# timohouben/GNN-XAI-TimeSeries-QualityControl

Measured on AMD Instinct MI355X. Metric: ROC-AUC (5-fold CV) + train windows/sec, CML GCN at 1/2/4/8 MI355X, higher is better.
Workload: dtype bf16; 1 GPU; model=CML GCN (GeneralConv16+mean pool+LSTM TimeLayer f16 n_stacks2+dense64), global_batch=128, seq_len=181, parallelism=dp1, adjacency=radius(max_sample_distance=20), graph_steps=8, trainable_params=188193, hip_graph=True

## Files before the change

csrc/kernels/lstm_chain.hip:

```cpp
#include "chain_head.h"
#include "common.h"
#include "gcn_fused.h"
#include "lstm_grads_body.h"
#include "lstm_tm_common.h"

#include <cstdlib>
#include <type_traits>

namespace gq {

typedef unsigned long long u64x2_t __attribute__((ext_vector_type(2)));
typedef unsigned u32x4_t __attribute__((ext_vector_type(4)));
typedef __bf16 bf16x2_t __attribute__((ext_vector_type(2)));

static constexpr int CHAIN_MAX = 8;
static constexpr int CHAIN_SPIN = 1 << 20;
#ifndef CHAIN_D
#define CHAIN_D 4
#endif
#ifndef CHAIN_D3
#define CHAIN_D3 2
#endif
#ifndef CHAIN_LEAD1
#define CHAIN_LEAD1 1
#endif
#ifndef CHAIN_D0
#define CHAIN_D0 6
#endif
#ifndef CHAIN_LD16
#define CHAIN_LD16 0
#endif
#ifndef CHAIN_W_SLEEP
#define CHAIN_W_SLEEP 0
#endif
#ifndef CHAIN_W_NAPMAX
#define CHAIN_W_NAPMAX 1
#endif
#ifndef CHAIN_RP_NAPMAX
#define CHAIN_RP_NAPMAX 16
#endif
#ifndef CHAIN_PRIO
#define CHAIN_PRIO 2
#endif
#ifndef CHAIN_LEAD3
#define CHAIN_LEAD3 1
#endif

struct ChainStage {
  const float* x;
  const unsigned long long* xin;
  const float* W;
  const float* U;
  const float* b;
  float* h;
  __bf16* g;
  float* c;
  unsigned long long* sout;
  float* pout;
  unsigned* iout;
  float* pin_out;
  unsigned char* pin_idx;
  long long* prof;
  int H, T, Din, Dw, KX, P, PIN;
};

struct ChainT4 {
  const unsigned long long* xin;
  const float* W;
  const float* U;
  const float* b;
  float* h;
  float* g;
  float* c;
  float* pin_out;
  unsigned char* pin_idx;
  int T, Din, Dw, on;
  ChainHead hd;
  float* hb;
};

struct ChainArgs {
  ChainStage st[CHAIN_MAX];
  int ns, ntiles, nt8, Mp;
  int* ctl;
  long long* trace;
  const float* pkU;
  const float* pkW;
  bf16x8_t* pk;
  int pkDw;
  int npk;
  ChainT4 t4;
  GcnCoefFwdJob cf;
  GcnProdJob gp;
};
static_assert(sizeof(ChainArgs) <= 4096, "chain forward kernel arguments");

__device__ __forceinline__ unsigned long long ld_granule(const unsigned long long* p) {
  return __hip_atomic_load(p, __ATOMIC_RELAXED, __HIP_MEMORY_SCOPE_AGENT);
}

__device__ __forceinline__ void st_granule(unsigned long long* p, float v, unsigned tag) {
  __hip_atomic_store(p, ((unsigned long long)tag << 32) | __float_as_uint(v), __ATOMIC_RELAXED,
                     __HIP_MEMORY_SCOPE_AGENT);
}

template <bool INL>
__device__ __forceinline__ unsigned long long chain_wait_body(const unsigned long long* p, unsigned want, int* ctl);
__device__ __noinline__ unsigned long long chain_wait(const unsigned long long* p, unsigned want, int* ctl) {
  return chain_wait_body<false>(p, want, ctl);
}
__device__ __forceinline__ unsigned long long chain_wait_inl(const unsigned long long* p, unsigned want, int* ctl) {
  return chain_wait_body<true>(p, want, ctl);
}
template <bool INL>
__device__ __forceinline__ unsigned long long chain_wait_body(const unsigned long long* p, unsigned want, int* ctl) {
  unsigned long long v = 0;
  const bool l0 = (threadIdx.x & 63) == 0;
#ifdef GQ_CHAIN_PROF
  if (l0) __hip_atomic_fetch_add(ctl + 9, 1, __ATOMIC_RELAXED, __HIP_MEMORY_SCOPE_AGENT);
#endif
  int nap = 1;
  const int lim0 = __hip_atomic_load(ctl + 6, __ATOMIC_RELAXED, __HIP_MEMORY_SCOPE_AGENT);
  const int lim = lim0 > 0 ? lim0 : CHAIN_SPIN;
  for (int it = 0; it < lim; ++it) {
    unsigned t0 = want;
    if (l0) t0 = (unsigned)(ld_granule(p) >> 32);
    if ((unsigned)__builtin_amdgcn_readfirstlane((int)t0) == want) {
      v = ld_granule(p);
      if (__builtin_amdgcn_ballot_w64((unsigned)(v >> 32) != want) == 0) return v;
    }
    for (int k = 0; k < nap; ++k) __builtin_amdgcn_s_sleep(CHAIN_W_SLEEP);
    nap = min(nap * 2, CHAIN_W_NAPMAX);
  }
  __hip_atomic_store(ctl + 2, 1, __ATOMIC_RELAXED, __HIP_MEMORY_SCOPE_AGENT);
  return v;
}

__device__ __forceinline__ void chain_wait_count(const int* p, int n, int* ctl) {
  const int lim0 = __hip_atomic_load(ctl + 6, __ATOMIC_RELAXED, __HIP_MEMORY_SCOPE_AGENT);
  const int lim = lim0 > 0 ? lim0 : CHAIN_SPIN;
  int nap = 1;
  for (int it = 0; it < lim; ++it) {
    if (__hip_atomic_load(p, __ATOMIC_RELAXED, __HIP_MEMORY_SCOPE_AGENT) >= n) return;
    for (int k = 0; k < nap; ++k) __builtin_amdgcn_s_sleep(CHAIN_W_SLEEP);
    nap = min(nap * 2, CHAIN_W_NAPMAX);
  }
  __hip_atomic_store(ctl + 2, 1, __ATOMIC_RELAXED, __HIP_MEMORY_SCOPE_AGENT);
}

static constexpr int CHAIN_PROF_STEPS = 64;
#ifdef GQ_CHAIN_PROF
__device__ __forceinline__ void chain_mark(long long* pr, int step, int k) {
  if (pr != nullptr && threadIdx.x == 0 && step < CHAIN_PROF_STEPS)
    pr[step * 8 + k] = (long long)__builtin_amdgcn_s_memtime();
}
__device__ __forceinline__ void chain_mark_wave(long long* pr, int step, int k) {
  if (pr != nullptr && (threadIdx.x & 63) == 0 && step < CHAIN_PROF_STEPS)
    pr[step * 8 + k] = (long long)__builtin_amdgcn_s_memtime();
}
#else
__device__ __forceinline__ void chain_mark(long long*, int, int) {}
__device__ __forceinline__ void chain_mark_wave(long long*, int, int) {}
#endif

__device__ __forceinline__ unsigned chain_tag_base(unsigned E) { return ((E % 0xFFFFFu) + 1u) << 12; }

template <int H, int KX>
struct ChainLds {
  static constexpr int HS = 2 * 16 * (TMC<H>::KPH + 8) * 2;
  static constexpr int XS = 2 * 16 * (32 * KX + 8) * 2;
  static constexpr int HF = 2 * 16 * TMC<H>::HP * 4;
  static constexpr int GS = 2 * 16 * H * 8;
  static constexpr int CS = 2 * 16 * H * 4;
  static constexpr int BYTES = HS + XS + HF + GS + CS;
};
constexpr int chain_max2(int a, int b) { return a > b ? a : b; }
static constexpr int CHAIN_LDS_STAGE = chain_max2(chain_max2(ChainLds<64, 2>::BYTES, ChainLds<32, 2>::BYTES),
                                                  ChainLds<16, 2>::BYTES);

__device__ __forceinline__ float chain_gate_scale(int ag) { return ag == 2 ? -2.8853900817779268f : -1.4426950408889634f; }

__host__ __device__ constexpr int chain_io_waves(int nt, int d, int ngl = 1, int pin = 1) {
  return nt + 64 * d + 64 <= 1024 && ngl * pin <= 12 ? d : 0;
}
__host__ __device__ constexpr int chain_io_group(int pin, int kx = 1, int h = 16) {
  return pin > 1 || (h == 64 && kx == 2) ? 2 : 1;
}
__host__ __device__ constexpr int chain_stage_d(int h, int kx, int d) {
  return h == 64 && kx == 2 && d > 3 ? 3 : d;
}
__host__ __device__ constexpr int chain_live_threads(int nt, int d, int kx, bool src, int pin, int h = 16) {
  return nt + 64 * chain_io_waves(nt, d * chain_io_group(pin, kx, h),
                                  (16 * 32 * kx / (src ? 2 : 4) + 64 * chain_io_group(pin, kx, h) - 1) /
                                      (64 * chain_io_group(pin, kx, h)),
                                  pin) +
         (chain_io_waves(nt, d * chain_io_group(pin, kx, h),
                         (16 * 32 * kx / (src ? 2 : 4) + 64 * chain_io_group(pin, kx, h) - 1) /
                             (64 * chain_io_group(pin, kx, h)),
                         pin) > 0 ? 64 : 0);
}

template <int H>
struct ChainCfg {
  static constexpr int CPL = H == 64 ? 2 : 1;
  static constexpr int NW = H / 4 / CPL, NT = 64 * NW, G4 = 4 * H;
  static constexpr int KSH = TMC<H>::KSH, KPH = TMC<H>::KPH, HP = TMC<H>::HP;
  static constexpr int NWV = H / 4, NCELL = 64 * NWV;
};

template <int H, bool TRAIN, int KX, int D, bool SRC, int PIN>
__device__ __forceinline__ void chain_stage(const ChainStage& S, int tile, int ntiles, int Mp, unsigned tagb,
                                            int* ctl, char* smem) {
  using C = ChainCfg<H>;
  constexpr int NW = C::NW, NT = C::NT, G4 = C::G4, CPL = C::CPL, NWV = C::NWV, NCELL = C::NCELL;
  constexpr int KPX = 32 * KX;
  constexpr int GR = SRC ? 2 : 4;
  constexpr int G = chain_io_group(PIN, KX, H);
  constexpr int NIOW = chain_io_waves(NT, D * G, (16 * KPX / GR + 64 * G - 1) / (64 * G), PIN);
  constexpr bool IOW = NIOW > 0;
  constexpr int NIO = IOW ? 64 * G : NT;
  constexpr int NSLOT = IOW ? 1 : D;
  constexpr int NGL = IOW ? (16 * KPX / GR + NIO - 1) / NIO : 1;
  using L = ChainLds<H, KX>;
  static_assert(L::BYTES <= CHAIN_LDS_STAGE && L::HS % 16 == 0 && L::XS % 16 == 0, "chain LDS layout");
  auto hs = reinterpret_cast<__bf16 (*)[16][C::KPH + 8]>(smem);
  auto xs = reinterpret_cast<__bf16 (*)[16][KPX + 8]>(smem + L::HS);
  auto hf = reinterpret_cast<float (*)[16][C::HP]>(smem + L::HS + L::XS);
  auto gst = reinterpret_cast<uint2 (*)[NCELL]>(smem + L::HS + L::XS + L::HF);
  auto cst = reinterpret_cast<float (*)[NCELL]>(smem + L::HS + L::XS + L::HF + L::GS);

  const int T = S.T, Din = S.Din, Dw = S.Dw, P = S.P;
  const int tid = threadIdx.x, lane = tid & 63;
  const int w = __builtin_amdgcn_readfirstlane(tid >> 6);
  const int col = lane & 15, quad = lane >> 4;
  const int row0 = tile * 16;
  const size_t hstep = (size_t)Mp * H;
  const int To = P > 0 ? T / P : T;

  constexpr int NTL = NT + 64 * NIOW + (IOW ? 64 : 0);
  for (int i = tid; i < 2 * 16 * (C::KPH + 8); i += NTL) (&hs[0][0][0])[i] = (__bf16)0.0f;
  for (int i = tid; i < 2 * 16 * (KPX + 8); i += NTL) (&xs[0][0][0])[i] = (__bf16)0.0f;

  const bool compute = w < NW;
  const int iow = IOW ? (w - NW) / G : 0;
  const int iot = IOW ? ((w - NW) % G) * 64 + lane : tid;
  const int n_gx = 16 * Din / GR;
  const size_t xstep = (size_t)Mp * Din;
  int goff[NGL], loff[NGL];
#pragma unroll
  for (int j = 0; j < NGL; ++j) {
    const int gx = min(iot + NIO * j, n_gx - 1) * GR;
    goff[j] = gx;
    loff[j] = ((gx / Din) * (KPX + 8) + gx % Din) * 2;
  }
  const size_t xbase = (size_t)row0 * Din;
  char* xsb = reinterpret_cast<char*>(&xs[0][0][0]);
  constexpr int XBUF = 16 * (KPX + 8) * 2;
  f32x4_t xr[NSLOT][NGL];
  u64x2_t xq[NSLOT][NGL][PIN];
  const __amdgpu_buffer_rsrc_t xrs = __builtin_amdgcn_make_buffer_rsrc(
      const_cast<unsigned long long*>(SRC ? S.xin : nullptr), (short)0, 0x7fffffff, 0x00020000);
  auto load_x = [&](int r, int tx) {
#pragma unroll
    for (int q = 0; q < (SRC ? PIN : 1); ++q) {
      const size_t tb = xbase + (size_t)(SRC ? PIN * tx + q : tx) * xstep;
#pragma unroll
      for (int j = 0; j < NGL; ++j) {
        if constexpr (SRC) {
#if CHAIN_LD16
          const u32x4_t v = __builtin_amdgcn_raw_buffer_load_b128(xrs, (int)((tb + goff[j]) * 8), 0, 16);
          xq[r][j][q] = u64x2_t{((unsigned long long)v.y << 32) | v.x, ((unsigned long long)v.w << 32) | v.z};
#else
          xq[r][j][q] = u64x2_t{ld_granule(S.xin + tb + goff[j]), ld_granule(S.xin + tb + goff[j] + 1)};
#endif
        } else {
          xr[r][j] = *reinterpret_cast<const f32x4_t*>(S.x + tb + goff[j]);
        }
      }
    }
  };
  auto stage_x = [&](int buf, int r, int tx) {
    if constexpr (SRC) {
      bool bad = false;
#pragma unroll
      for (int j = 0; j < NGL; ++j)
#pragma unroll
        for (int q = 0; q < PIN; ++q) {
          const unsigned want = tagb | (unsigned)(PIN * tx + q);
          bad |= (unsigned)(xq[r][j][q].x >> 32) != want || (unsigned)(xq[r][j][q].y >> 32) != want;
        }
      if (__builtin_amdgcn_ballot_w64(bad) != 0) {
#ifdef GQ_CHAIN_PROF
        if (lane == 0) __hip_atomic_fetch_add(ctl + 9, 1, __ATOMIC_RELAXED, __HIP_MEMORY_SCOPE_AGENT);
#endif
        const int lim0 = __hip_atomic_load(ctl + 6, __ATOMIC_RELAXED, __HIP_MEMORY_SCOPE_AGENT);
        const int lim = lim0 > 0 ? lim0 : CHAIN_SPIN;
        int nap = 1;
        for (int it = 0;; ++it) {
#pragma unroll
          for (int q = 0; q < PIN; ++q) {
            const size_t tb = xbase + (size_t)(PIN * tx + q) * xstep;
#pragma unroll
            for (int j = 0; j < NGL; ++j)
              xq[r][j][q] = u64x2_t{ld_granule(S.xin + tb + goff[j]), ld_granule(S.xin + tb + goff[j] + 1)};
          }
          bad = false;
#pragma unroll
          for (int j = 0; j < NGL; ++j)
#pragma unroll
            for (int q = 0; q < PIN; ++q) {
              const unsigned want = tagb | (unsigned)(PIN * tx + q);
              bad |= (unsigned)(xq[r][j][q].x >> 32) != want || (unsigned)(xq[r][j][q].y >> 32) != want;
            }
          if (__builtin_amdgcn_ballot_w64(bad) == 0) break;
          if (it >= lim) {
            __hip_atomic_store(ctl + 2, 1, __ATOMIC_RELAXED, __HIP_MEMORY_SCOPE_AGENT);
            break;
          }
          for (int k = 0; k < nap; ++k) __builtin_amdgcn_s_sleep(2);
          nap = min(nap * 2, CHAIN_RP_NAPMAX);
        }
      }
      const size_t po = xbase + (size_t)tx * xstep;
#pragma unroll
      for (int j = 0; j < NGL; ++j) {
        float m0 = __uint_as_float((unsigned)xq[r][j][0].x), m1 = __uint_as_float((unsigned)xq[r][j][0].y);
        if constexpr (PIN > 1) {
          unsigned a0 = 0, a1 = 0;
#pragma unroll
          for (int q = 1; q < PIN; ++q) {
            const float v0 = __uint_as_float((unsigned)xq[r][j][q].x), v1 = __uint_as_float((unsigned)xq[r][j][q].y);
            if (v0 > m0) { m0 = v0; a0 = q; }
            if (v1 > m1) { m1 = v1; a1 = q; }
          }
          *reinterpret_cast<float2*>(S.pin_out + po + goff[j]) = make_float2(m0, m1);
          *reinterpret_cast<unsigned short*>(S.pin_idx + po + goff[j]) = (unsigned short)(a0 | (a1 << 8));
        }
        *reinterpret_cast<bf16x2_t*>(xsb + buf * XBUF + loff[j]) = bf16x2_t{(__bf16)m0, (__bf16)m1};
      }
    } else {
#pragma unroll
      for (int j = 0; j < NGL; ++j) {
        const bf16x4_t v = __builtin_convertvector(xr[r][j], bf16x4_t);
        *reinterpret_cast<bf16x4_t*>(xsb + buf * XBUF + loff[j]) = v;
      }
    }
  };

  const int wc = compute ? w : 0;
  const int ag = col & 3;
  int unit[CPL];
  bf16x8_t ufr[CPL][C::KSH], wfr[CPL][KX];
  f32x4_t bias4[CPL];
#pragma unroll
  for (int cc = 0; cc < CPL; ++cc) {
    const int gi = wc + NW * cc;
    const int au = 4 * gi + (col >> 2);
    unit[cc] = 4 * gi + quad;
    bias4[cc] = f32x4_t{0.f, 0.f, 0.f, 0.f};
    if (compute) {
#pragma unroll
      for (int s = 0; s < C::KSH; ++s) {
        bf16x8_t v;
#pragma unroll
        for (int j = 0; j < 8; ++j) {
          const int k = 32 * s + 8 * quad + j;
          v[j] = (__bf16)(S.U[min(k, H - 1) * G4 + ag * H + au] * (k < H ? 1.0f : 0.0f));
        }
        ufr[cc][s] = v;
      }
#pragma unroll
      for (int s = 0; s < KX; ++s) {
        bf16x8_t v;
#pragma unroll
        for (int j = 0; j < 8; ++j) {
          const int k = 32 * s + 8 * quad + j;
          v[j] = (__bf16)(S.W[min(k, Dw - 1) * G4 + ag * H + au] * (k < Dw ? 1.0f : 0.0f));
        }
        wfr[cc][s] = v;
      }
      const int u = unit[cc];
      bias4[cc] = f32x4_t{S.b[u], S.b[H + u], S.b[2 * H + u], S.b[3 * H + u]};
    }
  }
  float* hp[CPL];
  unsigned long long* sp[CPL];
  __bf16* gp[CPL];
  float* cp[CPL];
  const size_t gstride = (size_t)ntiles * NWV * 64;
#pragma unroll
  for (int cc = 0; cc < CPL; ++cc) {
    const size_t hoff = (size_t)(row0 + col) * H + unit[cc];
    hp[cc] = S.h + hoff;
    sp[cc] = S.sout != nullptr ? S.sout + hoff : nullptr;
    gp[cc] = S.g + (((size_t)tile * NWV + wc + NW * cc) * 64 + lane) * 4;
    cp[cc] = S.c + ((size_t)tile * NWV + wc + NW * cc) * 64 + lane;
  }
  const bool publish = S.sout != nullptr;
  const bool own_pool = P > 0;

  constexpr int n_gh = 16 * H / 4;
  constexpr int NPT = IOW ? 64 : NT;
  constexpr int NPL = (n_gh + NPT - 1) / NPT;
  PoolAcc pool[NPL];
  const bool publisher = IOW && w == NW + NIOW;
  const bool pooler = IOW ? publisher : wave_uniform(tid < n_gh);
  auto pool_step = [&](int tp) {
#pragma unroll
    for (int q = 0; q < NPL; ++q) {
      const int gh = (((IOW ? lane : tid) + NPT * q) % n_gh) * 4;
      const float4 v = *reinterpret_cast<const float4*>(&hf[tp & 1][gh / H][gh % H]);
      pool[q].step(v, tp, P, To, S.pout, S.iout, (size_t)row0 * H + gh, hstep);
    }
  };

  const bool streamer = IOW ? (!compute && !publisher) : true;
  if (streamer) {
    if constexpr (SRC) {
      constexpr int LEAD = PIN > 1 ? CHAIN_LEAD3 : CHAIN_LEAD1;
      const int tw = min(D + LEAD, T - 1);
      (void)chain_wait(S.xin + xbase + goff[0] + 1 + (size_t)(PIN * tw + PIN - 1) * xstep,
                       tagb | (unsigned)(PIN * tw + PIN - 1), ctl);
    }
    if constexpr (IOW) {
      load_x(0, min(iow, T - 1));
    } else {
#pragma unroll
      for (int r = 0; r < D; ++r) load_x(r, min(r, T - 1));
    }
  }
  __syncthreads();
  if (IOW ? (streamer && iow == 0) : streamer) {
    stage_x(0, 0, 0);
    if (!IOW) load_x(0, min(D, T - 1));
  }
  float c[CPL];
#pragma unroll
  for (int cc = 0; cc < CPL; ++cc) c[cc] = 0.f;
  __syncthreads();

  long long* pr = (S.prof != nullptr && tile == 0) ? S.prof : nullptr;
  auto compute_step = [&](int t, auto IO, int rn) {
    constexpr bool DOI = decltype(IO)::value;
    const int p = t & 1;
    chain_mark(pr, t, 0);
    f32x4_t acc[CPL];
#pragma unroll
    for (int cc = 0; cc < CPL; ++cc) {
      f32x4_t accx = bias4[cc], acch = {0.f, 0.f, 0.f, 0.f};
#pragma unroll
      for (int s = 0; s < KX; ++s) {
        const bf16x8_t bx = *reinterpret_cast<const bf16x8_t*>(&xs[p][col][32 * s + 8 * quad]);
        accx = __builtin_amdgcn_mfma_f32_16x16x32_bf16(wfr[cc][s], bx, accx, 0, 0, 0);
      }
#pragma unroll
      for (int s = 0; s < C::KSH; ++s) {
        const bf16x8_t bh = *reinterpret_cast<const bf16x8_t*>(&hs[p][col][32 * s + 8 * quad]);
        acch = __builtin_amdgcn_mfma_f32_16x16x32_bf16(ufr[cc][s], bh, acch, 0, 0, 0);
      }
      acc[cc] = accx + acch;
    }
    chain_mark(pr, t, 1);
    if constexpr (DOI) {
      stage_x(p ^ 1, rn, min(t + 1, T - 1));
      load_x(rn, min(t + 1 + D, T - 1));
    }
#pragma unroll
    for (int cc = 0; cc < CPL; ++cc) {
      const f32x4_t a = acc[cc];
      const int u = unit[cc], cell = (wc + NW * cc) * 64 + lane;
      const float iv = __builtin_amdgcn_rcpf(1.0f + __builtin_amdgcn_exp2f(chain_gate_scale(0) * a[0]));
      const float fv = __builtin_amdgcn_rcpf(1.0f + __builtin_amdgcn_exp2f(chain_gate_scale(1) * a[1]));
      const float gv = 2.0f * __builtin_amdgcn_rcpf(1.0f + __builtin_amdgcn_exp2f(chain_gate_scale(2) * a[2])) - 1.0f;
      const float ov = __builtin_amdgcn_rcpf(1.0f + __builtin_amdgcn_exp2f(chain_gate_scale(3) * a[3]));
      c[cc] = fv * c[cc] + iv * gv;
      const float rc = __builtin_amdgcn_rcpf(1.0f + __builtin_amdgcn_exp2f(-2.8853900817779268f * c[cc]));
      const float hv = (2.0f * ov) * rc - ov;
      hs[p ^ 1][col][u] = (__bf16)hv;
      if (publish) st_granule(sp[cc] + (size_t)t * hstep, hv, tagb | (unsigned)t);
      if constexpr (IOW) {
        hf[p][col][u] = hv;
        if constexpr (TRAIN) {
          gst[p][cell] = gates_pack(iv, fv, gv, ov);
          cst[p][cell] = c[cc];
        }
      } else {
        if (own_pool) hf[p][col][u] = hv;
        hp[cc][(size_t)t * hstep] = hv;
        if constexpr (TRAIN) {
          *reinterpret_cast<uint2*>(gp[cc] + (size_t)t * gstride * 4) = gates_pack(iv, fv, gv, ov);
          cp[cc][(size_t)t * gstride] = c[cc];
        }
      }
    }
    chain_mark(pr, t, 2);
  };
  auto publish_step = [&](int tp) {
    const int pb = tp & 1;
    const size_t tile_off = ((size_t)tp * Mp + row0) * H;
#pragma unroll
    for (int q = lane; q < 16 * H / 4; q += 64) {
      const int e = 4 * q;
      *reinterpret_cast<float4*>(S.h + tile_off + e) = *reinterpret_cast<const float4*>(&hf[pb][e / H][e % H]);
    }
    if constexpr (TRAIN) {
      const size_t cell0 = ((size_t)tp * ntiles + tile) * NCELL;
#pragma unroll
      for (int q = lane; q < NCELL / 2; q += 64)
        *reinterpret_cast<uint4*>(S.g + (cell0 + 2 * q) * 4) = *reinterpret_cast<const uint4*>(&gst[pb][2 * q]);
#pragma unroll
      for (int q = lane; q < NCELL / 4; q += 64)
        *reinterpret_cast<float4*>(S.c + cell0 + 4 * q) = *reinterpret_cast<const float4*>(&cst[pb][4 * q]);
    }
    if (own_pool) pool_step(tp);
  };
  using yes = std::true_type;
  using no = std::false_type;
  if constexpr (IOW) {
    if (compute) {
      if (CHAIN_PRIO > 0) __builtin_amdgcn_s_setprio(CHAIN_PRIO);
      for (int t = 0; t < T; ++t) {
        compute_step(t, no{}, 0);
        lds_barrier();
        chain_mark(pr, t, 3);
      }
      __builtin_amdgcn_s_setprio(0);
    } else if (publisher) {
      for (int t = 0; t < T; ++t) {
        if (t >= 1) publish_step(t - 1);
        chain_mark_wave(pr, t, 7);
        lds_barrier();
      }
      publish_step(T - 1);
    } else {
      int kt = (iow + D - 1) % D;
      int next_ld = iow == 0 ? D : -1;
      for (int t = 0; t < T; ++t) {
        if (next_ld >= 0) {
          load_x(0, min(next_ld, T - 1));
          next_ld = -1;
        }
        if (kt == 0 && t + 1 < T) {
          if (iot == 0) chain_mark_wave(pr, t, 4);
          stage_x((t + 1) & 1, 0, t + 1);
          if (iot == 0) chain_mark_wave(pr, t, 5);
          next_ld = t + 1 + D;
          if (iot == 0) chain_mark_wave(pr, t, 6);
        }
        kt = kt == 0 ? D - 1 : kt - 1;
        lds_barrier();
      }
    }
  } else {
    for (int t0 = 0; t0 < T; t0 += D) {
#pragma unroll
      for (int r = 0; r < D; ++r) {
        const int t = t0 + r;
        if (t >= T) break;
        compute_step(t, yes{}, (r + 1 == D) ? 0 : r + 1);
        if (own_pool && pooler && t >= 1) pool_step(t - 1);
        lds_barrier();
        chain_mark(pr, t, 3);
      }
    }
  }
  if constexpr (!IOW) {
    if (own_pool && pooler) pool_step(T - 1);
  }
}

struct ChainT4Lds {
  static constexpr int HS = 2 * 16 * (128 + 8) * 2;
  static constexpr int XS = 2 * 16 * (64 + 8) * 2;
  static constexpr int HL = 16 * (128 + 4) * 4;
  static constexpr int DHT = 16 * (128 + 4) * 4;
  static constexpr int HF = ChainHeadFwdLds<128>::BYTES;
  static constexpr int HB = DHT + ChainHeadDhLds<128>::BYTES;
  static constexpr int BYTES = HS + XS + HL + HF + HB;
};

template <bool TRAIN>
__device__ __forceinline__ void chain_t4_stage(const ChainT4 Q, int tile, int ntiles, int Mp, unsigned tagb, int* ctl,
                                               char* smem) {
  constexpr int H = 128, G4 = 4 * H, NW = 16, CPL = 2, KX = 2, KSH = H / 32, HPB = H + 8, XP = 64 + 8;
  static_assert(ChainT4Lds::HS % 16 == 0 && ChainT4Lds::XS % 16 == 0 && ChainT4Lds::HL % 16 == 0, "t4 LDS layout");
  auto hs = reinterpret_cast<__bf16 (*)[16][HPB]>(smem);
  auto xs = reinterpret_cast<__bf16 (*)[16][XP]>(smem + ChainT4Lds::HS);
  float* hl = reinterpret_cast<float*>(smem + ChainT4Lds::HS + ChainT4Lds::XS);
  const int T = Q.T, Din = Q.Din, Dw = Q.Dw;
  const int tid = threadIdx.x, lane = tid & 63;
  const int w = __builtin_amdgcn_readfirstlane(tid >> 6);
  const int col = lane & 15, quad = lane >> 4;
  const int row0 = tile * 16;

  for (int i = tid; i < 2 * 16 * HPB; i += 1024) (&hs[0][0][0])[i] = (__bf16)0.0f;
  for (int i = tid; i < 2 * 16 * XP; i += 1024) (&xs[0][0][0])[i] = (__bf16)0.0f;
  const int n_el = 16 * Din;
  const bool own = tid < n_el;
  const int el = min(tid, n_el - 1), er = el / Din, ek = el % Din;
  const size_t xstep = (size_t)Mp * Din, xoff = (size_t)(row0 + er) * Din + ek;
  unsigned long long xq[3];
  auto load_x = [&](int tx) {
#pragma unroll
    for (int r = 0; r < 3; ++r) xq[r] = ld_granule(Q.xin + xoff + (size_t)(3 * tx + r) * xstep);
  };
  load_x(0);

  bf16x8_t ufr[CPL][KSH], wfr[CPL][KX];
  f32x4_t bias4[CPL];
  int unit[CPL];
#pragma unroll
  for (int cc = 0; cc < CPL; ++cc) {
    const int gi = w + NW * cc;
    const int au = 4 * gi + (col >> 2), ag = col & 3;
    unit[cc] = 4 * gi + quad;
#pragma unroll
    for (int s = 0; s < KSH; ++s) {
      bf16x8_t v;
#pragma unroll
      for (int j = 0; j < 8; ++j) v[j] = (__bf16)Q.U[(32 * s + 8 * quad + j) * G4 + ag * H + au];
      ufr[cc][s] = v;
    }
#pragma unroll
    for (int s = 0; s < KX; ++s) {
      bf16x8_t v;
#pragma unroll
      for (int j = 0; j < 8; ++j) {
        const int k = 32 * s + 8 * quad + j;
        v[j] = (__bf16)(Q.W[min(k, Dw - 1) * G4 + ag * H + au] * (k < Dw ? 1.0f : 0.0f));
      }
      wfr[cc][s] = v;
    }
    const int u = unit[cc];
    bias4[cc] = f32x4_t{Q.b[u], Q.b[H + u], Q.b[2 * H + u], Q.b[3 * H + u]};
  }

  auto stage_x = [&](int buf, int tx) {
    bool bad = false;
#pragma unroll
    for (int r = 0; r < 3; ++r) bad |= (unsigned)(xq[r] >> 32) != (tagb | (unsigned)(3 * tx + r));
    if (__builtin_amdgcn_ballot_w64(bad) != 0) {
      const int lim0 = __hip_atomic_load(ctl + 6, __ATOMIC_RELAXED, __HIP_MEMORY_SCOPE_AGENT);
      const int lim = lim0 > 0 ? lim0 : CHAIN_SPIN;
      for (int it = 0;; ++it) {
        __builtin_amdgcn_s_sleep(1);
#pragma unroll
        for (int r = 0; r < 3; ++r) xq[r] = ld_granule(Q.xin + xoff + (size_t)(3 * tx + r) * xstep);
        bad = false;
#pragma unroll
        for (int r = 0; r < 3; ++r) bad |= (unsigned)(xq[r] >> 32) != (tagb | (unsigned)(3 * tx + r));
        if (__builtin_amdgcn_ballot_w64(bad) == 0) break;
        if (it >= lim) {
          __hip_atomic_store(ctl + 2, 1, __ATOMIC_RELAXED, __HIP_MEMORY_SCOPE_AGENT);
          break;
        }
      }
    }
    float m = __uint_as_float((unsigned)xq[0]);
    unsigned arg = 0;
#pragma unroll
    for (int r = 1; r < 3; ++r) {
      const float v = __uint_as_float((unsigned)xq[r]);
      if (v > m) { m = v; arg = r; }
    }
    if (own) {
      Q.pin_out[xoff + (size_t)tx * xstep] = m;
      Q.pin_idx[xoff + (size_t)tx * xstep] = (unsigned char)arg;
      xs[buf][er][ek] = (__bf16)m;
    }
  };

  __syncthreads();
  stage_x(0, 0);
  if (T > 1) load_x(1);
  float c[CPL];
#pragma unroll
  for (int cc = 0; cc < CPL; ++cc) c[cc] = 0.f;
  __syncthreads();

  for (int t = 0; t < T; ++t) {
    const int p = t & 1;
    f32x4_t acc[CPL];
#pragma unroll
    for (int cc = 0; cc < CPL; ++cc) {
      f32x4_t accx = bias4[cc], acch = {0.f, 0.f, 0.f, 0.f};
#pragma unroll
      for (int s = 0; s < KX; ++s) {
        const bf16x8_t bx = *reinterpret_cast<const bf16x8_t*>(&xs[p][col][32 * s + 8 * quad]);
        accx = __builtin_amdgcn_mfma_f32_16x16x32_bf16(wfr[cc][s], bx, accx, 0, 0, 0);
      }
#pragma unroll
      for (int s = 0; s < KSH; ++s) {
        const bf16x8_t bh = *reinterpret_cast<const bf16x8_t*>(&hs[p][col][32 * s + 8 * quad]);
        acch = __builtin_amdgcn_mfma_f32_16x16x32_bf16(ufr[cc][s], bh, acch, 0, 0, 0);
      }
      acc[cc] = accx + acch;
    }
    if (wave_uniform(t + 1 < T)) {
      stage_x(p ^ 1, t + 1);
      if (wave_uniform(t + 2 < T)) load_x(t + 2);
    }
#pragma unroll
    for (int cc = 0; cc < CPL; ++cc) {
      const float iv = sigmoidf_fast(acc[cc][0]);
      const float fv = sigmoidf_fast(acc[cc][1]);
      const float gv = tanhf_fast(acc[cc][2]);
      const float ov = sigmoidf_fast(acc[cc][3]);
      const float cold = c[cc];
      c[cc] = fv * cold + iv * gv;
      const float hv = ov * tanhf_fast(c[cc]);
      const int u = unit[cc];
      hs[p ^ 1][col][u] = (__bf16)hv;
      Q.h[((size_t)t * Mp + row0 + col) * H + u] = hv;
      if (t == T - 1) hl[col * (H + 4) + u] = hv;
      if constexpr (TRAIN) {
        const int gi = w + NW * cc;
        const size_t o = ((((size_t)t * ntiles + tile) * 8 + (gi & 7)) * 4 + (gi >> 3)) * 64 + lane;
        *reinterpret_cast<float4*>(Q.g + o * 4) = make_float4(iv, fv, gv, ov);
        *reinterpret_cast<float2*>(Q.c + o * 2) = make_float2(c[cc], cold);
      }
    }
    lds_barrier();
  }
  __syncthreads();
}

__device__ __forceinline__ void chain_finish(int* ctl, int nblk) {
  if (threadIdx.x == 0) {
    const int old = __hip_atomic_fetch_add(ctl + 1, 1, __ATOMIC_RELAXED, __HIP_MEMORY_SCOPE_AGENT);
    if (old == nblk - 1) {
      __hip_atomic_store(ctl + 1, 0, __ATOMIC_RELAXED, __HIP_MEMORY_SCOPE_AGENT);
      __hip_atomic_store(ctl + 10, 0, __ATOMIC_RELAXED, __HIP_MEMORY_SCOPE_AGENT);
      __hip_atomic_fetch_add(ctl, 1, __ATOMIC_RELAXED, __HIP_MEMORY_SCOPE_AGENT);
    }
  }
}

static constexpr int CHAIN_LDS = ChainT4Lds::BYTES > CHAIN_LDS_STAGE ? ChainT4Lds::BYTES : CHAIN_LDS_STAGE;

template <bool TRAIN>
__global__ __launch_bounds__(1024) void lstm_chain_fwd_kernel(ChainArgs A) {
  const int nblk = gridDim.x;
  __shared__ __attribute__((aligned(16))) char smem[CHAIN_LDS];
  if ((int)blockIdx.x >= A.ns * A.nt8) {
    int r = (int)blockIdx.x - A.ns * A.nt8;
    if (A.t4.on) {
      if (r < A.nt8) {
        if (r < A.ntiles) {
          if (threadIdx.x == 0) A.trace[2 * blockIdx.x] = (long long)__builtin_amdgcn_s_memrealtime();
          const unsigned tagb = chain_tag_base((unsigned)__hip_atomic_load(A.ctl, __ATOMIC_RELAXED, __HIP_MEMORY_SCOPE_AGENT));
          constexpr int HOFF = ChainT4Lds::HS + ChainT4Lds::XS + ChainT4Lds::HL;
          float* hW1 = ch_head_fwd_weights<128>(smem + HOFF);
          ch_stage_weights<128>(A.t4.hd, hW1, hW1 + 128 * CH_WP);
          if (A.gp.on) {
            if (threadIdx.x == 0) chain_wait_count(A.ctl + 10, A.gp.Mp, A.ctl);
            __syncthreads();
          }
          const bool pre = TRAIN && A.t4.hb != nullptr;
          constexpr int OFF = HOFF + ChainT4Lds::HF;
          char* dhscr = smem + OFF + ChainT4Lds::DHT;
          if (pre) ch_mask_partials(A.t4.hd.mask, A.t4.hd.M, ch_head_dh_red<128>(dhscr));
          chain_t4_stage<TRAIN>(A.t4, r, A.ntiles, A.Mp, tagb, A.ctl, smem);
          long long* mk = blockIdx.x < 64 ? A.trace + 512 + blockIdx.x : nullptr;
          if (mk != nullptr && threadIdx.x == 0) mk[0] = (long long)__builtin_amdgcn_s_memrealtime();
          if (threadIdx.x >= 64 * CH_NW) return;
          ChainHeadKeep keep;
          chain_head_fwd<128>(A.t4.hd, r, A.ntiles, reinterpret_cast<const float*>(smem + ChainT4Lds::HS + ChainT4Lds::XS),
                              smem + HOFF, true, !pre, pre ? ch_head_dh_sz1<128>(dhscr) : nullptr, &keep);
          if (mk != nullptr && threadIdx.x == 0) mk[64] = (long long)__builtin_amdgcn_s_memrealtime();
          if constexpr (TRAIN) {
            if (A.t4.hb != nullptr) {
              float* dhs = reinterpret_cast<float*>(smem + OFF);
              chain_head_dh<128>(A.t4.hd, r, keep, smem + HOFF, dhscr, dhs);
              __syncthreads();
              for (int e = ch_tid(); e < 16 * 128; e += 64 * CH_NW)
                A.t4.hb[((size_t)r * 16 + e / 128) * 128 + e % 128] = dhs[(e / 128) * 132 + e % 128];
              chain_head_fwd_handoff<128>(A.t4.hd, r, A.ntiles, smem + HOFF);
            }
          }
          __syncthreads();
          if (threadIdx.x == 0) A.trace[2 * blockIdx.x + 1] = (long long)__builtin_amdgcn_s_memrealtime();
        }
        chain_finish(A.ctl, nblk);
        return;
      }
      r -= A.nt8;
    }
    if (r < A.npk) {
      const int f = r * 1024 + (int)threadIdx.x;
      if (A.pk != nullptr && f < T4PK_ALL) t4_pack_one(f, A.pkU, A.pkW, A.pkDw, A.pk);
    } else if (A.cf.on && r - A.npk < A.cf.Mp) {
      gcn_coef_fwd_body<2, 16>(A.cf, r - A.npk, smem);
    } else if (A.gp.on && r - A.npk - (A.cf.on ? A.cf.Mp : 0) < A.gp.Mp) {
      if (threadIdx.x == 0 && blockIdx.x < 256) A.trace[2 * blockIdx.x] = (long long)__builtin_amdgcn_s_memrealtime();
      const unsigned E = (unsigned)__hip_atomic_load(A.ctl, __ATOMIC_RELAXED, __HIP_MEMORY_SCOPE_AGENT);
      const int row = r - A.npk - (A.cf.on ? A.cf.Mp : 0);
      gcn_prod_body<2, 16>(A.gp, row, chain_tag_base(E), A.ctl + 10, smem, row < 32 ? A.trace + 640 + 4 * row : nullptr);
      if (threadIdx.x == 0 && blockIdx.x < 256) A.trace[2 * blockIdx.x + 1] = (long long)__builtin_amdgcn_s_memrealtime();
    }
    chain_finish(A.ctl, nblk);
    return;
  }
  const int s = blockIdx.x / A.nt8, tile = blockIdx.x % A.nt8;
  if (s >= A.ns || tile >= A.ntiles) {
    chain_finish(A.ctl, nblk);
    return;
  }
  if (threadIdx.x == 0) A.trace[2 * blockIdx.x] = (long long)__builtin_amdgcn_s_memrealtime();
  const unsigned E = (unsigned)__hip_atomic_load(A.ctl, __ATOMIC_RELAXED, __HIP_MEMORY_SCOPE_AGENT);
  const unsigned tagb = chain_tag_base(E);
  const ChainStage S = A.st[s];
  const int H = S.H, KX = S.KX;
  const bool src = s > 0 || A.gp.on;
#define GQ_CHAIN_BODY(HH, KXX, DD, SRCV, PINV)                                          \
  {                                                                                     \
    constexpr int DS = chain_stage_d(HH, KXX, DD);                                      \
    if (threadIdx.x >= chain_live_threads(ChainCfg<HH>::NT, DS, KXX, SRCV, PINV, HH)) return; \
    chain_stage<HH, TRAIN, KXX, DS, SRCV, PINV>(S, tile, A.ntiles, A.Mp, tagb, A.ctl, smem); \
  }
#define GQ_CHAIN_SRC(HH, PINV, DD)                                                      \
  if (KX == 1) GQ_CHAIN_BODY(HH, 1, DD, true, PINV) else GQ_CHAIN_BODY(HH, 2, DD, true, PINV)
#define GQ_CHAIN_KX(HH)                                                                 \
  if (src) { if (S.PIN == 3) { GQ_CHAIN_SRC(HH, 3, CHAIN_D3) } else { GQ_CHAIN_SRC(HH, 1, CHAIN_D) } } \
  else { if (KX == 1) GQ_CHAIN_BODY(HH, 1, CHAIN_D0, false, 1) else GQ_CHAIN_BODY(HH, 2, CHAIN_D0, false, 1) }
  if (H == 16) GQ_CHAIN_KX(16)
  else if (H == 32) GQ_CHAIN_KX(32)
  else GQ_CHAIN_KX(64)
#undef GQ_CHAIN_KX
#undef GQ_CHAIN_SRC
#undef GQ_CHAIN_BODY
  __syncthreads();
  if (threadIdx.x == 0) A.trace[2 * blockIdx.x + 1] = (long long)__builtin_amdgcn_s_memrealtime();
  chain_finish(A.ctl, nblk);
}

struct ChainBStage {
  const float* dh;
  const unsigned long long* din;
  const unsigned char* pidx;
  const __bf16* g;
  const float* c;
  const float* W;
  const float* U;
  __bf16* dz;
  unsigned long long* sout;
  float* dx;
  long long* trace_mid;
  long long* prof;
  const unsigned char* uidx;
  int uP, uT, punp;
  int H, T, Din, Dw, KX, P, Ts;
};

struct ChainT4B {
  const float* h;
  const float* g;
  const float* c;
  const bf16x8_t* pk;
  const float* hb;
  __bf16* dz;
  unsigned long long* sout;
  int T, Din, Dw, on;
  ChainHead hd;
};

struct ChainBArgs {
  ChainBStage st[CHAIN_MAX];
  int ns, ntiles, nt8, Mp;
  int* ctl;
  long long* trace;
  ChainT4B t4;
};
static_assert(sizeof(ChainBArgs) <= 4096, "chain backward kernel arguments");

#ifndef CHAINB_ZPAD
#define CHAINB_ZPAD 16
#endif
#ifndef CHAINB_XPAD
#define CHAINB_XPAD 1
#endif
template <int KX>
struct ChainBLds16 {
  static constexpr int ZS = 2 * 16 * (4 * 16 + CHAINB_ZPAD) * 2;
  static constexpr int DH = 2 * 16 * TMC<16>::HP * 4;
  static constexpr int DX = 2 * 16 * (32 * KX + CHAINB_XPAD) * 4;
  static constexpr int BYTES = ZS + DH + DX;
};
template <int H, int KX>
struct ChainBLdsSK {
  static constexpr int NW = TMC<H>::NW, UT = H / 16, KG = NW / UT, NXB = 2 * KX, KXG = NW / NXB;
  static constexpr int ZS = 2 * 16 * (4 * H + CHAINB_ZPAD) * 2;
  static constexpr int DH = 2 * 16 * TMC<H>::HP * 4;
  static constexpr int DP = KG * 16 * TMC<H>::HP * 4;
  static constexpr int XPP = 32 * KX + 4;
  static constexpr int XP = 2 * KXG * 16 * XPP * 4;
  static constexpr int BYTES = ZS + DH + DP + XP;
};
constexpr int chainb_max(int a, int b) { return a > b ? a : b; }
static constexpr int CHAINB_LDS_STAGE =
    chainb_max(chainb_max(ChainBLds16<1>::BYTES, ChainBLds16<2>::BYTES),
               chainb_max(chainb_max(ChainBLdsSK<32, 1>::BYTES, ChainBLdsSK<32, 2>::BYTES),
                          chainb_max(ChainBLdsSK<64, 1>::BYTES, ChainBLdsSK<64, 2>::BYTES)));

struct ChainT4BLds {
  static constexpr int DHT = 16 * 132 * 4;
  static constexpr int ZS = 16 * (512 + 8) * 2;
  static constexpr int DN = 2 * 16 * 132 * 4;
  static constexpr int DXP = 4 * 16 * 68 * 4;
  static constexpr int STEP = ZS + DN + DXP;
  static constexpr int HEAD = ChainHeadBwdLds<128>::BYTES;
  static constexpr int BYTES = DHT + (STEP > HEAD ? STEP : HEAD);
};
static constexpr int CHAINB_LDS = ChainT4BLds::BYTES > CHAINB_LDS_STAGE ? ChainT4BLds::BYTES : CHAINB_LDS_STAGE;

#ifndef CHAINB_LEAD
#define CHAINB_LEAD 1
#endif
#ifndef CHAINB_PUBBATCH
#define CHAINB_PUBBATCH 4
#endif
#ifndef CHAINB_NPUB
#define CHAINB_NPUB 4
#endif
#ifndef CHAINB_PUBPRIO
#define CHAINB_PUBPRIO 2
#endif
#ifndef CHAINB_DXPRIO
#define CHAINB_DXPRIO 2
#endif
#ifndef CHAINB_D16
#define CHAINB_D16 4
#endif
#ifndef CHAINB_D32
#define CHAINB_D32 4
#endif
#ifndef CHAINB_D64
#define CHAINB_D64 2
#endif
__host__ __device__ constexpr bool chainb_dxw(int h) {
  return h < 32 && TMC<16>::NT + 64 * CHAINB_NPUB + 64 <= 1024;
}
__host__ __device__ constexpr int chainb_npub(int h, int nt) {
  return nt + 64 > 1024 ? 0
       : chainb_max(1, CHAINB_NPUB < (1024 - nt - (chainb_dxw(h) ? 64 : 0) - 64) / 64
                           ? CHAINB_NPUB : (1024 - nt - (chainb_dxw(h) ? 64 : 0) - 64) / 64);
}
__host__ __device__ constexpr bool chainb_dzw(int h, int nt) {
  return chainb_npub(h, nt) > 0 && nt + 64 * chainb_npub(h, nt) + 64 + (chainb_dxw(h) ? 64 : 0) <= 1024;
}
__host__ __device__ constexpr int chainb_live_threads(int h, int nt) {
  return nt + 64 * chainb_npub(h, nt) + (chainb_dxw(h) ? 64 : 0) + (chainb_dzw(h, nt) ? 64 : 0);
}
static_assert(chainb_dxw(16) && chainb_dzw(16, TMC<16>::NT) && chainb_npub(16, TMC<16>::NT) == CHAINB_NPUB &&
                  !chainb_dxw(32) && chainb_dzw(32, TMC<32>::NT) && chainb_npub(32, TMC<32>::NT) == CHAINB_NPUB &&
                  chainb_live_threads(64, TMC<64>::NT) == 1024,
              "wave roles of the backward stages (chain_bwd_stage16, chain_bwd_stage_sk)");

template <int KX, int D, bool SRC, bool UP, bool XO>
__device__ __forceinline__ void chain_bwd_stage16(const ChainBStage S, int tile, int ntiles, int Mp, unsigned tagb,
                                                  int* ctl, char* smem) {
  constexpr int H = 16;
  using C = TMC<H>;
  constexpr int NW = C::NW, NT = C::NT, G4 = C::G4, KB = C::KB;
  constexpr int NXB = KX * 2;
  constexpr int NPUB = CHAINB_NPUB;
  static_assert(C::CPL == 1 && 16 * H == NT && KB == 2, "one dh element per lane, two K blocks of dz");
  static_assert(D >= 2, "H = 16 stage: ring of at least two steps");
  using L = ChainBLds16<KX>;
  static_assert(L::BYTES <= CHAINB_LDS_STAGE && L::ZS % 16 == 0 && L::DH % 16 == 0, "chain bwd LDS layout");
  auto zs = reinterpret_cast<__bf16 (*)[16][G4 + CHAINB_ZPAD]>(smem);
  auto dhs = reinterpret_cast<float (*)[16][C::HP]>(smem + L::ZS);
  auto dxs = reinterpret_cast<float (*)[16][32 * KX + CHAINB_XPAD]>(smem + L::ZS + L::DH);

  const int T = S.T, Din = S.Din, Dw = S.Dw, P = S.P, Ts = S.Ts;
  const int tid = threadIdx.x, lane = tid & 63;
  const int row0 = tile * 16;
  if (tid >= NT + 64 * NPUB + 64) {
    if (CHAINB_PUBPRIO > 0) __builtin_amdgcn_s_setprio(CHAINB_PUBPRIO);
    const int nsteps = (T + D - 1) / D * D;
    __syncthreads();
    __syncthreads();
    for (int s = 0; s < nsteps; ++s) {
      lds_barrier();
      if (s < T) {
        const int pb = s & 1;
        __bf16* zt = S.dz + ((size_t)(T - 1 - s) * Mp + row0) * G4;
#pragma unroll
        for (int q = lane; q < 16 * G4 / 8; q += 64) {
          const int e = 8 * q;
          *reinterpret_cast<uint4*>(zt + e) = *reinterpret_cast<const uint4*>(&zs[pb][e / G4][e % G4]);
        }
      }
    }
    __syncthreads();
    return;
  }
  if (tid >= NT + 64 * NPUB) {
    if (CHAINB_DXPRIO > 0) __builtin_amdgcn_s_setprio(CHAINB_DXPRIO);
    const int col = lane & 15, quad = lane >> 4;
    bf16x8_t wx[NXB][KB];
#pragma unroll
    for (int xb = 0; xb < NXB; ++xb) {
      const int din = 16 * xb + col;
#pragma unroll
      for (int k = 0; k < KB; ++k) {
        bf16x8_t v;
#pragma unroll
        for (int j = 0; j < 8; ++j)
          v[j] = (__bf16)(S.W[(size_t)min(din, Dw - 1) * G4 + 32 * k + 8 * quad + j] * (din < Dw ? 1.f : 0.f));
        wx[xb][k] = v;
      }
    }
    const int nsteps = (T + D - 1) / D * D;
    __syncthreads();
    __syncthreads();
    for (int s = 0; s < nsteps; ++s) {
      lds_barrier();
      if (s < T) {
        const int p = s & 1;
        bf16x8_t bz[KB];
#pragma unroll
        for (int k = 0; k < KB; ++k) bz[k] = *reinterpret_cast<const bf16x8_t*>(&zs[p][col][32 * k + 8 * quad]);
#pragma unroll
        for (int xb = 0; xb < NXB; ++xb) {
          f32x4_t a = {0.f, 0.f, 0.f, 0.f};
#pragma unroll
          for (int k = 0; k < KB; ++k) a = __builtin_amdgcn_mfma_f32_16x16x32_bf16(wx[xb][k], bz[k], a, 0, 0, 0);
#pragma unroll
          for (int r = 0; r < 4; ++r) dxs[p][col][16 * xb + 4 * quad + r] = a[r];
        }
        chain_mark_wave((S.prof != nullptr && tile == 0) ? S.prof : nullptr, s, 6);
      }
    }
    __syncthreads();
    return;
  }
  if (tid >= NT) {
    if (CHAINB_PUBPRIO > 0) __builtin_amdgcn_s_setprio(CHAINB_PUBPRIO);
    const int nsteps = (T + D - 1) / D * D;
    const int nx = 16 * Din;
    const size_t xstep = (size_t)Mp * Din;
    const int pj = (tid - NT) >> 6;
    constexpr int ESTR = 64 * NPUB;
    const int dq = ESTR / Din, dr = ESTR % Din;
    constexpr int PUBN = CHAINB_PUBBATCH > 0 ? CHAINB_PUBBATCH : 1;
    auto publish = [&](int buf, int ts) {
      const unsigned tag = tagb | (unsigned)ts;
      for (int e0 = 64 * pj; e0 < nx; e0 += ESTR * PUBN) {
        const int niter = min((nx - e0 + ESTR - 1) / ESTR, PUBN);
        float vv[PUBN];
        int row = (lane + e0) / Din, k = (lane + e0) % Din;
#pragma unroll
        for (int i = 0; i < PUBN; ++i) {
          if (i < niter) {
            vv[i] = dxs[buf][row][k];
          }
          row += dq;
          k += dr;
          if (k >= Din) { k -= Din; ++row; }
        }
#pragma unroll
        for (int i = 0; i < PUBN; ++i) {
          if (i < niter) {
            const int e = e0 + lane + ESTR * i;
            const size_t o = (size_t)row0 * Din + e + (size_t)ts * xstep;
            if constexpr (XO) st_granule(S.sout + o, vv[i], tag);
            else S.dx[o] = vv[i];
          }
        }
      }
    };
    __syncthreads();
    __syncthreads();
    long long* prw = (S.prof != nullptr && tile == 0 && pj == 0) ? S.prof : nullptr;
    for (int s = 0; s < nsteps; ++s) {
      lds_barrier();
      const int t = T - 1 - s;
      if (s >= 1 && s <= T) publish((s - 1) & 1, t + 1);
      if (s < T) chain_mark_wave(prw, s, 7);
    }
    __syncthreads();
    publish((T - 1) & 1, 0);
    return;
  }
  const int w = __builtin_amdgcn_readfirstlane(tid >> 6);
  const int col = lane & 15, quad = lane >> 4;

  for (int i = tid; i < 2 * 16 * C::HP; i += NT) (&dhs[0][0][0])[i] = 0.f;

  const int unit = 4 * w + quad;
  bf16x8_t ufr[KB];
  {
    const int au = 4 * w + (col >> 2);
#pragma unroll
    for (int s = 0; s < KB; ++s) {
      bf16x8_t v;
#pragma unroll
      for (int j = 0; j < 8; ++j) {
        const float val = S.U[(size_t)au * G4 + 32 * s + 8 * quad + j];
        v[j] = (__bf16)(val * ((col & 3) == 0 ? 1.f : 0.f));
      }
      ufr[s] = v;
    }
  }

  uint2 rg[D];
  float rc[D];
  unsigned long long rq[D];
  unsigned ri[D];
  const unsigned pmag = (UP && P > 1) ? 0xFFFFFFFFu / (unsigned)P + 1u : 0u;
  auto divp = [&](int tt) { return P > 1 ? (int)__umulhi((unsigned)tt, pmag) : tt; };
  auto src_t = [&](int tt) {
    if constexpr (UP) return tt < Ts * P ? divp(tt) : -1;
    else return tt;
  };
  const size_t eoff = (size_t)row0 * H + tid;
  const size_t hstep = (size_t)Mp * H;

  if constexpr (SRC) {
    int tw = T - 1 - (D + CHAINB_LEAD);
    tw = max(tw, 0);
    const int st = src_t(tw);
    if (st >= 0) (void)chain_wait(S.din + eoff + (size_t)st * hstep, tagb | (unsigned)st, ctl);
  }
  constexpr unsigned NOSRC = 0xFFFFFFFFu;
  const unsigned lo8 = (unsigned)((tile * NW + w) * 64 + lane) * 8u;
  const unsigned gstr = (unsigned)(ntiles * NW * 64 * 8);
  const char* gbase = reinterpret_cast<const char*>(S.g);
  const char* cbase = reinterpret_cast<const char*>(S.c);
  int stt = T - 1;
  auto state_load = [&](int J) {
    const unsigned o = (unsigned)__builtin_amdgcn_readfirstlane(stt) * gstr + lo8;
    rg[J] = *reinterpret_cast<const uint2*>(gbase + o);
    rc[J] = *reinterpret_cast<const float*>(cbase + (o >> 1));
    stt = max(stt - 1, 0);
  };
  constexpr unsigned ESZ = SRC ? 8 : 4;
  const unsigned eo = (unsigned)eoff;
  const unsigned hrow = (unsigned)hstep;
  const char* dbase = SRC ? reinterpret_cast<const char*>(S.din) : reinterpret_cast<const char*>(S.dh);
  const char* pbase = reinterpret_cast<const char*>(S.pidx);
  int dtt = T - 1;
  int dst = UP ? min(divp(dtt), Ts - 1) : dtt;
  int dph = UP ? dtt - dst * P : 0;
  const unsigned dlim = (unsigned)(UP ? Ts * P : T);
  unsigned rinf[D];
  auto ring_load = [&](int J) {
    const unsigned o = (unsigned)max(dst, 0) * hrow + eo;
    if constexpr (SRC) rq[J] = ld_granule(reinterpret_cast<const unsigned long long*>(dbase + o * ESZ));
    else rq[J] = (unsigned long long)__float_as_uint(*reinterpret_cast<const float*>(dbase + o * ESZ));
    if constexpr (UP) ri[J] = (unsigned)*reinterpret_cast<const unsigned char*>(pbase + o);
    else ri[J] = 0u;
    const unsigned inf = ((unsigned)dph << 12) | (unsigned)dst;
    rinf[J] = (unsigned)dtt < dlim ? inf : NOSRC;
    --dtt;
    if constexpr (UP) {
      const bool wrap = dph == 0;
      dst = wrap ? dst - 1 : dst;
      dph = wrap ? P - 1 : dph - 1;
    } else {
      --dst;
    }
  };
  auto stage = [&](int J) -> float {
    const unsigned inf = rinf[J];
    const bool has = inf != NOSRC;
    if constexpr (SRC) {
      const unsigned want = tagb | (inf & 0xfffu);
      const bool bad = has && (unsigned)(rq[J] >> 32) != want;
      if (__builtin_amdgcn_ballot_w64(bad) != 0) {
        rq[J] = chain_wait(S.din + eoff + (size_t)(inf & 0xfffu) * hstep, want, ctl);
      }
    }
    const float v = __uint_as_float((unsigned)rq[J]);
    bool keep = has;
    if constexpr (UP) keep = keep && ri[J] == (inf >> 12);
    return keep ? v : 0.f;
  };
  float tc, fo, ff, z0, z1, z2, z3;
  auto cell_pre_c = [&](int J) { tc = tanhf_fast(rc[J]); };
  auto cell_pre = [&](int J, int JN, int tt) {
    const float cp = rc[JN] * (tt > 0 ? 1.f : 0.f);
    const float4 g4 = gates_unpack(rg[J]);
    fo = g4.w * (1.f - tc * tc);
    ff = g4.y;
    z0 = g4.z * g4.x * (1.f - g4.x);
    z1 = cp * g4.y * (1.f - g4.y);
    z2 = g4.x * (1.f - g4.z * g4.z);
    z3 = tc * g4.w * (1.f - g4.w);
  };
  float dc = 0.f;
  auto cell_tail = [&](int pb, float dh) {
    const float dct = dc + dh * fo;
    dc = dct * ff;
    zs[pb][col][0 * H + unit] = (__bf16)(dct * z0);
    zs[pb][col][1 * H + unit] = (__bf16)(dct * z1);
    zs[pb][col][2 * H + unit] = (__bf16)(dct * z2);
    zs[pb][col][3 * H + unit] = (__bf16)(dh * z3);
  };

#pragma unroll
  for (int j = 0; j < D; ++j) {
    state_load(j);
    ring_load(j);
  }
  __syncthreads();
  dhs[0][tid / H][tid % H] = stage(0);
  ring_load(0);
  dhs[1][tid / H][tid % H] = stage(1);
  ring_load(1);
  __syncthreads();
  float dhn = dhs[0][col][unit];
  if (tid == 0 && S.trace_mid) S.trace_mid[blockIdx.x] = (long long)__builtin_amdgcn_s_memrealtime();
  cell_pre_c(0);
  cell_pre(0, 1, T - 1);
  cell_tail(0, dhn);
  state_load(0);

  long long* pr = (S.prof != nullptr && tile == 0) ? S.prof : nullptr;
  for (int s0 = 0; s0 < T; s0 += D) {
#pragma unroll
    for (int j = 0; j < D; ++j) {
      const int s = s0 + j;
      const int p = s & 1;
      const int j1 = (j + 1) % D, j2 = (j + 2) % D;
      lds_barrier();
      chain_mark(pr, s, 0);
      const bf16x8_t bz0 = *reinterpret_cast<const bf16x8_t*>(&zs[p][col][8 * quad]);
      __builtin_amdgcn_sched_barrier(0);
      f32x4_t a0 = __builtin_amdgcn_mfma_f32_16x16x32_bf16(ufr[0], bz0, f32x4_t{0.f, 0.f, 0.f, 0.f}, 0, 0, 0);
      __builtin_amdgcn_sched_barrier(0);
      const bf16x8_t bz1 = *reinterpret_cast<const bf16x8_t*>(&zs[p][col][32 + 8 * quad]);
      dhn = dhs[p ^ 1][col][unit];
      dhs[p][tid / H][tid % H] = stage(j2);
      ring_load(j2);
      chain_mark(pr, s, 1);
      __builtin_amdgcn_sched_barrier(0);
      const f32x4_t a1 = __builtin_amdgcn_mfma_f32_16x16x32_bf16(ufr[1], bz1, f32x4_t{0.f, 0.f, 0.f, 0.f}, 0, 0, 0);
      __builtin_amdgcn_sched_barrier(0);
      cell_pre_c(j1);
      cell_pre(j1, j2, T - 2 - s);
      __builtin_amdgcn_sched_barrier(0);
      float dhr = a0[0] + a1[0];
#ifdef GQ_CHAIN_PROF
      if (pr != nullptr) asm volatile("" : "+v"(dhr));
#endif
      chain_mark(pr, s, 2);
      cell_tail(p ^ 1, dhn + dhr);
      chain_mark(pr, s, 3);
      state_load(j1);
      chain_mark(pr, s, 4);
    }
  }
  __syncthreads();
}

template <int H, int KX, int D, bool SRC, bool UP, bool XO>
__device__ __forceinline__ void chain_bwd_stage_sk(const ChainBStage S, int tile, int ntiles, int Mp, unsigned tagb,
                                                   int* ctl, char* smem) {
  using C = TMC<H>;
  constexpr int CPL = C::CPL, NW = C::NW, NT = C::NT, G4 = C::G4, KB = C::KB;
  constexpr int NXB = KX * 2;
  static_assert(H >= 32 && CPL == 1 && 16 * H == NT, "one dh element per lane");
  using LK = ChainBLdsSK<H, KX>;
  constexpr int UT = LK::UT, KG = LK::KG, KXG = LK::KXG, KPG = KB / KG, KPX = KB / KXG;
  constexpr int NPUB = CHAINB_NPUB;
  static_assert(NW % UT == 0 && KB % KG == 0 && NW % NXB == 0 && KB % KXG == 0, "split-K tiling");
  static_assert(LK::BYTES <= CHAINB_LDS_STAGE && LK::ZS % 16 == 0 && LK::DH % 16 == 0, "chain bwd LDS layout");
  auto zs = reinterpret_cast<__bf16 (*)[16][G4 + CHAINB_ZPAD]>(smem);
  auto dhs = reinterpret_cast<float (*)[16][C::HP]>(smem + LK::ZS);
  auto dpart = reinterpret_cast<float (*)[16][C::HP]>(smem + LK::ZS + LK::DH);
  auto xpart = reinterpret_cast<float (*)[KXG][16][LK::XPP]>(smem + LK::ZS + LK::DH + LK::DP);

  const int T = S.T, Din = S.Din, Dw = S.Dw, P = S.P, Ts = S.Ts;
  const int tid = threadIdx.x, lane = tid & 63;
  const int row0 = tile * 16;
  constexpr bool PUBW = H == 32;
  if constexpr (PUBW) {
    if (tid >= NT + 64 * NPUB) {
      if (CHAINB_PUBPRIO > 0) __builtin_amdgcn_s_setprio(CHAINB_PUBPRIO);
      const int nsteps = (T + D - 1) / D * D;
      __syncthreads();
      __syncthreads();
      for (int s = 0; s < nsteps; ++s) {
        lds_barrier();
        if (s < T) {
          const int pb = s & 1;
          __bf16* zt = S.dz + ((size_t)(T - 1 - s) * Mp + row0) * G4;
#pragma unroll
          for (int q = lane; q < 16 * G4 / 8; q += 64) {
            const int e = 8 * q;
            *reinterpret_cast<uint4*>(zt + e) = *reinterpret_cast<const uint4*>(&zs[pb][e / G4][e % G4]);
          }
        }
        lds_barrier();
      }
      __syncthreads();
      return;
    }
    if (tid >= NT) {
      if (CHAINB_PUBPRIO > 0) __builtin_amdgcn_s_setprio(CHAINB_PUBPRIO);
      const int nsteps = (T + D - 1) / D * D;
      const int nx = 16 * Din;
      const size_t xstep = (size_t)Mp * Din;
      const int pj = (tid - NT) >> 6;
      constexpr int ESTR = 64 * NPUB;
      const int dq = ESTR / Din, dr = ESTR % Din;
      constexpr int PUBN = CHAINB_PUBBATCH > 0 ? CHAINB_PUBBATCH : 1;
      auto publish = [&](int buf, int ts) {
        const unsigned tag = tagb | (unsigned)ts;
        for (int e0 = 64 * pj; e0 < nx; e0 += ESTR * PUBN) {
          const int niter = min((nx - e0 + ESTR - 1) / ESTR, PUBN);
          float vv[PUBN];
          int row = (lane + e0) / Din, k = (lane + e0) % Din;
#pragma unroll
          for (int i = 0; i < PUBN; ++i) {
            if (i < niter) {
              float v = 0.f;
#pragma unroll
              for (int g = 0; g < KXG; ++g) v += xpart[buf][g][row][k];
              vv[i] = v;
            }
            row += dq;
            k += dr;
            if (k >= Din) { k -= Din; ++row; }
          }
#pragma unroll
          for (int i = 0; i < PUBN; ++i) {
            if (i < niter) {
              const int e = e0 + lane + ESTR * i;
              const size_t o = (size_t)row0 * Din + e + (size_t)ts * xstep;
              if constexpr (XO) st_granule(S.sout + o, vv[i], tag);
              else S.dx[o] = vv[i];
            }
          }
        }
      };
      __syncthreads();
      __syncthreads();
      for (int s = 0; s < nsteps; ++s) {
        lds_barrier();
        lds_barrier();
        if (s < T) publish(s & 1, T - 1 - s);
      }
      __syncthreads();
      return;
    }
  }
  const int w = __builtin_amdgcn_readfirstlane(tid >> 6);
  const int col = lane & 15, quad = lane >> 4;

  for (int i = tid; i < 2 * 16 * C::HP; i += NT) (&dhs[0][0][0])[i] = 0.f;

  const int unit = 4 * w + quad;
  const int ut = w % UT, kg = w / UT, xt = w % NXB, kx = w / NXB;
  bf16x8_t ufr[KPG];
  bf16x8_t ufk[KPX];
#pragma unroll
  for (int q = 0; q < KPG; ++q) {
    bf16x8_t v;
#pragma unroll
    for (int j = 0; j < 8; ++j) v[j] = (__bf16)S.U[(size_t)(16 * ut + col) * G4 + 32 * (kg * KPG + q) + 8 * quad + j];
    ufr[q] = v;
  }
  {
    const int din = 16 * xt + col;
#pragma unroll
    for (int q = 0; q < KPX; ++q) {
      bf16x8_t v;
#pragma unroll
      for (int j = 0; j < 8; ++j)
        v[j] = (__bf16)(S.W[(size_t)min(din, Dw - 1) * G4 + 32 * (kx * KPX + q) + 8 * quad + j] * (din < Dw ? 1.f : 0.f));
      ufk[q] = v;
    }
  }

  uint2 rg[D];
  float rc[D];
  unsigned long long rq[D];
  unsigned ri[D];
  auto sidx = [&](int tt) { return ((((size_t)tt * ntiles + tile) * NW + w)) * 64 + lane; };
  const unsigned pmag = (UP && P > 1) ? 0xFFFFFFFFu / (unsigned)P + 1u : 0u;
  auto divp = [&](int tt) { return P > 1 ? (int)__umulhi((unsigned)tt, pmag) : tt; };
  auto src_t = [&](int tt) {
    if constexpr (UP) return tt < Ts * P ? divp(tt) : -1;
    else return tt;
  };
  const size_t eoff = (size_t)row0 * H + tid;
  const size_t hstep = (size_t)Mp * H;
  auto load_dh = [&](int J, int SS) {
    const int tt = max(T - 1 - SS, 0);
    const int st = max(src_t(tt), 0);
    if constexpr (SRC) rq[J] = ld_granule(S.din + eoff + (size_t)st * hstep);
    else rq[J] = (unsigned long long)__float_as_uint(S.dh[eoff + (size_t)st * hstep]);
    if constexpr (UP) ri[J] = (unsigned)S.pidx[eoff + (size_t)st * hstep];
    else ri[J] = 0u;
  };
  auto load = [&](int J, int SS) {
    const size_t o = sidx(max(T - 1 - SS, 0));
    rg[J] = *reinterpret_cast<const uint2*>(S.g + o * 4);
    rc[J] = S.c[o];
    load_dh(J, SS);
  };
  auto stage_dh = [&](int J, int tt) -> float {
    const int st = tt >= 0 ? src_t(tt) : -1;
    if constexpr (SRC) {
      const bool bad = st >= 0 && (unsigned)(rq[J] >> 32) != (tagb | (unsigned)st);
      if (__builtin_amdgcn_ballot_w64(bad) != 0)
        rq[J] = chain_wait(S.din + eoff + (size_t)max(st, 0) * hstep, tagb | (unsigned)max(st, 0), ctl);
    }
    const float v = __uint_as_float((unsigned)rq[J]);
    bool keep = st >= 0;
    if constexpr (UP) keep = keep && ri[J] == (unsigned)(tt - st * P);
    return keep ? v : 0.f;
  };
  const int gz_seq = tid / (G4 / 4), gz_c = (tid % (G4 / 4)) * 4;
  __bf16* zbase = S.dz + (size_t)(row0 + gz_seq) * G4 + gz_c;
  const size_t zstep = (size_t)Mp * G4;
  constexpr int NQ = (16 * 64 + NT - 1) / NT;
  const int nx = 16 * Din;
  const size_t xstep = (size_t)Mp * Din;
  int xrow[NQ], xk[NQ], xo[NQ];
#pragma unroll
  for (int q = 0; q < NQ; ++q) {
    const int e = min(tid + q * NT, nx - 1);
    xrow[q] = e / Din;
    xk[q] = e % Din;
    xo[q] = row0 * Din + e;
  }
  auto store_dx = [&](int buf, int ts, unsigned tag) {
#pragma unroll
    for (int q = 0; q < NQ; ++q) {
      float v = 0.f;
#pragma unroll
      for (int g = 0; g < KXG; ++g) v += xpart[buf][g][xrow[q]][xk[q]];
      const size_t o = (size_t)xo[q] + (size_t)ts * xstep;
      if constexpr (XO) st_granule(S.sout + o, v, tag);
      else S.dx[o] = v;
    }
  };

  if constexpr (SRC) {
    int tw = T - 1 - (D + CHAINB_LEAD);
    tw = max(tw, 0);
    const int st = src_t(tw);
    if (st >= 0) (void)chain_wait(S.din + eoff + (size_t)st * hstep, tagb | (unsigned)st, ctl);
  }
#pragma unroll
  for (int j = 0; j < D; ++j) load(j, j);
  __syncthreads();
  dhs[0][tid / H][tid % H] = stage_dh(0, T - 1);
  load_dh(0, D);
  float dc = 0.f, dhr = 0.f, dhn;
  __syncthreads();
  dhn = dhs[0][col][unit];
  if (tid == 0 && S.trace_mid) S.trace_mid[blockIdx.x] = (long long)__builtin_amdgcn_s_memrealtime();

  long long* pr = (S.prof != nullptr && tile == 0) ? S.prof : nullptr;
  for (int s0 = 0; s0 < T; s0 += D) {
#pragma unroll
    for (int j = 0; j < D; ++j) {
      const int s = s0 + j;
      const int t = T - 1 - s;
      const int p = s & 1;
      const int jn = (j + 1 == D) ? 0 : j + 1;
      chain_mark(pr, s, 0);
      {
        const float cp = rc[jn] * (t > 0 ? 1.f : 0.f);
        const float dh = dhn + dhr;
        const float4 g4 = gates_unpack(rg[j]);
        const float tc = tanhf_fast(rc[j]);
        const float dct = dc + dh * g4.w * (1.f - tc * tc);
        dc = dct * g4.y;
        zs[p][col][0 * H + unit] = (__bf16)(dct * g4.z * g4.x * (1.f - g4.x));
        zs[p][col][1 * H + unit] = (__bf16)(dct * cp * g4.y * (1.f - g4.y));
        zs[p][col][2 * H + unit] = (__bf16)(dct * g4.x * (1.f - g4.z * g4.z));
        zs[p][col][3 * H + unit] = (__bf16)(dh * tc * g4.w * (1.f - g4.w));
      }
      {
        const int tt = max(T - 1 - (s + D), 0);
        const size_t o = sidx(tt);
        rg[j] = *reinterpret_cast<const uint2*>(S.g + o * 4);
        rc[j] = S.c[o];
      }
      chain_mark(pr, s, 1);
      dhs[p ^ 1][tid / H][tid % H] = stage_dh(jn, t - 1);
      chain_mark(pr, s, 2);
      {
        const int tt = max(T - 1 - (s + 1 + D), 0);
        const int st = max(src_t(tt), 0);
        if constexpr (SRC) rq[jn] = ld_granule(S.din + eoff + (size_t)st * hstep);
        else rq[jn] = (unsigned long long)__float_as_uint(S.dh[eoff + (size_t)st * hstep]);
        if constexpr (UP) ri[jn] = (unsigned)S.pidx[eoff + (size_t)st * hstep];
        else ri[jn] = 0u;
      }
      lds_barrier();
      chain_mark(pr, s, 3);
      dhn = dhs[p ^ 1][col][unit];
      {
        f32x4_t a = {0.f, 0.f, 0.f, 0.f};
#pragma unroll
        for (int q = 0; q < KPG; ++q) {
          const bf16x8_t bz = *reinterpret_cast<const bf16x8_t*>(&zs[p][col][32 * (kg * KPG + q) + 8 * quad]);
          a = __builtin_amdgcn_mfma_f32_16x16x32_bf16(ufr[q], bz, a, 0, 0, 0);
        }
        f32x4_t b = {0.f, 0.f, 0.f, 0.f};
#pragma unroll
        for (int q = 0; q < KPX; ++q) {
          const bf16x8_t bz = *reinterpret_cast<const bf16x8_t*>(&zs[p][col][32 * (kx * KPX + q) + 8 * quad]);
          b = __builtin_amdgcn_mfma_f32_16x16x32_bf16(ufk[q], bz, b, 0, 0, 0);
        }
#pragma unroll
        for (int r = 0; r < 4; ++r) {
          dpart[kg][col][16 * ut + 4 * quad + r] = a[r];
          xpart[p][kx][col][16 * xt + 4 * quad + r] = b[r];
        }
      }
      chain_mark(pr, s, 4);
      if constexpr (!PUBW) {
        const uint2 zv = *reinterpret_cast<const uint2*>(&zs[p][gz_seq][gz_c]);
        const int tz = t >= 0 ? t : T;
        *reinterpret_cast<uint2*>(zbase + (size_t)tz * zstep) = zv;
      }
      if constexpr (!PUBW) {
        const int ts = (s >= 1 && s <= T) ? t + 1 : T;
        store_dx(p ^ 1, ts, tagb | (unsigned)ts);
      }
      {
        lds_barrier();
        float sdh = 0.f;
#pragma unroll
        for (int g = 0; g < KG; ++g) sdh += dpart[g][col][unit];
        dhr = sdh;
      }
      chain_mark(pr, s, 5);
    }
  }
  __syncthreads();
  if constexpr (!PUBW) store_dx((T - 1) & 1, 0, tagb);
}

typedef __attribute__((address_space(4))) ChainBArgs ChainBKernArgs;
typedef __attribute__((address_space(3))) char ChainLdsChar;
__device__ __noinline__ void chain_t4_bwd_records(const ChainBKernArgs* ka, ChainLdsChar* smem, int tile, int ntiles,
                                                  int Mp) {
  using L = ChainT4BLds;
  char* s = (char*)smem;
  const ChainT4B& Q = ((const ChainBArgs*)ka)->t4;
  chain_head_bwd<128>(Q.hd, Q.h + (size_t)(Q.T - 1) * Mp * 128, tile, ntiles, reinterpret_cast<float*>(s), s + L::DHT);
}

__device__ __forceinline__ void chain_t4_bwd_stage(const ChainT4B Q, const ChainBKernArgs* kargs, int tile, int ntiles,
                                                   int Mp, unsigned tagb, char* smem, long long* mk = nullptr) {
  constexpr int H = 128, G4 = 4 * H, NW = 16, CPL = 2, HP = H + 4, ZP = G4 + 8, XP = 68;
  using L = ChainT4BLds;
  static_assert(L::DHT % 16 == 0 && L::ZS % 16 == 0 && L::DN % 16 == 0, "t4 backward LDS layout");
  float* dhT = reinterpret_cast<float*>(smem);
  char* rs = smem + L::DHT;
  auto zs = reinterpret_cast<__bf16 (*)[ZP]>(rs);
  auto dhn = reinterpret_cast<float (*)[16][HP]>(rs + L::ZS);
  auto dxp = reinterpret_cast<float (*)[16][XP]>(rs + L::ZS + L::DN);
  const int T = Q.T, Din = Q.Din, Dw = Q.Dw;
  const int tid = threadIdx.x, lane = tid & 63;
  const int w = __builtin_amdgcn_readfirstlane(tid >> 6);
  const int col = lane & 15, quad = lane >> 4;
  const int row0 = tile * 16;

  int unit[CPL];
  size_t so[CPL];
#pragma unroll
  for (int cc = 0; cc < CPL; ++cc) {
    const int gi = w + NW * cc;
    unit[cc] = 4 * gi + quad;
    so[cc] = (((size_t)tile * 8 + (gi & 7)) * 4 + (gi >> 3)) * 64 + lane;
  }
  const size_t sstep = (size_t)ntiles * 8 * 4 * 64;
  float4 rg[2][CPL];
  float2 rcs[2][CPL];
  auto load_slot = [&](int j, int t) {
    const size_t tc = (size_t)max(t, 0);
#pragma unroll
    for (int cc = 0; cc < CPL; ++cc) {
      const size_t o = tc * sstep + so[cc];
      rg[j][cc] = *reinterpret_cast<const float4*>(Q.g + o * 4);
      rcs[j][cc] = *reinterpret_cast<const float2*>(Q.c + o * 2);
    }
  };
  load_slot(0, T - 1);
  load_slot(1, T - 2);
  if (Q.hb != nullptr) {
    const float gl = Q.hd.dloss[0];
    for (int e = tid; e < 16 * H; e += 1024) dhT[(e / H) * HP + e % H] = gl * Q.hb[((size_t)tile * 16 + e / H) * H + e % H];
  } else {
    chain_head_bwd<H>(Q.hd, Q.h + (size_t)(T - 1) * Mp * H, tile, ntiles, dhT, rs);
  }
  const int ut = w & 7, kh = w >> 3, dt = w & 3, kq = w >> 2;
  bf16x8_t ufr[8], wfr[4];
  {
    const bf16x8_t* pu = Q.pk + T4PK_N + (size_t)ut * 16 * 64 + lane;
    const bf16x8_t* pw = Q.pk + T4PK_N + T4PK_BU + (size_t)(dt + 4 * (kq >> 1)) * 8 * 64 + lane;
#pragma unroll
    for (int s = 0; s < 8; ++s) ufr[s] = pu[(8 * kh + s) * 64];
#pragma unroll
    for (int s = 0; s < 4; ++s) wfr[s] = pw[(4 * (kq & 1) + s) * 64];
  }
  __syncthreads();
  if (mk != nullptr && tid == 0) mk[0] = (long long)__builtin_amdgcn_s_memrealtime();
  const int nx = 16 * Din;
  const bool ownx = tid < nx;
  const int ex = min(tid, nx - 1), er = ex / Din, ek = ex % Din;
  const size_t xstep = (size_t)Mp * Din, xoff = (size_t)(row0 + er) * Din + ek;
  const int zq = tid >> 6, zc = (tid & 63) * 8;
  float dc[CPL], dhr[CPL];
#pragma unroll
  for (int cc = 0; cc < CPL; ++cc) dc[cc] = dhr[cc] = 0.f;
  for (int s0 = 0; s0 < T; s0 += 2) {
#pragma unroll
  for (int j = 0; j < 2; ++j) {
    const int s = s0 + j;
    if (s >= T) break;
    const int t = T - 1 - s;
#pragma unroll
    for (int cc = 0; cc < CPL; ++cc) {
      const int u = unit[cc];
      const float dh = dhr[cc] + (s == 0 ? dhT[col * HP + u] : 0.f);
      const float4 g = rg[j][cc];
      const float cprev = rcs[j][cc].y;
      const float tc = tanhf_fast(rcs[j][cc].x);
      const float dct = dc[cc] + dh * g.w * (1.f - tc * tc);
      dc[cc] = dct * g.y;
      zs[col][0 * H + u] = (__bf16)(dct * g.z * g.x * (1.f - g.x));
      zs[col][1 * H + u] = (__bf16)(dct * cprev * g.y * (1.f - g.y));
      zs[col][2 * H + u] = (__bf16)(dct * g.x * (1.f - g.z * g.z));
      zs[col][3 * H + u] = (__bf16)(dh * tc * g.w * (1.f - g.w));
    }
    load_slot(j, t - 2);
    lds_barrier();
    *reinterpret_cast<uint4*>(Q.dz + ((size_t)t * Mp + row0 + zq) * G4 + zc) = *reinterpret_cast<const uint4*>(&zs[zq][zc]);
    {
      f32x4_t a0 = {0.f, 0.f, 0.f, 0.f}, a1 = a0, b0 = a0, b1 = a0;
#pragma unroll
      for (int q = 0; q < 8; ++q) {
        const bf16x8_t bz = *reinterpret_cast<const bf16x8_t*>(&zs[col][32 * (8 * kh + q) + 8 * quad]);
        if (q & 1) a1 = __builtin_amdgcn_mfma_f32_16x16x32_bf16(ufr[q], bz, a1, 0, 0, 0);
        else a0 = __builtin_amdgcn_mfma_f32_16x16x32_bf16(ufr[q], bz, a0, 0, 0, 0);
      }
#pragma unroll
      for (int q = 0; q < 4; ++q) {
        const bf16x8_t bz = *reinterpret_cast<const bf16x8_t*>(&zs[col][32 * (4 * kq + q) + 8 * quad]);
        if (q & 1) b1 = __builtin_amdgcn_mfma_f32_16x16x32_bf16(wfr[q], bz, b1, 0, 0, 0);
        else b0 = __builtin_amdgcn_mfma_f32_16x16x32_bf16(wfr[q], bz, b0, 0, 0, 0);
      }
      const f32x4_t a = a0 + a1, b = b0 + b1;
#pragma unroll
      for (int r = 0; r < 4; ++r) {
        dhn[kh][col][16 * ut + 4 * quad + r] = a[r];
        dxp[kq][col][16 * dt + 4 * quad + r] = b[r];
      }
    }
    lds_barrier();
#pragma unroll
    for (int cc = 0; cc < CPL; ++cc) dhr[cc] = dhn[0][col][unit[cc]] + dhn[1][col][unit[cc]];
    const float v = (dxp[0][er][ek] + dxp[1][er][ek]) + (dxp[2][er][ek] + dxp[3][er][ek]);
    if (ownx) st_granule(Q.sout + xoff + (size_t)t * xstep, v, tagb | (unsigned)t);
  }
  }
  if (mk != nullptr && tid == 0) mk[64] = (long long)__builtin_amdgcn_s_memrealtime();
  if (Q.hb != nullptr) {
    __syncthreads();
    chain_t4_bwd_records(kargs, (ChainLdsChar*)smem, tile, ntiles, Mp);
  }
  chain_head_bwd_reduce<H>(Q.hd, tile, ntiles);
}

__global__ __launch_bounds__(1024) void lstm_chain_bwd_kernel(ChainBArgs A) {
  const int nblk = gridDim.x;
  __shared__ __attribute__((aligned(16))) char smem[CHAINB_LDS];
  const int s = blockIdx.x / A.nt8, tile = blockIdx.x % A.nt8;
  if (s == A.ns && A.t4.on && tile < A.ntiles) {
    if (threadIdx.x == 0) A.trace[2 * blockIdx.x] = (long long)__builtin_amdgcn_s_memrealtime();
    const unsigned tagb = chain_tag_base((unsigned)__hip_atomic_load(A.ctl, __ATOMIC_RELAXED, __HIP_MEMORY_SCOPE_AGENT));
    chain_t4_bwd_stage(A.t4, (const ChainBKernArgs*)__builtin_amdgcn_kernarg_segment_ptr(), tile, A.ntiles, A.Mp, tagb,
                       smem, blockIdx.x < 64 ? A.trace + 512 + blockIdx.x : nullptr);
    __syncthreads();
    if (threadIdx.x == 0) A.trace[2 * blockIdx.x + 1] = (long long)__builtin_amdgcn_s_memrealtime();
    chain_finish(A.ctl, nblk);
    return;
  }
  if (s >= A.ns || tile >= A.ntiles) {
    chain_finish(A.ctl, nblk);
    return;
  }
  if (threadIdx.x == 0) A.trace[2 * blockIdx.x] = (long long)__builtin_amdgcn_s_memrealtime();
  const unsigned E = (unsigned)__hip_atomic_load(A.ctl, __ATOMIC_RELAXED, __HIP_MEMORY_SCOPE_AGENT);
  const unsigned tagb = chain_tag_base(E);
  const ChainBStage S = A.st[s];
  const int H = S.H, KX = S.KX;
  const bool src = s > 0 || A.t4.on;
#define GQ_CHAINB_STAGE_16(KXX, DD, SRCV, UPV, XOV) chain_bwd_stage16<KXX, DD, SRCV, UPV, XOV>
#define GQ_CHAINB_STAGE_32(KXX, DD, SRCV, UPV, XOV) chain_bwd_stage_sk<32, KXX, DD, SRCV, UPV, XOV>
#define GQ_CHAINB_STAGE_64(KXX, DD, SRCV, UPV, XOV) chain_bwd_stage_sk<64, KXX, DD, SRCV, UPV, XOV>
#define GQ_CHAINB_BODY3(HH, KXX, DD, SRCV, UPV, XOV)                                    \
  {                                                                                     \
    if (threadIdx.x >= chainb_live_threads(HH, TMC<HH>::NT)) return;                    \
    GQ_CHAINB_STAGE_##HH(KXX, DD, SRCV, UPV, XOV)(S, tile, A.ntiles, A.Mp, tagb, A.ctl, smem); \
  }
#define GQ_CHAINB_BODY2(HH, KXX, DD, SRCV, UPV)                                         \
  if (!SRCV || S.sout) GQ_CHAINB_BODY3(HH, KXX, DD, SRCV, UPV, true)                    \
  else GQ_CHAINB_BODY3(HH, KXX, DD, SRCV, UPV, false)
#define GQ_CHAINB_BODY(HH, KXX, DD)                                                     \
  {                                                                                     \
    if (src) { if (S.P > 0 && !S.punp) { GQ_CHAINB_BODY2(HH, KXX, DD, true, true) }    \
               else { GQ_CHAINB_BODY2(HH, KXX, DD, true, false) } }                     \
    else { if (S.P > 0) { GQ_CHAINB_BODY3(HH, KXX, DD, false, true, true) }             \
           else { GQ_CHAINB_BODY3(HH, KXX, DD, false, false, true) } }                  \
  }
  if (H == 16) { if (KX == 1) GQ_CHAINB_BODY(16, 1, CHAINB_D16) else GQ_CHAINB_BODY(16, 2, CHAINB_D16) }
  else if (H == 32) { if (KX == 1) GQ_CHAINB_BODY(32, 1, CHAINB_D32) else GQ_CHAINB_BODY(32, 2, CHAINB_D32) }
  else { if (KX == 1) GQ_CHAINB_BODY(64, 1, CHAINB_D64) else GQ_CHAINB_BODY(64, 2, CHAINB_D64) }
#undef GQ_CHAINB_BODY
#undef GQ_CHAINB_BODY2
#undef GQ_CHAINB_BODY3
#undef GQ_CHAINB_STAGE_16
#undef GQ_CHAINB_STAGE_32
#undef GQ_CHAINB_STAGE_64
  __syncthreads();
  if (threadIdx.x == 0) A.trace[2 * blockIdx.x + 1] = (long long)__builtin_amdgcn_s_memrealtime();
  chain_finish(A.ctl, nblk);
}

static long long* chain_trace_buf(int dev) {
  static long long* tr[64] = {nullptr};
  if (!tr[dev]) TORCH_CHECK(hipMalloc(&tr[dev], 3 * 256 * sizeof(long long)) == hipSuccess,
                            "lstm_chain: trace");
  return tr[dev];
}

static long long* chain_prof_buf(int dev);
static void chain_prof_clear(int dev) {
  long long* pb = chain_prof_buf(dev);
  if (pb != nullptr)
    TORCH_CHECK(hipMemsetAsync(pb, 0, CHAIN_MAX * CHAIN_PROF_STEPS * 8 * sizeof(long long), stream()) == hipSuccess,
                "chain prof clear");
}
static long long* chain_prof_buf(int dev) {
#ifdef GQ_CHAIN_PROF
  static const bool on = [] {
    const char* e = std::getenv("GNNQC_CHAIN_PROF");
    return e != nullptr && e[0] == '1';
  }();
#else
  const bool on = false;
#endif
  if (!on) return nullptr;
  static long long* pb[64] = {nullptr};
  if (!pb[dev]) {
    TORCH_CHECK(hipMalloc(&pb[dev], CHAIN_MAX * CHAIN_PROF_STEPS * 8 * sizeof(long long)) == hipSuccess, "chain prof");
    TORCH_CHECK(hipMemset(pb[dev], 0, CHAIN_MAX * CHAIN_PROF_STEPS * 8 * sizeof(long long)) == hipSuccess, "chain prof");
  }
  return pb[dev];
}

at::Tensor lstm_chain_prof(const at::Tensor& like) {
  c10::DeviceGuard guard(like.device());
  long long* p = chain_prof_buf(like.get_device());
  TORCH_CHECK(p != nullptr, "lstm_chain_prof: build with GNNQC_CHAIN_PROF_BUILD=1 and set GNNQC_CHAIN_PROF=1 "
                            "before the first chain launch");
  at::Tensor o = at::empty({CHAIN_MAX, CHAIN_PROF_STEPS, 8}, like.options().dtype(at::kLong));
  TORCH_CHECK(hipMemcpyAsync(o.data_ptr<int64_t>(), p, o.numel() * sizeof(long long), hipMemcpyDeviceToDevice,
                             stream()) == hipSuccess, "lstm_chain_prof");
  return o;
}

int* chain_ctl(int dev) {
  static int* ctl[64] = {nullptr};
  TORCH_CHECK(dev >= 0 && dev < 64, "lstm_chain: device index");
  if (!ctl[dev]) {
    hipStreamCaptureStatus cs;
    TORCH_CHECK(hipStreamIsCapturing(stream(), &cs) == hipSuccess && cs == hipStreamCaptureStatusNone,
                "lstm_chain: first use must not be inside a graph capture");
    int* p = nullptr;
    TORCH_CHECK(hipMalloc(&p, 16 * sizeof(int)) == hipSuccess, "lstm_chain: control word allocation");
    const int init[16] = {1, 0};
    TORCH_CHECK(hipMemcpy(p, init, sizeof(init), hipMemcpyHostToDevice) == hipSuccess, "lstm_chain: init");
    ctl[dev] = p;
  }
  return ctl[dev];
}

static int chain_capacity(int dev) {
  static int cap[64] = {0};
  TORCH_CHECK(dev >= 0 && dev < 64, "lstm_chain: device index");
  if (cap[dev] == 0) {
    hipDeviceProp_t prop;
    TORCH_CHECK(hipGetDeviceProperties(&prop, dev) == hipSuccess, "lstm_chain: device properties");
    int occ = 1 << 30;
    const void* kernels[] = {reinterpret_cast<const void*>(&lstm_chain_fwd_kernel<true>),
                             reinterpret_cast<const void*>(&lstm_chain_fwd_kernel<false>),
                             reinterpret_cast<const void*>(&lstm_chain_bwd_kernel)};
    for (const void* k : kernels) {
      int n = 0;
      TORCH_CHECK(hipOccupancyMaxActiveBlocksPerMultiprocessor(&n, k, 1024, 0) == hipSuccess,
                  "lstm_chain: occupancy query");
      occ = std::min(occ, n);
    }
    cap[dev] = std::max(0, occ) * prop.multiProcessorCount;
  }
  return cap[dev];
}

int64_t lstm_chain_capacity(const at::Tensor& like) {
  TORCH_CHECK(like.is_cuda(), "lstm_chain_capacity: a GPU tensor names the device");
  return chain_capacity(like.get_device());
}

at::Tensor lstm_chain_ctl(const at::Tensor& like) {
  TORCH_CHECK(like.is_cuda(), "lstm_chain_ctl: a GPU tensor names the device");
  c10::DeviceGuard guard(like.device());
  int* p = chain_ctl(like.get_device());
  return at::from_blob(p, {16}, like.options().dtype(at::kInt));
}

struct T4Host {
  const at::Tensor* b;
  at::TensorList head;
  const at::Tensor* y;
  const at::Tensor* mask;
  int64_t M;
  double alpha1, alpha2, w0, w1;
  at::Tensor sums, hist;
};

void t4_head_fwd_args(ChainHead& hd, at::TensorList head, const at::Tensor& y, const at::Tensor& mask, int64_t M,
                      int Mp, double alpha1, double alpha2, double w0, double w1, const at::Tensor& sums,
                      const at::Tensor& hist, at::Tensor& logits, at::Tensor& loss, at::Tensor& part);

static std::vector<at::Tensor> chain_fwd_impl(const at::Tensor& x, at::TensorList W, at::TensorList U,
                                              at::TensorList b, at::IntArrayRef pool, bool train, const at::Tensor* pkW,
                                              const at::Tensor* pkU, const T4Host* t4 = nullptr);

std::vector<at::Tensor> lstm_chain_fwd(const at::Tensor& x, at::TensorList W, at::TensorList U, at::TensorList b,
                                       at::IntArrayRef pool, bool train) {
  return chain_fwd_impl(x, W, U, b, pool, train, nullptr, nullptr);
}

std::vector<at::Tensor> lstm_chain_fwd_pack(const at::Tensor& x, at::TensorList W, at::TensorList U,
                                            at::TensorList b, at::IntArrayRef pool, bool train, const at::Tensor& Wt4,
                                            const at::Tensor& Ut4) {
  return chain_fwd_impl(x, W, U, b, pool, train, &Wt4, &Ut4);
}

std::vector<at::Tensor> lstm_chain_head_fwd(const at::Tensor& x, at::TensorList W, at::TensorList U, at::TensorList b,
                                            at::IntArrayRef pool, bool train, const at::Tensor& Wt4,
                                            const at::Tensor& Ut4, const at::Tensor& bt4, at::TensorList head,
                                            const at::Tensor& y, const at::Tensor& mask, int64_t M, double alpha1,
                                            double alpha2, double w0, double w1, at::Tensor sums, at::Tensor hist) {
  T4Host h4{&bt4, head, &y, &mask, M, alpha1, alpha2, w0, w1, sums, hist};
  return chain_fwd_impl(x, W, U, b, pool, train, &Wt4, &Ut4, &h4);
}

static std::vector<at::Tensor> chain_fwd_impl(const at::Tensor& x, at::TensorList W, at::TensorList U,
                                              at::TensorList b, at::IntArrayRef pool, bool train, const at::Tensor* pkW,
                                              const at::Tensor* pkU, const T4Host* t4) {
  check_f32_cuda(x, "x");
  const int ns = (int)W.size();
  TORCH_CHECK(ns >= 1 && ns <= CHAIN_MAX && (int)U.size() == ns && (int)b.size() == ns && (int)pool.size() == ns,
              "lstm_chain: stage lists");
  TORCH_CHECK(x.dim() == 3 && x.is_contiguous(), "lstm_chain: x must be a contiguous [T, Mp, Din]");
  const int Mp = (int)x.size(1);
  TORCH_CHECK(Mp % 16 == 0, "lstm_chain: Mp must be a multiple of 16");
  const int ntiles = Mp / 16, nt8 = (ntiles + 7) / 8 * 8;
  TORCH_CHECK(ns * nt8 <= chain_capacity(x.get_device()), "lstm_chain: ", ns * nt8,
              " workgroups cannot all be resident on this device");
  TORCH_CHECK(x.size(2) % 4 == 0 && reinterpret_cast<uintptr_t>(x.data_ptr()) % 16 == 0,
              "lstm_chain: x channels must be float4 granules");
  c10::DeviceGuard guard(x.device());
  auto opt = x.options();
  ChainArgs A{};
  A.ns = ns;
  A.ntiles = ntiles;
  A.nt8 = nt8;
  A.Mp = Mp;
  A.ctl = chain_ctl(x.get_device());
  A.trace = chain_trace_buf(x.get_device());
  chain_prof_clear(x.get_device());
  std::vector<at::Tensor> out;
  at::Tensor prev_stream;
  int T = (int)x.size(0), Din = (int)x.size(2);
  for (int s = 0; s < ns; ++s) {
    for (const at::Tensor* t : {&W[s], &U[s], &b[s]}) check_f32_cuda(*t, "lstm_chain weight");
    const int H = (int)U[s].size(0), Dw = (int)W[s].size(0);
    TORCH_CHECK(H == 16 || H == 32 || H == 64, "lstm_chain: hidden size ", H);
    TORCH_CHECK(W[s].size(1) == 4 * H && U[s].size(1) == 4 * H && b[s].numel() == 4 * H, "lstm_chain: weights");
    TORCH_CHECK(Dw <= Din && Din <= 64 && (s == 0 || Din <= H), "lstm_chain: stage ", s, " input width ", Din);
    TORCH_CHECK(T >= 1 && T < 4096, "lstm_chain: sequence length");
    const int P = (int)pool[s];
    const bool last = s + 1 == ns && t4 == nullptr;
    TORCH_CHECK(last || P == 0 || P == 3, "lstm_chain: pools between stages must be 3 (got ", P, ")");
    TORCH_CHECK(t4 == nullptr || s + 1 < ns || P == 3, "lstm_chain_head_fwd: the last chain stage must pool by 3");
    ChainStage& S = A.st[s];
    S.x = s == 0 ? x.data_ptr<float>() : nullptr;
    S.xin = s == 0 ? nullptr : reinterpret_cast<const unsigned long long*>(prev_stream.data_ptr<int64_t>());
    S.W = W[s].data_ptr<float>();
    S.U = U[s].data_ptr<float>();
    S.b = b[s].data_ptr<float>();
    at::Tensor h = at::empty({T + 1, Mp, H}, opt);
    at::Tensor g = train ? at::empty({T + 1, Mp, H, 4}, opt.dtype(at::kBFloat16)) : at::empty({0}, opt);
    at::Tensor c = train ? at::empty({T + 1, Mp, H}, opt) : at::empty({0}, opt);
    at::Tensor pooled, pidx;
    const TmPool pl = tm_pool_outputs(P, T, Mp, H, opt, pooled, pidx);
    const int To = P > 0 ? T / P : T;
    TORCH_CHECK(To >= 1, "lstm_chain: pooled length");
    at::Tensor so = !last ? at::empty({T, Mp, H}, opt.dtype(at::kLong)) : at::Tensor();
    S.h = h.data_ptr<float>();
    S.g = train ? bf16_ptr(g) : nullptr;
    S.c = train ? c.data_ptr<float>() : nullptr;
    S.sout = so.defined() ? reinterpret_cast<unsigned long long*>(so.data_ptr<int64_t>()) : nullptr;
    S.pout = last ? pl.out : nullptr;
    S.iout = last ? pl.idx : nullptr;
    S.P = last ? P : 0;
    if (!last && P > 0 && s + 1 < ns) {
      A.st[s + 1].pin_out = pooled.data_ptr<float>();
      A.st[s + 1].pin_idx = pidx.data_ptr<uint8_t>();
    } else if (!last && P > 0) {
      A.t4.pin_out = pooled.data_ptr<float>();
      A.t4.pin_idx = pidx.data_ptr<uint8_t>();
    }
    S.H = H;
    S.T = T;
    S.Din = Din;
    S.Dw = Dw;
    S.KX = (Din + 31) / 32;
    S.PIN = s > 0 ? std::max(1, (int)pool[s - 1]) : 1;
    TORCH_CHECK(H < 64 || 16 * Din / (s == 0 ? 4 : 2) <= 64 * TMC<64>::NW, "lstm_chain: stage ", s, " input tile");
    TORCH_CHECK(s == 0 || (long)T * Mp * Din * 8 < (1L << 31), "lstm_chain: stage ", s, " input stream too large");
    TORCH_CHECK(s == 0 || Din % 2 == 0, "lstm_chain: stage ", s, " input width must be even");
    TORCH_CHECK(s > 0 || Din % 4 == 0, "lstm_chain: the input width must be a multiple of 4");
    {
      long long* pb = chain_prof_buf(x.get_device());
      S.prof = pb != nullptr ? pb + (size_t)s * CHAIN_PROF_STEPS * 8 : nullptr;
    }
    out.insert(out.end(), {h.narrow(0, 0, T), g, c, pooled, pidx});
    if (so.defined()) out.push_back(so);
    prev_stream = so;
    T = To;
    Din = H;
  }
  int nblk = ns * nt8;
  std::vector<at::Tensor> t4out;
  at::Tensor hb_t;
  if (t4 != nullptr) {
    TORCH_CHECK(pkW != nullptr && pkU != nullptr, "lstm_chain_head_fwd: time4 weights");
    check_f32_cuda(*t4->b, "bt4");
    const int Dw4 = (int)pkW->size(0);
    TORCH_CHECK(T >= 1 && T <= 16, "lstm_chain_head_fwd: time4 sequence length 1..16 (got ", T, ")");
    TORCH_CHECK(Din <= 64 && Dw4 >= 1 && Dw4 <= Din && t4->b->numel() == 512, "lstm_chain_head_fwd: time4 input width");
    ChainT4& Q = A.t4;
    Q.on = 1;
    Q.xin = reinterpret_cast<const unsigned long long*>(prev_stream.data_ptr<int64_t>());
    Q.W = pkW->data_ptr<float>();
    Q.U = pkU->data_ptr<float>();
    Q.b = t4->b->data_ptr<float>();
    at::Tensor h4 = at::empty({T, Mp, 128}, opt);
    at::Tensor g4 = train ? at::empty({(long)T * Mp * 128 * 4}, opt) : at::empty({0}, opt);
    at::Tensor c4 = train ? at::empty({(long)T * Mp * 128 * 2}, opt) : at::empty({0}, opt);
    Q.h = h4.data_ptr<float>();
    Q.g = train ? g4.data_ptr<float>() : nullptr;
    Q.c = train ? c4.data_ptr<float>() : nullptr;
    Q.T = T;
    Q.Din = Din;
    Q.Dw = Dw4;
    at::Tensor logits, loss, part;
    t4_head_fwd_args(Q.hd, t4->head, *t4->y, *t4->mask, t4->M, Mp, t4->alpha1, t4->alpha2, t4->w0, t4->w1, t4->sums,
                     t4->hist, logits, loss, part);
    t4out = {h4, g4, c4, logits, loss, part};
    const char* hbe = std::getenv("GNNQC_HEAD_BWD_IN_FWD");
    if (train && !(hbe != nullptr && hbe[0] == '0')) {
      hb_t = at::empty({(long)ntiles * 16 * 128}, opt);
      Q.hb = hb_t.data_ptr<float>();
    } else {
      hb_t = at::empty({0}, opt);
    }
    nblk += nt8;
  }
  at::Tensor pk;
  if (pkW != nullptr) {
    check_f32_cuda(*pkW, "Wt4");
    check_f32_cuda(*pkU, "Ut4");
    TORCH_CHECK(pkU->size(0) == 128 && pkU->size(1) == 512 && pkW->size(1) == 512 && pkW->size(0) <= 64,
                "lstm_chain_fwd_pack: time4 weights must be [<=64, 512] and [128, 512]");
    pk = at::empty({(long)T4PK_ALL * 4}, opt);
    A.pkU = pkU->data_ptr<float>();
    A.pkW = pkW->data_ptr<float>();
    A.pkDw = (int)pkW->size(0);
    A.pk = reinterpret_cast<bf16x8_t*>(pk.data_ptr<float>());
    A.npk = (T4PK_ALL + 1023) / 1024;
    nblk += A.npk;
    TORCH_CHECK(nblk <= chain_capacity(x.get_device()), "lstm_chain: ", nblk,
                " workgroups cannot all be resident on this device");
  }
  std::vector<at::Tensor> gp_keep;
  {
    const int dev = x.get_device();
    const GcnProdJob& P = gcn_pending(dev).prod;
    if (P.on) {
      const int H0 = A.st[0].H, Din0 = A.st[0].Din;
      const bool mine = train && t4 != nullptr && P.out == x.data_ptr<float>() && P.Mp == Mp &&
                        P.Cp == Din0 && P.D.T == (int)x.size(0) && Din0 % 2 == 0 &&
                        (H0 < 64 || 16 * Din0 / 2 <= 64 * TMC<64>::NW) &&
                        (long)P.D.T * Mp * Din0 * 8 < (1L << 31) && nblk + P.Mp <= chain_capacity(dev);
      if (mine) {
        static_assert(GcnProdLds::BYTES <= CHAIN_LDS, "GCN producer LDS");
        gcn_prod_take(dev, A.gp, gp_keep);
        A.st[0].xin = A.gp.gout;
        nblk += A.gp.Mp;
      } else {
        gcn_prod_flush_dev(dev);
      }
    }
  }
  std::vector<at::Tensor> cf_keep;
  if (gcn_pending(x.get_device()).job.on && train &&
      nblk + gcn_pending(x.get_device()).job.Mp <= chain_capacity(x.get_device())) {
    static_assert(GcnCoefFwdLds::BYTES <= CHAIN_LDS, "coefficient job LDS");
    gcn_coef_take(x.get_device(), A.cf, cf_keep);
    nblk += A.cf.Mp;
  }
  if (train)
    hipLaunchKernelGGL(lstm_chain_fwd_kernel<true>, dim3(nblk), dim3(1024), 0, stream(), A);
  else
    hipLaunchKernelGGL(lstm_chain_fwd_kernel<false>, dim3(nblk), dim3(1024), 0, stream(), A);
  GQ_LAUNCH_CHECK();
  std::vector<at::Tensor> res;
  for (auto& t : out)
    if (t.scalar_type() != at::kLong) res.push_back(t);
  if (pk.defined()) res.push_back(pk);
  if (hb_t.defined()) res.push_back(hb_t);
  for (int i = 0; i < 5 && i < (int)t4out.size(); ++i) res.push_back(t4out[i]);
  return res;
}

static std::vector<at::Tensor> chain_bwd_setup(ChainBArgs& A, std::vector<at::Tensor>& keep, const at::Tensor& dh,
                                               at::TensorList g, at::TensorList c, at::TensorList W, at::TensorList U,
                                               at::TensorList pidx, at::IntArrayRef pool, at::IntArrayRef x_width,
                                               at::IntArrayRef T_in, int extra_blocks);

std::vector<at::Tensor> lstm_chain_bwd(const at::Tensor& dh, at::TensorList g, at::TensorList c, at::TensorList W,
                                       at::TensorList U, at::TensorList pidx, at::IntArrayRef pool,
                                       at::IntArrayRef x_width, at::IntArrayRef T_in) {
  ChainBArgs A{};
  std::vector<at::Tensor> keep;
  auto res = chain_bwd_setup(A, keep, dh, g, c, W, U, pidx, pool, x_width, T_in, 0);
  hipLaunchKernelGGL(lstm_chain_bwd_kernel, dim3(A.ns * A.nt8), dim3(1024), 0, stream(), A);
  GQ_LAUNCH_CHECK();
  return res;
}

void t4_head_bwd_args(ChainHead& hd, at::TensorList head, const at::Tensor& y, const at::Tensor& mask, int64_t M,
                      int Mp, double alpha1, double alpha2, double w0, double w1, const at::Tensor& dloss,
                      at::TensorList hgrads, at::Tensor& gpart);

std::vector<at::Tensor> lstm_chain_head_bwd(const at::Tensor& dloss, const at::Tensor& x4, const at::Tensor& h4,
                                            const at::Tensor& g4, const at::Tensor& c4, const at::Tensor& Wt4,
                                            const at::Tensor& Ut4, const at::Tensor& pk, const at::Tensor& hb,
                                            at::TensorList head, const at::Tensor& y,
                                            const at::Tensor& mask, int64_t M, double alpha1, double alpha2, double w0,
                                            double w1, at::TensorList hgrads, at::TensorList g, at::TensorList c,
                                            at::TensorList W, at::TensorList U, at::TensorList pidx,
                                            at::IntArrayRef pool, at::IntArrayRef x_width, at::IntArrayRef T_in) {
  check_f32_cuda(x4, "x4");
  for (const at::Tensor* t : {&dloss, &h4, &g4, &c4, &Wt4, &Ut4}) check_f32_cuda(*t, "lstm_chain_head_bwd operand");
  TORCH_CHECK(x4.dim() == 3 && x4.is_contiguous(), "lstm_chain_head_bwd: x4 must be a contiguous [T4, Mp, Din]");
  const int T4 = (int)x4.size(0), Mp = (int)x4.size(1), Din = (int)x4.size(2), Dw = (int)Wt4.size(0);
  TORCH_CHECK(T4 >= 1 && T4 <= 16 && Din <= 64 && Dw >= 1 && Dw <= Din && Wt4.size(1) == 512 && Ut4.size(0) == 128 &&
                  Ut4.size(1) == 512, "lstm_chain_head_bwd: time4 shapes");
  TORCH_CHECK(dloss.numel() == 1, "lstm_chain_head_bwd: dloss must be a scalar");
  TORCH_CHECK(h4.numel() == (long)T4 * Mp * 128 && g4.numel() == (long)T4 * Mp * 128 * 4 && c4.numel() == (long)T4 * Mp * 128 * 2,
              "lstm_chain_head_bwd: time4 saved state shapes");
  TORCH_CHECK(pool.size() >= 1 && pool[0] == 3, "lstm_chain_head_bwd: the top chain stage must pool by 3");
  ChainBArgs A{};
  std::vector<at::Tensor> keep;
  c10::DeviceGuard guard(x4.device());
  auto opt = x4.options();
  at::Tensor so = at::empty({T4, Mp, Din}, opt.dtype(at::kLong));
  auto res = chain_bwd_setup(A, keep, x4, g, c, W, U, pidx, pool, x_width, T_in, (Mp / 16 + 7) / 8 * 8);
  A.st[0].dh = nullptr;
  A.st[0].din = reinterpret_cast<const unsigned long long*>(so.data_ptr<int64_t>());
  ChainT4B& Q = A.t4;
  Q.on = 1;
  Q.h = h4.data_ptr<float>();
  Q.g = g4.data_ptr<float>();
  Q.c = c4.data_ptr<float>();
  TORCH_CHECK(pk.is_cuda() && pk.is_contiguous() && pk.nbytes() == (size_t)T4PK_ALL * 16,
              "lstm_chain_head_bwd: pk must be the forward's full fragment image");
  Q.pk = reinterpret_cast<const bf16x8_t*>(pk.data_ptr());
  if (hb.numel() > 0) {
    check_f32_cuda(hb, "lstm_chain_head_bwd hb");
    TORCH_CHECK(hb.numel() == (long)(Mp / 16) * 16 * 128, "lstm_chain_head_bwd: hb must be the forward's dh tiles");
    Q.hb = hb.data_ptr<float>();
  } else {
    Q.hb = nullptr;
  }
  at::Tensor dz4 = at::empty({T4 + 1, Mp, 512}, opt.dtype(at::kBFloat16));
  Q.dz = bf16_ptr(dz4);
  Q.sout = reinterpret_cast<unsigned long long*>(so.data_ptr<int64_t>());
  Q.T = T4;
  Q.Din = Din;
  Q.Dw = Dw;
  at::Tensor gpart;
  t4_head_bwd_args(Q.hd, head, y, mask, M, Mp, alpha1, alpha2, w0, w1, dloss, hgrads, gpart);
  hipLaunchKernelGGL(lstm_chain_bwd_kernel, dim3((A.ns + 1) * A.nt8), dim3(1024), 0, stream(), A);
  GQ_LAUNCH_CHECK();
  res.insert(res.begin(), dz4);
  return res;
}

static std::vector<at::Tensor> chain_bwd_setup(ChainBArgs& A, std::vector<at::Tensor>& keep, const at::Tensor& dh,
                                               at::TensorList g, at::TensorList c, at::TensorList W, at::TensorList U,
                                               at::TensorList pidx, at::IntArrayRef pool, at::IntArrayRef x_width,
                                               at::IntArrayRef T_in, int extra_blocks) {
  check_f32_cuda(dh, "dh");
  const int ns = (int)W.size();
  TORCH_CHECK(ns >= 1 && ns <= CHAIN_MAX && (int)U.size() == ns && (int)g.size() == ns && (int)c.size() == ns &&
                  (int)pidx.size() == ns && (int)pool.size() == ns && (int)x_width.size() == ns &&
                  (int)T_in.size() == ns, "lstm_chain_bwd: stage lists");
  TORCH_CHECK(dh.dim() == 3 && dh.is_contiguous(), "lstm_chain_bwd: dh must be a contiguous [Ts, Mp, H]");
  const int Mp = (int)dh.size(1);
  TORCH_CHECK(Mp % 16 == 0, "lstm_chain_bwd: Mp");
  const int ntiles = Mp / 16, nt8 = (ntiles + 7) / 8 * 8;
  TORCH_CHECK(ns * nt8 + extra_blocks <= chain_capacity(dh.get_device()), "lstm_chain_bwd: ", ns * nt8 + extra_blocks,
              " workgroups cannot all be resident on this device");
  c10::DeviceGuard guard(dh.device());
  auto opt = dh.options();
  A.ns = ns;
  A.ntiles = ntiles;
  A.nt8 = nt8;
  A.Mp = Mp;
  A.ctl = chain_ctl(dh.get_device());
  A.trace = chain_trace_buf(dh.get_device());
  chain_prof_clear(dh.get_device());
  std::vector<at::Tensor> dzs;
  at::Tensor dx, prev;
  for (int s = 0; s < ns; ++s) {
    const int H = (int)U[s].size(0), Dw = (int)W[s].size(0), T = (int)T_in[s], Din = (int)x_width[s];
    const int P = (int)pool[s];
    TORCH_CHECK(H == 16 || H == 32 || H == 64, "lstm_chain_bwd: hidden size ", H);
    TORCH_CHECK(Dw <= Din && Din <= 64 && Din % 4 == 0 && T >= 1 && T < 4096, "lstm_chain_bwd: stage ", s, " shape");
    for (const at::Tensor* t : {&c[s], &W[s], &U[s]}) check_f32_cuda(*t, "lstm_chain_bwd operand");
    check_gates_cuda(g[s]);
    TORCH_CHECK(g[s].numel() == (long)(T + 1) * Mp * H * 4 && c[s].numel() == (long)(T + 1) * Mp * H,
                "lstm_chain_bwd: saved state shapes");
    TORCH_CHECK(H != 16 || (long)(T + 1) * Mp * H * 8 < (1L << 32), "lstm_chain_bwd: stage ", s, " state too large");
    const int Ts = P > 0 ? T / P : T;
    if (s == 0) {
      TORCH_CHECK(dh.size(0) == Ts && dh.size(2) == H, "lstm_chain_bwd: dh shape");
    } else {
      TORCH_CHECK((int)x_width[s - 1] == H, "lstm_chain_bwd: stage ", s, " output width");
      TORCH_CHECK((int)T_in[s - 1] == Ts, "lstm_chain_bwd: lengths");
    }
    if (P > 0) {
      TORCH_CHECK(pidx[s].numel() == (long)Ts * Mp * H && pidx[s].scalar_type() == at::kByte,
                  "lstm_chain_bwd: argmax bytes");
    }
    ChainBStage& S = A.st[s];
    S.dh = s == 0 ? dh.data_ptr<float>() : nullptr;
    S.din = s == 0 ? nullptr : reinterpret_cast<const unsigned long long*>(prev.data_ptr<int64_t>());
    S.pidx = P > 0 ? pidx[s].data_ptr<uint8_t>() : nullptr;
    S.g = bf16_ptr(g[s]);
    S.c = c[s].data_ptr<float>();
    S.W = W[s].data_ptr<float>();
    S.U = U[s].data_ptr<float>();
    at::Tensor dz = at::empty({T + 1, Mp, 4 * H}, opt.dtype(at::kBFloat16));
    S.dz = bf16_ptr(dz);
    dzs.push_back(dz);
    const bool last = s + 1 == ns && ns > 1;
    if (!last) {
      at::Tensor so = at::empty({T + 1, Mp, Din}, opt.dtype(at::kLong));
      S.sout = reinterpret_cast<unsigned long long*>(so.data_ptr<int64_t>());
      S.dx = nullptr;
      keep.push_back(so);
      prev = so;
    } else {
      dx = at::empty({T + 1, Mp, Din}, opt);
      S.sout = nullptr;
      S.dx = dx.data_ptr<float>();
    }
    S.H = H;
    S.T = T;
    S.Din = Din;
    S.Dw = Dw;
    S.KX = (Din + 31) / 32;
    S.P = P;
    S.Ts = Ts;
    S.trace_mid = A.trace + 512;
    {
      long long* pb = chain_prof_buf(dh.get_device());
      S.prof = pb != nullptr ? pb + (size_t)s * CHAIN_PROF_STEPS * 8 : nullptr;
    }
  }
  dzs.push_back(dx.defined() ? dx.narrow(0, 0, (int)T_in[ns - 1]) : at::empty({0}, opt));
  return dzs;
}

at::Tensor lstm_chain_status(const at::Tensor& like) {
  c10::DeviceGuard guard(like.device());
  int* p = chain_ctl(like.get_device());
  at::Tensor o = at::empty({12}, like.options().dtype(at::kInt));
  TORCH_CHECK(hipMemcpyAsync(o.data_ptr<int>(), p, 12 * sizeof(int), hipMemcpyDeviceToDevice, stream()) == hipSuccess,
              "lstm_chain_status");
  return o;
}

at::Tensor lstm_chain_trace(const at::Tensor& like) {
  c10::DeviceGuard guard(like.device());
  long long* p = chain_trace_buf(like.get_device());
  at::Tensor o = at::empty({3 * 256}, like.options().dtype(at::kLong));
  TORCH_CHECK(hipMemcpyAsync(o.data_ptr<int64_t>(), p, o.numel() * sizeof(long long), hipMemcpyDeviceToDevice,
                             stream()) == hipSuccess, "lstm_chain_trace");
  return o;
}

}

TORCH_LIBRARY_IMPL(gnnqc, CUDA, m) {
  m.impl("lstm_chain_fwd", &gq::lstm_chain_fwd);
  m.impl("lstm_chain_fwd_pack", &gq::lstm_chain_fwd_pack);
  m.impl("lstm_chain_head_fwd", &gq::lstm_chain_head_fwd);
  m.impl("lstm_chain_status", &gq::lstm_chain_status);
  m.impl("lstm_chain_capacity", &gq::lstm_chain_capacity);
  m.impl("lstm_chain_ctl", &gq::lstm_chain_ctl);
  m.impl("lstm_chain_trace", &gq::lstm_chain_trace);
  m.impl("lstm_chain_prof", &gq::lstm_chain_prof);
  m.impl("lstm_chain_bwd", &gq::lstm_chain_bwd);
  m.impl("lstm_chain_head_bwd", &gq::lstm_chain_head_bwd);
}
```

csrc/kernels/lstm_grads_jobs.hip:

```cpp
#include "common.h"

#include <cstdlib>
#include "gcn_fused.h"
#include "lstm_grads_body.h"
#include "lstm_tm_bwd_body.h"
#include "lstm_tm_common.h"

namespace gq {

template <int HR, int HG, int DT>
__global__ __launch_bounds__(TMC<HR>::NT) void lstm_tm_bwd_dual_kernel(
    const float* __restrict__ dh, const __bf16* __restrict__ g, const float* __restrict__ c,
    const float* __restrict__ W, const float* __restrict__ U, __bf16* __restrict__ dz, int Mp, int T, int Dw,
    int ntiles, GradJob gj, RedJob rj) {
  constexpr int D = HR >= 64 ? 2 : 4;
  const int b = blockIdx.x;
  if (b < ntiles) {
    lstm_tm_bwd_body<HR, 1, 1, D, true, false, false>(dh, g, c, W, U, nullptr, dz, Mp, T, Dw, Dw, b, ntiles);
    return;
  }
  if (threadIdx.x >= 256) return;
  const int gb = b - ntiles;
  if (gb < gj.nblocks) {
    if constexpr (HG > 0)
      {
      __shared__ __attribute__((aligned(16))) char gsm[GradsLds<HG, DT>::BYTES];
      lstm_grads_body<HG, DT, 4>(gj.dz, gj.x, gj.h, gj.W, nullptr, gj.ws, gj.rows, gj.period, gj.hshift, gj.Din,
                                 gj.ldx, 0, gj.Din, gj.xg, gj.x_elems, gb % gj.ncb, gb / gj.ncb, gj.ncb, gj.splits, gsm);
    }
    return;
  }
  const int rb = gb - gj.nblocks;
  if (rb < rj.nblocks) {
    if (rj.kb > 1)
      lstm_grads_reduce_multi<PIPE_RED_KB>(rj.ws, rj.splits, rj.RC, rj.ncb, rj.DT, rj.HT, rj.Din, rj.H, rj.dW, rj.db,
                                           rj.dU, rb, rj.nf);
    else
      lstm_grads_reduce_body(rj.ws, rj.splits, rj.RC, nullptr, rj.ncb, rj.DT, rj.HT, rj.Din, rj.H, rj.dW, rj.db,
                             rj.dU, rb, 0, 1, rj.nf);
  }
}

static constexpr int MULTI_MAX = 12;
struct MultiGrad {
  GradJob j[MULTI_MAX];
  int start[MULTI_MAX + 1];
  int key[MULTI_MAX];
  int n;
  int gcn_nb;
  GcnBwdJob gcn;
  int gcn_coef;
  GcnCoefJob gcnc;
};
struct MultiRed {
  RedJob j[MULTI_MAX];
  int start[MULTI_MAX + 1];
  int n;
  int* nf;
};

__global__ __launch_bounds__(256) void lstm_grads_multi_kernel(MultiGrad M) {
  __shared__ __attribute__((aligned(16))) char smem[GradsLds<128, 5>::BYTES];
  static_assert(GcnBwdLds<2, 16>::BYTES <= GradsLds<128, 5>::BYTES, "GCN job LDS");
  if ((int)blockIdx.x < M.gcn_nb) {
    const int gb = blockIdx.x;
    if (M.gcn_coef) gcn_coef_bwd_body<2, 16>(M.gcnc, gb);
    else if (M.gcn.key == 2 * 64 + 16)
      gcn_fused_bwd_body<2, 16>(M.gcn, gb % M.gcn.B, gb / M.gcn.B, smem);
    return;
  }
  const int b = blockIdx.x - M.gcn_nb;
  int k = 0;
  while (k + 1 < M.n && b >= M.start[k + 1]) ++k;
  const GradJob gj = M.j[k];
  const int gb = b - M.start[k];
#define GQ_MG(HG, DT)                                                                                    \
  case HG * 8 + DT:                                                                                      \
    lstm_grads_body<HG, DT, 4>(gj.dz, gj.x, gj.h, gj.W, nullptr, gj.ws, gj.rows, gj.period, gj.hshift, gj.Din, \
                               gj.ldx, 0, gj.Din, gj.xg, gj.x_elems, gb % gj.ncb, gb / gj.ncb, gj.ncb, gj.splits, \
                               smem);                                                                    \
    break;
#define GQ_MG_H(HG) GQ_MG(HG, 1) GQ_MG(HG, 2) GQ_MG(HG, 3) GQ_MG(HG, 4) GQ_MG(HG, 5)
  switch (M.key[k]) {
    GQ_MG_H(16) GQ_MG_H(32) GQ_MG_H(64) GQ_MG_H(128)
    default: break;
  }
#undef GQ_MG_H
#undef GQ_MG
}

__global__ __launch_bounds__(256) void lstm_grads_reduce_multi_kernel(MultiRed M) {
  const int b = blockIdx.x;
  int k = 0;
  while (k + 1 < M.n && b >= M.start[k + 1]) ++k;
  const RedJob rj = M.j[k];
  if (rj.kb > 1)
    lstm_grads_reduce_multi<PIPE_RED_KB>(rj.ws, rj.splits, rj.RC, rj.ncb, rj.DT, rj.HT, rj.Din, rj.H, rj.dW, rj.db,
                                         rj.dU, b - M.start[k], M.nf);
  else
    lstm_grads_reduce_body(rj.ws, rj.splits, rj.RC, nullptr, rj.ncb, rj.DT, rj.HT, rj.Din, rj.H, rj.dW, rj.db,
                           rj.dU, b - M.start[k], 0, 1, M.nf);
}

at::Tensor lstm_grads_job_ws(const at::Tensor& dz, const at::Tensor& x, const at::Tensor& W, int64_t H) {
  check_f32_cuda(W, "W");
  const GradsGeom geo((int)H, (int)W.size(0));
  const long rows = x.numel() / x.size(-1);
  const long ntiles = (rows + 31) / 32;
  static const int tps = [] {
    const char* e = std::getenv("GNNQC_GRADS_TPS");
    return e != nullptr ? std::max(1, std::atoi(e)) : 4;
  }();
  const int splits = (int)std::max<long>(1, std::min<long>({(ntiles + tps - 1) / tps, (long)std::max(64, 2048 / geo.ncb),
                                                            (long)PIPE_MAX_SPLITS}));
  c10::DeviceGuard guard(x.device());
  return at::empty({(long)splits * geo.RC}, x.options());
}

static bool grads_job_ok(const at::Tensor& x, int Dw) {
  const int ldx = (int)x.stride(-2);
  return ldx % 4 == 0 && ldx >= Dw && ldx <= 144 && reinterpret_cast<uintptr_t>(x.data_ptr()) % 16 == 0 &&
         GradsGeom::din_tiles(Dw) <= 5 && x.stride(-1) == 1;
}

at::Tensor lstm_tm_bwd_pipe(const at::Tensor& dh, const at::Tensor& g, const at::Tensor& c, const at::Tensor& W,
                            const at::Tensor& U, int64_t T, const at::Tensor& gz, const at::Tensor& gx,
                            const at::Tensor& gh, const at::Tensor& gW, int64_t g_period, int64_t g_hshift,
                            const at::Tensor& gws, const at::Tensor& rws, const at::Tensor& rW, at::Tensor rdW,
                            at::Tensor rdU, at::Tensor rdb) {
  const bool rec = dh.numel() > 0, job = gz.numel() > 0, red = rws.numel() > 0;
  const at::Tensor& ref = rec ? dh : (job ? gz : rws);
  c10::DeviceGuard guard(ref.device());
  int HR = 16, Mp = 0, ntiles = 0, Dw = 1;
  at::Tensor dz = at::empty({0}, ref.options());
  if (rec) {
    for (const at::Tensor* t : {&dh, &c, &W, &U}) check_f32_cuda(*t, "lstm_tm_bwd_pipe operand");
    check_gates_cuda(g);
    HR = (int)U.size(0);
    Mp = (int)dh.size(1);
    TORCH_CHECK(dh.dim() == 3 && dh.size(0) == T && dh.size(2) == HR && Mp % 16 == 0, "lstm_tm_bwd_pipe: dh shape");
    TORCH_CHECK(g.numel() == (long)(T + 1) * Mp * HR * 4 && c.numel() == (long)(T + 1) * Mp * HR,
                "lstm_tm_bwd_pipe: saved state shapes");
    TORCH_CHECK(HR == 16 || HR == 32 || HR == 64, "lstm_tm_bwd_pipe: hidden size");
    ntiles = Mp / 16;
    Dw = (int)W.size(0);
    dz = at::empty({T + 1, Mp, 4 * HR}, dh.options().dtype(at::kBFloat16));
  }
  GradJob gj{};
  at::Tensor gz_b;
  int HG = 0, DTG = 1;
  if (job) {
    check_dz_cuda(gz);
    for (const at::Tensor* t : {&gh, &gW, &gws}) check_f32_cuda(*t, "lstm_tm_bwd_pipe job operand");
    gz_b = job_dz(gz);
    TORCH_CHECK(gx.is_cuda() && gx.scalar_type() == at::kFloat, "lstm_tm_bwd_pipe: job x");
    HG = (int)gW.size(1) / 4;
    TORCH_CHECK(grads_job_ok(gx, (int)gW.size(0)), "lstm_tm_bwd_pipe: job x layout");
    DTG = GradsGeom::din_tiles((int)gW.size(0));
    gj = make_grad_job(gz_b, gx, gh, gW, g_period, g_hshift, gws, "lstm_tm_bwd_pipe: job workspace size");
  }
  RedJob rj{};
  if (red) {
    for (const at::Tensor* t : {&rws, &rW}) check_f32_cuda(*t, "lstm_tm_bwd_pipe reduce operand");
    for (at::Tensor* t : {&rdW, &rdU, &rdb}) check_f32_cuda(*t, "lstm_tm_bwd_pipe reduce gradient");
    const int H = (int)rW.size(1) / 4, Din = (int)rW.size(0);
    const int splits = GradsGeom(H, Din).job_splits(rws, "lstm_tm_bwd_pipe: reduce workspace size");
    TORCH_CHECK(rdW.numel() == rW.numel() && rdU.numel() == (long)H * 4 * H && rdb.numel() == 4 * H,
                "lstm_tm_bwd_pipe: reduce gradient buffers");
    rj = make_red_job(rws.data_ptr<float>(), H, Din, splits, rdW.data_ptr<float>(), rdU.data_ptr<float>(),
                      rdb.data_ptr<float>(), chain_ctl(rws.get_device()) + 7);
  }
  const int nblk = ntiles + gj.nblocks + rj.nblocks;
  if (nblk == 0) return dz;
  TORCH_CHECK(!job || HG == HR || HG == 2 * HR || !rec, "lstm_tm_bwd_pipe: job hidden size must be H or 2H of the rec");
  const __bf16* gp = rec ? bf16_ptr(g) : nullptr;
  const float* dhp = rec ? dh.data_ptr<float>() : nullptr;
  const float* cp = rec ? c.data_ptr<float>() : nullptr;
  const float* Wp = rec ? W.data_ptr<float>() : nullptr;
  const float* Up = rec ? U.data_ptr<float>() : nullptr;
  __bf16* dzp = rec ? bf16_ptr(dz) : nullptr;
  auto st = stream();
  const int HL = rec ? HR : (HG <= 32 ? 16 : HG / 2);
  dispatch_int<16, 32, 64>(HL, "lstm_tm_bwd_pipe: job hidden size", [&](auto hrc) {
    dispatch_int<0, 1, 2>(job ? HG / HL : 0, "lstm_tm_bwd_pipe: job hidden size", [&](auto kc) {
      dispatch_int<1, 2, 3, 4, 5>(DTG, "lstm_tm_bwd_pipe: job x layout", [&](auto dtc) {
        constexpr int HRV = decltype(hrc)::value, HGV = decltype(kc)::value * HRV, DTV = decltype(dtc)::value;
        if constexpr (HGV == 0 && DTV != 1) {
          TORCH_CHECK(false, "lstm_tm_bwd_pipe: no job, no din tiles");
        } else
          hipLaunchKernelGGL((lstm_tm_bwd_dual_kernel<HRV, HGV, DTV>), dim3(nblk), dim3(TMC<HRV>::NT), 0, st, dhp, gp,
                             cp, Wp, Up, dzp, Mp, (int)T, Dw, ntiles, gj, rj);
      });
    });
  });
  GQ_LAUNCH_CHECK();
  return dz;
}

void lstm_grads_multi(at::TensorList gz, at::TensorList gx, at::TensorList gh, at::TensorList gW,
                      at::IntArrayRef period, at::IntArrayRef hshift, at::TensorList gws, at::TensorList rws,
                      at::TensorList rW, at::TensorList rdW, at::TensorList rdU, at::TensorList rdb,
                      at::TensorList gcn_t, at::IntArrayRef gcn_i) {
  const int ng = (int)gz.size(), nr = (int)rws.size();
  TORCH_CHECK(ng <= MULTI_MAX && nr <= MULTI_MAX && (int)gx.size() == ng && (int)gh.size() == ng &&
                  (int)gW.size() == ng && (int)period.size() == ng && (int)hshift.size() == ng &&
                  (int)gws.size() == ng && (int)rW.size() == nr && (int)rdW.size() == nr && (int)rdU.size() == nr &&
                  (int)rdb.size() == nr, "lstm_grads_multi: job lists");
  TORCH_CHECK((gcn_t.size() == 0 && gcn_i.size() == 0) || (gcn_t.size() == 21 && gcn_i.size() == 4) ||
                  (gcn_t.size() == 10 && gcn_i.size() == 1), "lstm_grads_multi: gcn job lists");
  TORCH_CHECK(gcn_t.size() == 0 || ng > 0, "lstm_grads_multi: a GCN job rides on a gradient launch");
  if (ng + nr == 0) return;
  c10::DeviceGuard guard(ng ? gz[0].device() : rws[0].device());
  auto st = stream();
  if (ng) {
    MultiGrad M{};
    M.n = ng;
    if (gcn_t.size() == 10) {
      M.gcnc = gcn_coef_job(gcn_t[0], gcn_i[0], gcn_t[1], gcn_t[2], gcn_t[3], gcn_t[4], gcn_t[5], gcn_t[6], gcn_t[7],
                            gcn_t[8], gcn_t[9]);
      M.gcn_coef = 1;
      M.gcn_nb = M.gcnc.nblocks;
    } else if (gcn_t.size() > 0) {
      const c10::optional<at::Tensor> cur = gcn_t[11].numel() > 0 ? c10::optional<at::Tensor>(gcn_t[11]) : c10::nullopt;
      M.gcn = gcn_bwd_job(gcn_t[0], gcn_i[0], gcn_t[1], gcn_t[2], gcn_t[3], gcn_t[4], gcn_t[5], gcn_t[6], gcn_t[7],
                          gcn_t[8], gcn_t[9], gcn_t[10], cur, gcn_i[1], gcn_i[2], gcn_i[3] != 0, gcn_t[12], gcn_t[13],
                          gcn_t[14], gcn_t[15], gcn_t[16], gcn_t[17], gcn_t[18], gcn_t[19], gcn_t[20], M.gcn_nb);
      TORCH_CHECK(M.gcn.key == 2 * 64 + 16, "lstm_grads_multi: the GCN job takes 2 input / 16 output channels");
    }
    int nb = 0;
    std::vector<at::Tensor> zb(ng);
    for (int k = 0; k < ng; ++k) {
      check_dz_cuda(gz[k]);
      zb[k] = job_dz(gz[k]);
      for (const at::Tensor* t : {&gh[k], &gW[k], &gws[k]}) check_f32_cuda(*t, "lstm_grads_multi operand");
      TORCH_CHECK(gx[k].is_cuda() && gx[k].scalar_type() == at::kFloat, "lstm_grads_multi: x");
      const int HG = (int)gW[k].size(1) / 4, Dw = (int)gW[k].size(0);
      TORCH_CHECK(HG == 16 || HG == 32 || HG == 64 || HG == 128, "lstm_grads_multi: hidden size");
      TORCH_CHECK(grads_job_ok(gx[k], Dw), "lstm_grads_multi: x layout");
      M.j[k] = make_grad_job(zb[k], gx[k], gh[k], gW[k], period[k], hshift[k], gws[k], "lstm_grads_multi: workspace size");
      M.key[k] = HG * 8 + GradsGeom::din_tiles(Dw);
      M.start[k] = nb;
      nb += M.j[k].nblocks;
    }
    M.start[ng] = nb;
    hipLaunchKernelGGL(lstm_grads_multi_kernel, dim3(M.gcn_nb + nb), dim3(256), 0, st, M);
    GQ_LAUNCH_CHECK();
  }
  if (nr) {
    MultiRed R{};
    R.n = nr;
    R.nf = chain_ctl(rws[0].get_device()) + 7;
    int nb = 0;
    for (int k = 0; k < nr; ++k) {
      const int H = (int)rW[k].size(1) / 4, Din = (int)rW[k].size(0);
      const int splits = GradsGeom(H, Din).job_splits(rws[k], "lstm_grads_multi: reduce workspace size");
      TORCH_CHECK(rdW[k].numel() == rW[k].numel() && rdU[k].numel() == (long)H * 4 * H && rdb[k].numel() == 4 * H,
                  "lstm_grads_multi: gradient buffers");
      R.j[k] = make_red_job(rws[k].data_ptr<float>(), H, Din, splits, rdW[k].data_ptr<float>(), rdU[k].data_ptr<float>(),
                            rdb[k].data_ptr<float>(), nullptr);
      R.start[k] = nb;
      nb += R.j[k].nblocks;
    }
    R.start[nr] = nb;
    hipLaunchKernelGGL(lstm_grads_reduce_multi_kernel, dim3(nb), dim3(256), 0, st, R);
    GQ_LAUNCH_CHECK();
  }
}

bool lstm_defer_reduce(bool flag) {
  const bool old = defer_reduce_mode();
  defer_reduce_mode() = flag;
  return old;
}

int64_t lstm_reduce_flush() {
  auto& q = deferred_reds();
  const int n = (int)q.size();
  for (int k0 = 0; k0 < n; k0 += MULTI_MAX) {
    const int kn = std::min(MULTI_MAX, n - k0);
    MultiRed R{};
    R.n = kn;
    R.nf = chain_ctl(c10::hip::current_device()) + 7;
    int nb = 0;
    for (int k = 0; k < kn; ++k) {
      const DeferredRed& d = q[k0 + k];
      TORCH_CHECK(d.ws.numel() >= (long)d.splits * GradsGeom(d.H, d.Din).RC, "lstm_reduce_flush: workspace size");
      R.j[k] = make_red_job(d.ws.data_ptr<float>(), d.H, d.Din, d.splits, d.dW, d.dU, d.db, nullptr);
      R.start[k] = nb;
      nb += R.j[k].nblocks;
    }
    R.start[kn] = nb;
    c10::DeviceGuard guard(q[k0].ws.device());
    hipLaunchKernelGGL(lstm_grads_reduce_multi_kernel, dim3(nb), dim3(256), 0, stream(), R);
    GQ_LAUNCH_CHECK();
  }
  q.clear();
  return n;
}

at::Tensor lstm_tm_grads(const at::Tensor& dz, const at::Tensor& x, const at::Tensor& h, const at::Tensor& W,
                         at::Tensor dW, at::Tensor dU, at::Tensor db, bool need_dx) {
  check_dz_cuda(dz);
  for (const at::Tensor* t : {&x, &h, &W}) check_f32_cuda(*t, "lstm_tm_grads operand");
  for (const at::Tensor* t : {&dW, &dU, &db}) check_f32_cuda(*t, "lstm_tm_grads gradient");
  const int T = (int)x.size(0), Mp = (int)x.size(1), Din = (int)x.size(2), H = (int)h.size(2);
  const int Dw = (int)W.size(0);
  TORCH_CHECK(dz.size(0) >= T && dz.size(1) == Mp && dz.size(2) == 4 * H && h.size(0) == T && h.size(1) == Mp,
              "lstm_tm_grads: shapes");
  TORCH_CHECK(Dw <= Din && dW.numel() == (long)Dw * 4 * H && dU.numel() == (long)H * 4 * H && db.numel() == 4 * H,
              "lstm_tm_grads: gradient buffer shapes");
  c10::DeviceGuard guard(x.device());
  const long rows = (long)T * Mp;
  const int ncb = lstm_grads_col_blocks(H);
  at::Tensor dx = need_dx ? at::empty({ncb, T, Mp, Din}, x.options()) : at::empty({0}, x.options());
  lstm_grads_rows(dz.data_ptr(), dz_bf16(dz), x.data_ptr<float>(), h.data_ptr<float>(), W.data_ptr<float>(),
                  need_dx ? dx.data_ptr<float>() : nullptr, dW.data_ptr<float>(), dU.data_ptr<float>(),
                  db.data_ptr<float>(), rows, rows, Mp, H, Dw, Din, rows * Din, Din, rows * Din, stream());
  if (!need_dx) return dx;
  return ncb == 1 ? dx[0] : dx.sum(0);
}

}

TORCH_LIBRARY_IMPL(gnnqc, CUDA, m) {
  m.impl("lstm_tm_grads", &gq::lstm_tm_grads);
  m.impl("lstm_tm_bwd_pipe", &gq::lstm_tm_bwd_pipe);
  m.impl("lstm_grads_job_ws", &gq::lstm_grads_job_ws);
  m.impl("lstm_grads_multi", &gq::lstm_grads_multi);
}
```

csrc/kernels/registry.hip:

```cpp
#include <ATen/ATen.h>
#include <torch/library.h>

#include "common.h"

namespace gq {
bool lstm_defer_reduce(bool flag);
int64_t lstm_reduce_flush();
static bool set_deterministic(bool flag) {
  const bool old = deterministic_mode();
  deterministic_mode() = flag;
  return old;
}
}

TORCH_LIBRARY(gnnqc, m) {
  m.def("set_deterministic(bool flag) -> bool", &gq::set_deterministic);
  m.def("lstm_defer_reduce(bool flag) -> bool", &gq::lstm_defer_reduce);
  m.def("lstm_reduce_flush() -> int", &gq::lstm_reduce_flush);
  m.def("lstm_fwd(Tensor x, Tensor W, Tensor U, Tensor b, bool train, bool bf16) -> Tensor[]");
  m.def("lstm_bwd(Tensor dh, Tensor gates, Tensor cseq, Tensor U, bool bf16) -> Tensor");
  m.def("lstm_grads(Tensor dz, Tensor x, Tensor hseq, Tensor W, Tensor(a!) dW, Tensor(b!) dU, Tensor(c!) db, "
        "bool need_dx) -> Tensor");
  m.def("lstm_tm_fwd(Tensor x, Tensor W, Tensor U, Tensor b, bool train, bool store_gates=True) -> Tensor[]");
  m.def("lstm_tm2_fwd(Tensor x, Tensor WA, Tensor UA, Tensor bA, Tensor WB, Tensor UB, Tensor bB, "
        "bool train, bool store_gates=True, int pool=0) -> Tensor[]");
  m.def("lstm_tm_grads(Tensor dz, Tensor x, Tensor h, Tensor W, Tensor(a!) dW, Tensor(b!) dU, Tensor(c!) db, "
        "bool need_dx) -> Tensor");
  m.def("lstm_dx(Tensor dz, Tensor W, Tensor like) -> Tensor");
  m.def("lstm_chain_fwd(Tensor x, Tensor[] W, Tensor[] U, Tensor[] b, int[] pool, bool train) -> Tensor[]");
  m.def("lstm_chain_fwd_pack(Tensor x, Tensor[] W, Tensor[] U, Tensor[] b, int[] pool, bool train, Tensor Wt4, "
        "Tensor Ut4) -> Tensor[]");
  m.def("lstm_chain_head_fwd(Tensor x, Tensor[] W, Tensor[] U, Tensor[] b, int[] pool, bool train, Tensor Wt4, "
        "Tensor Ut4, Tensor bt4, Tensor[] head, Tensor y, Tensor mask, int M, float alpha1, float alpha2, float w0, "
        "float w1, Tensor(a!) sums, Tensor(b!) hist) -> Tensor[]");
  m.def("lstm_chain_status(Tensor like) -> Tensor");
  m.def("lstm_chain_capacity(Tensor like) -> int");
  m.def("lstm_chain_ctl(Tensor like) -> Tensor");
  m.def("lstm_grads_multi(Tensor[] gz, Tensor[] gx, Tensor[] gh, Tensor[] gW, int[] period, int[] hshift, "
        "Tensor[] gws, Tensor[] rws, Tensor[] rW, Tensor(a!)[] rdW, Tensor(b!)[] rdU, Tensor(c!)[] rdb, "
        "Tensor[] gcn_t, int[] gcn_i) -> ()");
  m.def("lstm_chain_trace(Tensor like) -> Tensor");
  m.def("lstm_chain_prof(Tensor like) -> Tensor");
  m.def("lstm_chain_bwd(Tensor dh, Tensor[] g, Tensor[] c, Tensor[] W, Tensor[] U, Tensor[] pidx, int[] pool, "
        "int[] x_width, int[] T_in) -> Tensor[]");
  m.def("lstm_chain_head_bwd(Tensor dloss, Tensor x4, Tensor h4, Tensor g4, Tensor c4, Tensor Wt4, Tensor Ut4, "
        "Tensor pk, Tensor hb, Tensor[] head, Tensor y, Tensor mask, int M, float alpha1, float alpha2, float w0, float w1, "
        "Tensor(a!)[] hgrads, Tensor[] g, Tensor[] c, Tensor[] W, Tensor[] U, Tensor[] pidx, int[] pool, "
        "int[] x_width, int[] T_in) -> Tensor[]");
  m.def("time4_head_fwd(Tensor x, Tensor W, Tensor U, Tensor b, Tensor pk, bool train, Tensor[] head, Tensor y, Tensor mask, "
        "int M, float alpha1, float alpha2, float w0, float w1, Tensor(a!) sums, Tensor(b!) hist) -> Tensor[]");
  m.def("time4_head_bwd(Tensor dloss, Tensor x, Tensor h, Tensor g, Tensor c, Tensor W, Tensor U, Tensor pk, Tensor[] head, "
        "Tensor y, Tensor mask, int M, float alpha1, float alpha2, float w0, float w1, Tensor(a!)[] hgrads) -> Tensor[]");
  m.def("time4_trace(Tensor like) -> Tensor");
  m.def("time4_fwd(Tensor x, Tensor W, Tensor U, Tensor b, bool train, bool all_h, int max_blocks=0) -> Tensor[]");
  m.def("time4_bwd(Tensor dh, Tensor x, Tensor g, Tensor c, Tensor W, Tensor U, bool need_dz, int max_blocks=0, "
        "Tensor? row_scale=None) -> Tensor[]");
  m.def("time4_prob_fwd(Tensor x, Tensor W, Tensor U, Tensor b, Tensor[] head, float alpha1, float alpha2, int M, "
        "bool train, int max_blocks=0) -> Tensor[]");
  m.def("lstm_tm_bwd_pipe(Tensor dh, Tensor g, Tensor c, Tensor W, Tensor U, int T, Tensor gz, Tensor gx, "
        "Tensor gh, Tensor gW, int g_period, int g_hshift, Tensor gws, Tensor rws, Tensor rW, Tensor(a!) rdW, "
        "Tensor(b!) rdU, Tensor(c!) rdb) -> Tensor");
  m.def("lstm_grads_job_ws(Tensor dz, Tensor x, Tensor W, int H) -> Tensor");
  m.def("lstm_tm_bwd(Tensor dh, Tensor g, Tensor c, Tensor x, Tensor h, Tensor W, Tensor U, Tensor b, Tensor(a!) dW, "
        "Tensor(b!) dU, Tensor(c!) db, bool need_dx, Tensor? pidx=None, int pool=0) -> Tensor");
  m.def("gcn_stats(Tensor x, Tensor mask) -> Tensor");
  m.def("gcn_pool_fwd(Tensor x, Tensor w, Tensor anom, Tensor W, Tensor b, Tensor scale, Tensor shift, "
        "Tensor alpha, int Mp=0, int Cp=0) -> Tensor");
  m.def("gcn_pool_bwd(Tensor x, Tensor w, Tensor dout, Tensor W, Tensor b, Tensor scale, Tensor shift, "
        "Tensor alpha, int c_off, bool time_major=False) -> Tensor");
  m.def("gcn_pool_bwd_input(Tensor x, Tensor w, Tensor mask, Tensor dout, Tensor W, Tensor b, Tensor scale, "
        "Tensor shift, Tensor alpha, Tensor dzcoef, int c_off, bool time_major=False) -> Tensor");
  m.def("gcn_window_prep(Tensor series, Tensor shift, Tensor scale, Tensor win_group, Tensor win_center, "
        "Tensor win_valid, Tensor group_adj, Tensor group_anom_pos, int tb, int seq_len, bool time_norm, "
        "bool agg_mean, int pool) -> Tensor[]");
  m.def("gcn_fused_fwd(Tensor series, Tensor shift, Tensor scale, Tensor win_group, Tensor win_center, "
        "Tensor win_valid, Tensor win_label, Tensor group_anom_pos, Tensor mom, Tensor pw, Tensor wids, "
        "Tensor table, Tensor? cursor, int tb, int seq_len, bool time_norm, Tensor W, Tensor b, Tensor gamma, "
        "Tensor beta, Tensor alpha, Tensor(a!) rmean, Tensor(b!) rvar, bool training, float momentum, float eps, "
        "int Mp, int Cp, bool with_coef=False, bool defer=False) -> Tensor[]");
  m.def("gcn_fused_bwd(Tensor dh, int c_off, Tensor series, Tensor shift, Tensor scale, Tensor win_group, "
        "Tensor win_center, Tensor win_valid, Tensor group_anom_pos, Tensor pw, Tensor wids, Tensor table, "
        "Tensor? cursor, int tb, int seq_len, bool time_norm, Tensor S, Tensor st, Tensor W, Tensor b, "
        "Tensor alpha, Tensor(a!) dW, Tensor(b!) dgamma, Tensor(c!) dbeta, Tensor(d!) dalpha) -> ()");
  m.def("gcn_coef_flush(Tensor like) -> bool");
  m.def("gcn_prod_flush(Tensor like) -> bool");
  m.def("gcn_coef_bwd(Tensor dh, int c_off, Tensor coef, Tensor S, Tensor st, Tensor W, Tensor b, Tensor(a!) dW, "
        "Tensor(b!) dgamma, Tensor(c!) dbeta, Tensor(d!) dalpha) -> ()");
  m.def("gcn_adj_bits(Tensor adj, bool agg_mean) -> Tensor[]");
  m.def("gcn_node_fwd(Tensor x, Tensor bits, Tensor rs, Tensor mask, Tensor W, Tensor b, Tensor scale, "
        "Tensor shift, Tensor alpha, int Mp, int Cp) -> Tensor");
  m.def("gcn_node_bwd(Tensor x, Tensor bitsT, Tensor rs, Tensor mask, Tensor dout, Tensor W, Tensor b, "
        "Tensor scale, Tensor shift, Tensor alpha) -> Tensor");
  m.def("gcn_node_bwd_input(Tensor x, Tensor bitsT, Tensor rs, Tensor mask, Tensor dout, Tensor W, Tensor b, "
        "Tensor scale, Tensor shift, Tensor alpha, Tensor coef) -> Tensor");
  m.def("gcn_pool_weights(Tensor adj, Tensor mask, Tensor anom_pos, bool agg_mean, int pool) -> Tensor");
  m.def("gcn_bn_prep(Tensor S, Tensor W, Tensor b, Tensor gamma, Tensor beta, Tensor(a!) rmean, Tensor(b!) rvar, "
        "bool training, float momentum, float eps) -> Tensor");
  m.def("gcn_prep(Tensor x, Tensor adj, Tensor mask, Tensor anom_pos, bool agg_mean, int pool, Tensor W, Tensor b, "
        "Tensor gamma, Tensor beta, Tensor(a!) rmean, Tensor(b!) rvar, bool training, float momentum, float eps) -> Tensor[]");
  m.def("gcn_bwd_finalize(Tensor acc, Tensor S, Tensor W, Tensor b, Tensor st, bool training, Tensor(a!) dW, "
        "Tensor(b!) db, Tensor(c!) dgamma, Tensor(d!) dbeta, Tensor(e!) dalpha) -> Tensor");
  m.def("conv1d_fwd(Tensor x, Tensor W, Tensor b, float alpha, bool gap, bool store_y) -> Tensor[]");
  m.def("conv1d_bwd(Tensor dy, Tensor y, Tensor x, Tensor W, float alpha, bool gap, Tensor(a!) dW, "
        "Tensor(b!) db, bool need_dx) -> Tensor");
  m.def("adam_step(Tensor(a!) p, Tensor(d!) g, Tensor(b!) m, Tensor(c!) v, Tensor lr, Tensor step, float beta1, "
        "float beta2, float eps, float grad_scale, float weight_decay, Tensor? guard=None, bool zero_grad=False) -> ()");
  m.def("adam_guarded(Tensor(a!) p, Tensor(d!) g, Tensor(b!) m, Tensor(c!) v, Tensor lr, Tensor(e!) step, float beta1, "
        "float beta2, float eps, float grad_scale, float weight_decay, Tensor(f!) state, Tensor(g!)? ext=None, "
        "Tensor(h!)? cursor=None, int cursor_mod=1) -> bool");
  m.def("adam_flagged(Tensor(a!) p, Tensor(d!) g, Tensor(b!) m, Tensor(c!) v, Tensor lr, Tensor(e!) step, float beta1, "
        "float beta2, float eps, float grad_scale, float weight_decay, Tensor(f!) state, Tensor(g!) ext, "
        "Tensor(h!)? cursor=None, int cursor_mod=1) -> ()");
  m.def("nonfinite_count(Tensor x) -> Tensor");
  m.def("ig_interp(Tensor v, Tensor alpha) -> Tensor");
  m.def("ig_gcn_pool_fwd(Tensor x, Tensor w, Tensor anom, Tensor W, Tensor b, Tensor scale, Tensor shift, "
        "Tensor alpha, Tensor alphas, int Cp) -> Tensor");
  m.def("ig_gcn_pool_bwd(Tensor x, Tensor w, Tensor mask, Tensor g, Tensor W, Tensor b, Tensor scale, Tensor shift, "
        "Tensor alpha, Tensor alphas, Tensor wts, Tensor(a!) acc_x, Tensor(b!) acc_a, bool overwrite=False) -> ()");
  m.def("ig_interp_base(Tensor v, Tensor b, Tensor alpha) -> Tensor");
  m.def("ig_gcn_pool_fwd_base(Tensor x, Tensor xb, Tensor w, Tensor anom, Tensor ab, Tensor W, Tensor b, Tensor scale, "
        "Tensor shift, Tensor alpha, Tensor alphas, int Cp) -> Tensor");
  m.def("ig_gcn_pool_bwd_base(Tensor x, Tensor xb, Tensor w, Tensor mask, Tensor g, Tensor W, Tensor b, Tensor scale, "
        "Tensor shift, Tensor alpha, Tensor alphas, Tensor wts, Tensor(a!) acc_x, Tensor(b!) acc_a, "
        "bool overwrite=False) -> ()");
  m.def("ig_accum(Tensor(a!) acc, Tensor g, Tensor w) -> ()");
  m.def("ig_finalize(Tensor acc, Tensor v, int mode) -> Tensor");
  m.def("chain_poison(Tensor(a!) g, Tensor ext) -> ()");
  m.def("grad_guard(Tensor g, Tensor(a!) state, Tensor(b!) step, Tensor(c!)? ext=None) -> ()");
  m.def("score_histogram(Tensor scores, Tensor labels, Tensor mask, int bins) -> Tensor");
  m.def("head_fwd(Tensor feat, Tensor W1, Tensor b1, Tensor W2, Tensor b2, Tensor W3, Tensor b3, Tensor y, "
        "Tensor mask, float alpha1, float alpha2, float w0, float w1, Tensor(a!) sums, Tensor(b!) hist) -> Tensor[]");
  m.def("head_bwd(Tensor feat, Tensor W1, Tensor W2, Tensor W3, Tensor z1, Tensor z2, Tensor logits, Tensor y, "
        "Tensor mask, float alpha1, float alpha2, float w0, float w1, Tensor gout, Tensor aux, Tensor(a!) dW1, "
        "Tensor(b!) db1, Tensor(c!) dW2, Tensor(d!) db2, Tensor(e!) dW3, Tensor(f!) db3, bool need_dfeat) -> Tensor");
  m.def("head_prob_fwd(Tensor feat, Tensor W1, Tensor b1, Tensor W2, Tensor b2, Tensor W3, Tensor b3, float alpha1, "
        "float alpha2) -> Tensor[]");
  m.def("head_prob_bwd(Tensor feat, Tensor W1, Tensor W2, Tensor W3, Tensor z1, Tensor z2, Tensor prob, "
        "float alpha1, float alpha2) -> Tensor");
  m.def("maxpool1d_fwd(Tensor x, int p) -> Tensor[]");
  m.def("maxpool1d_bwd(Tensor dy, Tensor idx, int T, int p) -> Tensor");
  m.def("window_gather(Tensor series, Tensor shift, Tensor scale, Tensor win_group, Tensor win_center, "
        "Tensor win_valid, Tensor wids, int tb, int seq_len, bool time_norm) -> Tensor");
  m.def("batch_meta(Tensor wids, Tensor win_group, Tensor win_valid, Tensor group_adj, Tensor group_anom_pos, "
        "Tensor win_label, Tensor win_label_valid, Tensor valid_sample, Tensor x) -> Tensor[]");
  m.def("batch_gather(Tensor series, Tensor shift, Tensor scale, Tensor win_group, Tensor win_center, "
        "Tensor win_valid, Tensor wids, Tensor table, Tensor? cursor, Tensor group_adj, Tensor group_anom_pos, "
        "Tensor win_label, Tensor win_label_valid, Tensor valid_sample, int tb, int seq_len, bool time_norm) -> Tensor[]");
  m.def("series_tm_gather(Tensor series, Tensor shift, Tensor scale, Tensor win_group, Tensor win_center, "
        "Tensor win_valid, Tensor win_label, Tensor group_anom_pos, Tensor wids, Tensor table, Tensor? cursor, "
        "int tb, int seq_len, bool time_norm) -> Tensor[]");
  m.def("predict_emit(Tensor vals, bool logits, Tensor y, Tensor mask, Tensor wid, Tensor(a!) p_out, Tensor(b!) y_out, "
        "Tensor(c!) mask_out, Tensor(d!) wid_out, Tensor(e!) cursor) -> ()");
}
```

gnnqc/ops/lstm.py:

```python
from __future__ import annotations

import contextlib
from typing import Optional

import torch

_ACT = {
    "tanh": torch.tanh,
    "relu": torch.relu,
    "sigmoid": torch.sigmoid,
    "linear": lambda x: x,
    None: lambda x: x,
}


def lstm_eager(x: torch.Tensor, W: torch.Tensor, U: torch.Tensor, b: torch.Tensor,
               return_sequences: bool = True, activation: str = "tanh") -> torch.Tensor:
    from .lstm_ref import KernelLSTM, kernel_rounding_on
    if kernel_rounding_on() and activation == "tanh":
        return KernelLSTM.apply(x, W, U, b, bool(return_sequences), True)
    act = _ACT[activation]
    M, T, _ = x.shape
    H = U.shape[0]
    xp = torch.matmul(x, W) + b
    h = x.new_zeros(M, H)
    c = x.new_zeros(M, H)
    outs = []
    for t in range(T):
        z = xp[:, t] + h @ U
        i, f, g, o = z.split(H, dim=-1)
        i, f, o = torch.sigmoid(i), torch.sigmoid(f), torch.sigmoid(o)
        c = f * c + i * act(g)
        h = o * act(c)
        if return_sequences:
            outs.append(h)
    return torch.stack(outs, 1) if return_sequences else h


class _DirectGrad:

    enabled = False


class _Pipe:

    enabled = True
    job = None
    red = None
    batch = []
    gcn = None


PIPE_MAX_SEQ = 2048


_MULTI_MAX = 12


def _pipe_on(sinks, n_seq: int) -> bool:
    return _Pipe.enabled and _DirectGrad.enabled and all(d for _, d in sinks) and n_seq <= PIPE_MAX_SEQ


def _pipe_job(dz, x, h, W, sinks, period: int, hshift: int):
    from ..utils.native import hip_ops
    H = W.shape[1] // 4
    return dict(dz=dz, x=x, h=h, W=W, period=int(period), hshift=int(hshift),
                ws=hip_ops().lstm_grads_job_ws(dz, x, W, H), g=[s for s, _ in sinks])


def _pipe_launch(dh=None, g=None, c=None, W=None, U=None, T: int = 0, job=None, red=None):
    from ..utils.native import hip_ops
    ref = dh if dh is not None else (job or red)["dz"]
    e = ref.new_zeros(0)
    rec = (dh, g, c, W, U) if dh is not None else (e, e, e, e, e)
    jb = (job["dz"], job["x"], job["h"], job["W"], job["period"], job["hshift"], job["ws"]) if job else \
        (e, e, e, e, 1, 1, e)
    rd = (red["ws"], red["W"], *red["g"]) if red else (e, e, e, e, e)
    return hip_ops().lstm_tm_bwd_pipe(*rec, int(T), *jb, *rd)


def _pipe_drain_one():
    job, red = _Pipe.job, _Pipe.red
    if job is None and red is None:
        return
    _pipe_launch(job=job, red=red)
    _Pipe.job, _Pipe.red = None, job


def defer_to_grads_launch(gcn_lists) -> bool:
    import os
    if not (_DirectGrad.enabled and _Pipe.batch and _Pipe.gcn is None and os.environ.get("GNNQC_GCN_DEFER", "1") == "1"):
        return False
    _Pipe.gcn = gcn_lists
    return True


def pipe_flush():
    if _Pipe.batch:
        from ..utils.native import hip_ops
        grads = ([_Pipe.job] if _Pipe.job is not None else []) + _Pipe.batch
        reds = ([_Pipe.red] if _Pipe.red is not None else []) + grads
        gt, gi = _Pipe.gcn if _Pipe.gcn is not None else ([], [])
        hip_ops().lstm_grads_multi([j["dz"] for j in grads], [j["x"] for j in grads], [j["h"] for j in grads],
                                   [j["W"] for j in grads], [j["period"] for j in grads],
                                   [j["hshift"] for j in grads], [j["ws"] for j in grads],
                                   [r["ws"] for r in reds], [r["W"] for r in reds], [r["g"][0] for r in reds],
                                   [r["g"][1] for r in reds], [r["g"][2] for r in reds], gt, gi)
        _Pipe.job, _Pipe.red, _Pipe.batch, _Pipe.gcn = None, None, [], None
    while _Pipe.job is not None or _Pipe.red is not None:
        _pipe_drain_one()


def _pipe_push(job):
    if _Pipe.job is not None:
        _pipe_drain_one()
    _Pipe.job = job


def _pipe_tm_backward(dh, g, c, x, h, W, U, sinks, need_dx):
    from ..utils.native import hip_ops
    T, Mp = x.shape[0], x.shape[1]
    HR = U.shape[0]
    if dh.dim() == 2:
        dh = torch.nn.functional.pad(dh.unsqueeze(0), (0, 0, 0, 0, T - 1, 0))
    job, red = _Pipe.job, _Pipe.red
    if job is not None and job["W"].shape[1] // 4 not in (HR, 2 * HR):
        _pipe_drain_one()
        job, red = _Pipe.job, _Pipe.red
    dz = _pipe_launch(dh, g, c, W, U, T, job, red)
    _Pipe.job, _Pipe.red = None, job
    dx = hip_ops().lstm_dx(dz, W, x) if need_dx else None
    _pipe_push(_pipe_job(dz, x, h, W, sinks, T * Mp, Mp))
    return dx


def _pipe_x_ok(x: torch.Tensor, Dw: int) -> bool:
    return (x.stride(-1) == 1 and x.stride(-2) % 4 == 0 and x.data_ptr() % 16 == 0 and (Dw + 16) // 16 <= 5
            and x.shape[-1] % 4 == 0)


@contextlib.contextmanager
def _deferred_reduce(on: bool):
    import os
    if not (on and _DirectGrad.enabled and os.environ.get("GNNQC_DEFER_REDUCE", "1") == "1"):
        yield
        return
    from ..utils.native import hip_ops
    ops = hip_ops()
    prev = ops.lstm_defer_reduce(True)
    _Deferred.pending = True
    try:
        yield
    finally:
        ops.lstm_defer_reduce(prev)


class _Deferred:
    pending = False


@contextlib.contextmanager
def direct_grad_accumulation(flag: bool = True):
    prev = _DirectGrad.enabled
    _DirectGrad.enabled = flag
    try:
        yield
    finally:
        _DirectGrad.enabled = prev
        if _Pipe.job is not None or _Pipe.red is not None or _Pipe.batch:
            pipe_flush()
        _Pipe.gcn = None
        if _Deferred.pending:
            from ..utils.native import hip_ops
            _Deferred.pending = False
            hip_ops().lstm_reduce_flush()


class _Unflagged:
    count = 0


def unflagged_grad_writes() -> int:
    return _Unflagged.count


def _grad_sink(p: torch.Tensor):
    g = p.grad if _DirectGrad.enabled and isinstance(p, torch.nn.Parameter) else None
    if g is not None and g.is_contiguous() and g.dtype == torch.float32 and g.device == p.device:
        return g, True
    _Unflagged.count += 1
    return torch.zeros_like(p), False


class _HipLSTM(torch.autograd.Function):
    @staticmethod
    def forward(ctx, x, W, U, b, bf16: bool, return_sequences: bool):
        from ..utils.native import hip_ops
        ops = hip_ops()
        if not (x.stride(2) == 1 and x.stride(0) == x.shape[1] * x.stride(1)):
            x = x.clone(memory_format=torch.contiguous_format)
        need = any(ctx.needs_input_grad[:4])
        h, c, g = ops.lstm_fwd(x, W.contiguous(), U.contiguous(), b.contiguous(), need, bf16)
        ctx.bf16 = bf16
        ctx.return_sequences = return_sequences
        ctx.params = (W, U, b)
        if need:
            ctx.save_for_backward(x, W, U, h, c, g)
        return h if return_sequences else h[:, -1]

    @staticmethod
    def backward(ctx, dout):
        from ..utils.native import hip_ops
        ops = hip_ops()
        x, W, U, h, c, g = ctx.saved_tensors
        M, T, Din = x.shape
        H = U.shape[0]
        if ctx.return_sequences:
            dh = dout.contiguous()
        else:
            dh = torch.nn.functional.pad(dout.unsqueeze(1), (0, 0, T - 1, 0))
        dz = ops.lstm_bwd(dh, g, c, U.contiguous(), ctx.bf16)
        if not ctx.bf16:
            dz2 = dz.reshape(M * T, 4 * H)
            dx = (dz2 @ W.t()).view(M, T, Din) if ctx.needs_input_grad[0] else None
            dW = torch.einsum("mtd,mtg->dg", x, dz) if ctx.needs_input_grad[1] else None
            dU = None
            if ctx.needs_input_grad[2]:
                dU = torch.einsum("mth,mtg->hg", h[:, :-1], dz[:, 1:]) if T > 1 else torch.zeros_like(U)
            db = dz2.sum(0) if ctx.needs_input_grad[3] else None
            return dx, dW, dU, db, None, None
        if not any(ctx.needs_input_grad[1:4]):
            dx = None
            if ctx.needs_input_grad[0]:
                if Din % 4 == 0 and Din <= 128:
                    dx = ops.lstm_dx(dz, W.contiguous(), x)
                else:
                    dx = (dz.reshape(M * T, 4 * H).float() @ W.t()).view(M, T, Din)
            return dx, None, None, None, None, None
        Wp, Up, bp = ctx.params
        gW, dW_in = _grad_sink(Wp)
        gU, dU_in = _grad_sink(Up)
        gb, db_in = _grad_sink(bp)
        need_dx = bool(ctx.needs_input_grad[0])
        Wc = W.contiguous()
        if (dW_in and dU_in and db_in and _pipe_on(((gW, True),), M) and _pipe_x_ok(x, W.shape[0])):
            dx = ops.lstm_dx(dz, Wc, x) if need_dx else None
            _pipe_push(_pipe_job(dz, x, h, Wc, ((gW, True), (gU, True), (gb, True)), T, 1))
            return dx, None, None, None, None, None
        with _deferred_reduce(dW_in and dU_in and db_in):
            dx = ops.lstm_grads(dz, x, h, Wc, gW, gU, gb, need_dx)
        return (dx if need_dx else None,
                None if dW_in or not ctx.needs_input_grad[1] else gW,
                None if dU_in or not ctx.needs_input_grad[2] else gU,
                None if db_in or not ctx.needs_input_grad[3] else gb,
                None, None)


def _tm_layer_backward(dout, x, W, U, b, h, g, c, params, need_w, need_dx):
    from ..utils.native import hip_ops
    wgrad = any(need_w)
    if not wgrad and not need_dx:
        return None, [None, None, None]
    if wgrad:
        sinks = [_grad_sink(p) for p in params]
    else:
        e = x.new_zeros(0)
        sinks = [(e, True)] * 3
    Wc, Uc = W.contiguous(), U.contiguous()
    if wgrad and g.numel() > 0 and _pipe_on(sinks, x.shape[1]) and _pipe_x_ok(x, W.shape[0]):
        dx = _pipe_tm_backward(dout.contiguous(), g, c, x, h, Wc, Uc, sinks, need_dx)
    else:
        with _deferred_reduce(wgrad and all(d for _, d in sinks)):
            dx = hip_ops().lstm_tm_bwd(dout.contiguous(), g, c, x, h, Wc, Uc, b.contiguous(), sinks[0][0],
                                       sinks[1][0], sinks[2][0], need_dx)
    grads = [None if (direct or not n) else buf for (buf, direct), n in zip(sinks, need_w)]
    return (dx if need_dx else None), grads


class _HipLSTMChain(torch.autograd.Function):

    @staticmethod
    def forward(ctx, x, pools, *params):
        from ..utils.native import hip_ops
        ns = len(pools)
        Ws = [params[3 * i].contiguous() for i in range(ns)]
        Us = [params[3 * i + 1].contiguous() for i in range(ns)]
        bs = [params[3 * i + 2].contiguous() for i in range(ns)]
        need = any(ctx.needs_input_grad)
        outs = hip_ops().lstm_chain_fwd(x, Ws, Us, bs, [int(p) for p in pools], need)
        ctx.pools = tuple(int(p) for p in pools)
        ctx.params = params
        if need:
            ctx.save_for_backward(x, *Ws, *Us, *outs)
        last = outs[5 * (ns - 1):]
        return last[3] if pools[-1] else last[0]

    @staticmethod
    def backward(ctx, dout):
        from ..utils.native import hip_ops
        ops = hip_ops()
        pools = ctx.pools
        ns = len(pools)
        saved = ctx.saved_tensors
        x, Ws, Us, outs = saved[0], saved[1:1 + ns], saved[1 + ns:1 + 2 * ns], saved[1 + 2 * ns:]
        need = ctx.needs_input_grad
        grads = [None] * (3 * ns)
        dh = dout.contiguous()
        dx = None

        def layer_x(i):
            if i == 0:
                return x
            return outs[5 * (i - 1) + 3] if pools[i - 1] else outs[5 * (i - 1)]

        if _chain_bwd_on() and chain_fits(dh.shape[1], ns, dh.device) and all(layer_x(i).shape[-1] % 4 == 0 for i in range(ns)):
            order = list(reversed(range(ns)))
            e8 = x.new_zeros(0, dtype=torch.uint8)
            res = ops.lstm_chain_bwd(dh, [outs[5 * i + 1] for i in order], [outs[5 * i + 2] for i in order],
                                     [Ws[i] for i in order], [Us[i] for i in order],
                                     [outs[5 * i + 4] if pools[i] else e8 for i in order],
                                     [pools[i] for i in order], [layer_x(i).shape[-1] for i in order],
                                     [outs[5 * i].shape[0] for i in order])
            for k, i in enumerate(order):
                nw = need[2 + 3 * i:5 + 3 * i]
                if not any(nw):
                    continue
                h = outs[5 * i]
                xi = layer_x(i)
                sinks = [_grad_sink(p) for p in ctx.params[3 * i:3 * i + 3]]
                if (_pipe_on(sinks, h.shape[1]) and _pipe_x_ok(xi, Ws[i].shape[0])
                        and len(_Pipe.batch) < _MULTI_MAX - 2):
                    _Pipe.batch.append(_pipe_job(res[k], xi, h, Ws[i], sinks, h.shape[0] * h.shape[1], h.shape[1]))
                else:
                    ops.lstm_tm_grads(res[k], xi, h, Ws[i], sinks[0][0], sinks[1][0], sinks[2][0], False)
                grads[3 * i:3 * i + 3] = [None if (direct or not n) else buf for (buf, direct), n in zip(sinks, nw)]
            dx = res[ns]
            return (dx if need[0] else None, None, *grads)
        for i in reversed(range(ns)):
            h, g, c, _, idx = outs[5 * i:5 * i + 5]
            T, Mp, H = h.shape
            if pools[i]:
                dh = ops.maxpool1d_bwd(dh.view(1, -1, Mp * H), idx.view(1, -1, Mp * H), T, pools[i]).view(T, Mp, H)
            if i == 0:
                xi = x
            else:
                xi = outs[5 * (i - 1) + 3] if pools[i - 1] else outs[5 * (i - 1)]
            need_dx = i > 0 or bool(need[0])
            dx, gr = _tm_layer_backward(dh, xi, Ws[i], Us[i], ctx.params[3 * i + 2], h, g, c,
                                        ctx.params[3 * i:3 * i + 3], need[2 + 3 * i:5 + 3 * i], need_dx)
            grads[3 * i:3 * i + 3] = gr
            dh = dx
        return (dx if need[0] else None, None, *grads)


class _HipLSTMChainHead(torch.autograd.Function):

    @staticmethod
    def forward(ctx, x, y, mask, sums, hist, consts, pools, M, *params):
        from ..utils.native import hip_ops
        ops = hip_ops()
        ns = len(pools)
        Ws = [params[3 * i].contiguous() for i in range(ns + 1)]
        Us = [params[3 * i + 1].contiguous() for i in range(ns + 1)]
        bs = [params[3 * i + 2].contiguous() for i in range(ns + 1)]
        head = [p.contiguous() for p in params[3 * (ns + 1):]]
        need = any(ctx.needs_input_grad)
        e = x.new_zeros(0)
        sums_ = sums if sums is not None else e.double()
        hist_ = hist if hist is not None else e
        if _t4_chain_on() and pools[-1] == 3:
            outs = ops.lstm_chain_head_fwd(x, Ws[:ns], Us[:ns], bs[:ns], [int(p) for p in pools], need, Ws[ns],
                                           Us[ns], bs[ns], head, y, mask, int(M), *[float(c) for c in consts],
                                           sums_, hist_)
            h4, g4, c4, logits, loss = outs[-5:]
            del outs[-5:]
            hb = outs.pop()
            pk = outs.pop()
        else:
            outs = ops.lstm_chain_fwd_pack(x, Ws[:ns], Us[:ns], bs[:ns], [int(p) for p in pools], need, Ws[ns],
                                           Us[ns])
            pk = outs.pop()
            hb = e
            xt = outs[5 * (ns - 1) + 3] if pools[-1] else outs[5 * (ns - 1)]
            h4, g4, c4, logits, loss = ops.time4_head_fwd(xt, Ws[ns], Us[ns], bs[ns], pk, need, head, y, mask, int(M),
                                                          *[float(c) for c in consts], sums_, hist_)
        ctx.pools, ctx.consts, ctx.M = tuple(int(p) for p in pools), tuple(float(c) for c in consts), int(M)
        ctx.params = params
        ctx.set_materialize_grads(False)
        if need:
            ctx.save_for_backward(x, y, mask, *Ws, *Us, *head, *outs, h4, g4, c4, pk, hb)
        ctx.mark_non_differentiable(logits)
        return loss.reshape(()), logits

    @staticmethod
    def backward(ctx, dloss, _dlogits):
        from ..utils.native import hip_ops
        ops = hip_ops()
        pools = ctx.pools
        ns = len(pools)
        saved = ctx.saved_tensors
        x, y, mask = saved[:3]
        Ws, Us = saved[3:4 + ns], saved[4 + ns:5 + 2 * ns]
        head = saved[5 + 2 * ns:11 + 2 * ns]
        outs = saved[11 + 2 * ns:11 + 7 * ns]
        h4, g4, c4, pk, hb = saved[11 + 7 * ns:]
        need = ctx.needs_input_grad
        npar = 3 * (ns + 1)

        def layer_x(i):
            if i == 0:
                return x
            return outs[5 * (i - 1) + 3] if pools[i - 1] else outs[5 * (i - 1)]

        g = dloss.reshape(1).float()
        if not g.is_contiguous():
            g = g.contiguous()
        hsinks = [_grad_sink(p) for p in ctx.params[npar:]]
        xt = layer_x(ns)
        order = list(reversed(range(ns)))
        e8 = x.new_zeros(0, dtype=torch.uint8)
        chain_args = ([outs[5 * i + 1] for i in order], [outs[5 * i + 2] for i in order],
                      [Ws[i] for i in order], [Us[i] for i in order],
                      [outs[5 * i + 4] if pools[i] else e8 for i in order],
                      [pools[i] for i in order], [layer_x(i).shape[-1] for i in order],
                      [outs[5 * i].shape[0] for i in order])
        grads = [None] * npar
        sinks = {i: [_grad_sink(p) for p in ctx.params[3 * i:3 * i + 3]] for i in range(ns + 1)}
        if _t4_chain_on() and pools[-1] == 3 and xt.is_contiguous():
            res = ops.lstm_chain_head_bwd(g, xt, h4, g4, c4, Ws[ns], Us[ns], pk, hb, list(head), y, mask, ctx.M, *ctx.consts,
                                          [s for s, _ in hsinks], *chain_args)
            dz4 = res.pop(0)
        else:
            dz4, dxt = ops.time4_head_bwd(g, xt, h4, g4, c4, Ws[ns], Us[ns], pk, list(head), y, mask, ctx.M,
                                          *ctx.consts, [s for s, _ in hsinks])
            res = ops.lstm_chain_bwd(dxt, *chain_args)
        dzs = {ns: dz4}
        hs = {ns: h4}
        for k, i in enumerate(order):
            dzs[i] = res[k]
            hs[i] = outs[5 * i]
        for i in [ns] + order:
            nw = need[8 + 3 * i:11 + 3 * i]
            if not any(nw):
                continue
            h = hs[i]
            xi = layer_x(i)
            sk = sinks[i]
            if (_pipe_on(sk, h.shape[1]) and _pipe_x_ok(xi, Ws[i].shape[0])
                    and len(_Pipe.batch) < _MULTI_MAX - 2):
                _Pipe.batch.append(_pipe_job(dzs[i], xi, h, Ws[i], sk, h.shape[0] * h.shape[1], h.shape[1]))
            else:
                ops.lstm_tm_grads(dzs[i], xi, h, Ws[i], sk[0][0], sk[1][0], sk[2][0], False)
            grads[3 * i:3 * i + 3] = [None if (direct or not n) else buf for (buf, direct), n in zip(sk, nw)]
        hgrads = [None if (direct or not n) else buf for (buf, direct), n in zip(hsinks, need[8 + npar:])]
        dx = res[ns]
        return (dx if need[0] else None, None, None, None, None, None, None, None, *grads, *hgrads)


def lstm_chain_head_tm(x_tm: torch.Tensor, mods, pools, head, y: torch.Tensor, mask: torch.Tensor, M: int,
                       alpha1: float, alpha2: float, w0: float, w1: float, sums=None, hist=None):
    params = []
    for m in mods:
        params += [m.kernel, m.recurrent_kernel, m.bias]
    for d in head:
        params += [d.kernel, d.bias]
    return _HipLSTMChainHead.apply(x_tm, y, mask, sums, hist, (alpha1, alpha2, w0, w1), tuple(int(p) for p in pools),
                                   int(M), *params)


def _chain_bwd_on() -> bool:
    import os
    return os.environ.get("GNNQC_CHAIN_BWD", "1") == "1"


def _t4_chain_on() -> bool:
    import os
    return os.environ.get("GNNQC_T4_CHAIN", "1") == "1"


def _chain_on() -> bool:
    import os
    return os.environ.get("GNNQC_CHAIN", "1") == "1"


def lstm_chain_tm(x_tm: torch.Tensor, mods, pools) -> torch.Tensor:
    params = []
    for m in mods:
        params += [m.kernel, m.recurrent_kernel, m.bias]
    return _HipLSTMChain.apply(x_tm, tuple(int(p) for p in pools), *params)


_CHAIN_CAP = {}


def chain_capacity(device) -> int:
    device = torch.device(device)
    if device.type != "cuda":
        return 0
    idx = device.index if device.index is not None else torch.cuda.current_device()
    cap = _CHAIN_CAP.get(idx)
    if cap is None:
        from ..utils.native import hip_ops
        cap = int(hip_ops().lstm_chain_capacity(torch.empty(0, device=torch.device("cuda", idx))))
        _CHAIN_CAP[idx] = cap
    return cap


def chain_fits(Mp: int, n_stages: int, device=None, spare: int = 0) -> bool:
    if device is None:
        device = torch.device("cuda", torch.cuda.current_device())
    return (2 <= n_stages <= 8 and n_stages * ((Mp // 16 + 7) // 8 * 8) + spare <= chain_capacity(device))


_CHAIN_CTL = {}


def chain_ctl(device) -> Optional[torch.Tensor]:
    device = torch.device(device)
    if device.type != "cuda":
        return None
    idx = device.index if device.index is not None else torch.cuda.current_device()
    t = _CHAIN_CTL.get(idx)
    if t is None:
        from ..utils.native import hip_ops
        t = hip_ops().lstm_chain_ctl(torch.empty(0, device=torch.device("cuda", idx)))
        _CHAIN_CTL[idx] = t
    return t


class ChainTimeoutError(RuntimeError):
    """A chain consumer gave up waiting for its producer (not all workgroups were resident, or
    another kernel held the CUs): the affected results were computed from stale data."""


def check_chain(device, rejected_before: Optional[int] = None) -> int:
    ctl = chain_ctl(device)
    if ctl is None:
        return 0
    v = ctl.cpu().tolist()
    if v[2]:
        ctl[2:3].zero_()
        raise ChainTimeoutError("LSTM chain kernel: a consumer spin timed out; results of this pass are invalid "
                                "(is another kernel sharing the GPU, or is the device partitioned?)")
    if rejected_before is not None and v[3] > rejected_before:
        raise ChainTimeoutError(f"LSTM chain kernel: {v[3] - rejected_before} training step(s) rejected after a "
                                "consumer spin timeout (skipped on the device, parameters untouched)")
    return int(v[3])


class _HipLSTMTM(torch.autograd.Function):

    @staticmethod
    def forward(ctx, x, W, U, b, return_sequences: bool, pool: int = 0):
        from ..utils.native import hip_ops
        x = x.contiguous()
        need = any(ctx.needs_input_grad[:4])
        sg = not recompute_gates(x, U.shape[0], any(ctx.needs_input_grad[1:4]))
        h, g, c = hip_ops().lstm_tm_fwd(x, W.contiguous(), U.contiguous(), b.contiguous(), need, sg)
        ctx.params = (W, U, b)
        ctx.return_sequences = return_sequences
        out, idx = _pool_out(h, pool) if (pool and return_sequences) else (h, x.new_zeros(0, dtype=torch.uint8))
        ctx.pool = int(pool) if return_sequences else 0
        if need:
            ctx.save_for_backward(x, W, U, b, h, g, c, idx)
        return out if return_sequences else h[-1]

    @staticmethod
    def backward(ctx, dout):
        from ..utils.native import hip_ops
        x, W, U, b, h, g, c, idx = ctx.saved_tensors
        need = ctx.needs_input_grad
        wgrad = any(need[1:4])
        need_dx = bool(need[0])
        if not wgrad and not need_dx:
            return None, None, None, None, None
        if wgrad:
            sinks = [_grad_sink(p) for p in ctx.params]
        else:
            e = x.new_zeros(0)
            sinks = [(e, True)] * 3
        if wgrad and g.numel() > 0 and _pipe_on(sinks, x.shape[1]) and _pipe_x_ok(x, W.shape[0]):
            dout = _unpool(dout, idx, ctx.pool, h.shape[0])
            dx = _pipe_tm_backward(dout.contiguous(), g, c, x, h, W.contiguous(), U.contiguous(), sinks, need_dx)
        else:
            with _deferred_reduce(wgrad and all(d for _, d in sinks)):
                dx = hip_ops().lstm_tm_bwd(dout.contiguous(), g, c, x, h, W.contiguous(), U.contiguous(),
                                           b.contiguous(), sinks[0][0], sinks[1][0], sinks[2][0], need_dx,
                                           idx if ctx.pool else None, ctx.pool)
        grads = [None if (direct or not n) else buf for (buf, direct), n in zip(sinks, need[1:4])]
        return (dx if need_dx else None, *grads, None, None)


class _HipLSTMTMPair(torch.autograd.Function):

    @staticmethod
    def forward(ctx, x, WA, UA, bA, WB, UB, bB, pool: int = 0):
        from ..utils.native import hip_ops
        x = x.contiguous()
        need = any(ctx.needs_input_grad[:7])
        sg = not recompute_gates(x, UA.shape[0], any(ctx.needs_input_grad[1:7]))
        import os
        kp = int(pool) if (pool and os.environ.get("GNNQC_TM_POOL_IN_FWD", "0") == "1") else 0
        hA, gA, cA, hB, gB, cB, pooled, pidx = hip_ops().lstm_tm2_fwd(
            x, WA.contiguous(), UA.contiguous(), bA.contiguous(), WB.contiguous(), UB.contiguous(), bB.contiguous(),
            need, sg, kp)
        ctx.params = (WA, UA, bA, WB, UB, bB)
        if kp:
            out, idx = pooled, pidx
        else:
            out, idx = _pool_out(hB, pool) if pool else (hB, x.new_zeros(0, dtype=torch.uint8))
        ctx.pool = int(pool)
        if need:
            ctx.save_for_backward(x, WA, UA, bA, hA, gA, cA, WB, UB, bB, hB, gB, cB, idx)
        return out

    @staticmethod
    def backward(ctx, dout):
        from ..utils.native import hip_ops
        ops = hip_ops()
        x, WA, UA, bA, hA, gA, cA, WB, UB, bB, hB, gB, cB, idx = ctx.saved_tensors
        need = ctx.needs_input_grad
        e = x.new_zeros(0)
        dout = dout.contiguous()

        def sinks(params, flags):
            if any(flags):
                return [_grad_sink(p) for p in params]
            return [(e, True)] * 3

        sB = sinks(ctx.params[3:], need[4:7])
        sA = sinks(ctx.params[:3], need[1:4])
        need_dx = bool(need[0])
        dx = None
        if (any(need[4:7]) and any(need[1:4]) and gA.numel() > 0 and _pipe_on(sB, x.shape[1])
                and _pipe_on(sA, x.shape[1])
                and _pipe_x_ok(x, WA.shape[0]) and _pipe_x_ok(hA, WB.shape[0])):
            dout = _unpool(dout, idx, ctx.pool, hB.shape[0])
            dhA = _pipe_tm_backward(dout, gB, cB, hA, hB, WB.contiguous(), UB.contiguous(), sB, True)
            dx = _pipe_tm_backward(dhA, gA, cA, x, hA, WA.contiguous(), UA.contiguous(), sA, need_dx)
        else:
            with _deferred_reduce(all(d for _, d in sB) and all(d for _, d in sA)):
                dhA = ops.lstm_tm_bwd(dout, gB, cB, hA, hB, WB.contiguous(), UB.contiguous(), bB.contiguous(),
                                      sB[0][0], sB[1][0], sB[2][0], True, idx if ctx.pool else None, ctx.pool)
                if need_dx or any(need[1:4]):
                    dx = ops.lstm_tm_bwd(dhA, gA, cA, x, hA, WA.contiguous(), UA.contiguous(), bA.contiguous(),
                                         sA[0][0], sA[1][0], sA[2][0], need_dx)
        gA_ = [None if (direct or not n) else buf for (buf, direct), n in zip(sA, need[1:4])]
        gB_ = [None if (direct or not n) else buf for (buf, direct), n in zip(sB, need[4:7])]
        return (dx if need_dx else None, *gA_, *gB_, None)


def _pool_out(h: torch.Tensor, pool: int):
    from ..utils.native import hip_ops
    T, Mp, H = h.shape
    y, idx = hip_ops().maxpool1d_fwd(h.contiguous().view(1, T, Mp * H), int(pool))
    return y.view(T // pool, Mp, H), idx.view(T // pool, Mp, H)


def _unpool(dout: torch.Tensor, idx: torch.Tensor, pool: int, T: int) -> torch.Tensor:
    if not pool:
        return dout
    from ..utils.native import hip_ops
    Ts, Mp, H = dout.shape
    return hip_ops().maxpool1d_bwd(dout.contiguous().view(1, Ts, Mp * H), idx.view(1, Ts, Mp * H), T,
                                   int(pool)).view(T, Mp, H)


def pool_fusion() -> bool:
    import os
    return os.environ.get("GNNQC_TM_POOL_FUSE", "1") == "1"


def lstm_pair_tm(x_tm, A, B, pool: int = 0) -> torch.Tensor:
    return _HipLSTMTMPair.apply(x_tm, A.kernel, A.recurrent_kernel, A.bias, B.kernel, B.recurrent_kernel, B.bias,
                                int(pool))


def recompute_gates(x: torch.Tensor, H: int, weight_grads: bool) -> bool:
    import os
    if os.environ.get("GNNQC_TM_RG", "1") != "1" or H not in (16, 32):
        return False
    Din = x.shape[-1]
    if Din % 4 or Din > 64 or x.data_ptr() % 16 or not x.is_contiguous():
        return False
    return (not weight_grads) or x.shape[1] > PIPE_MAX_SEQ or not _Pipe.enabled


def tm_eligible(x: torch.Tensor, H: int, Din: int, activation: str = "tanh", bf16: bool = True) -> bool:
    from . import use_hip
    return (use_hip(x) and bf16 and activation == "tanh" and H in (16, 32, 64) and 1 <= Din <= 127
            and (16 * Din) // (4 if Din % 4 == 0 else (2 if Din % 2 == 0 else 1)) <= 16 * H)


def lstm_layer_tm(x_tm: torch.Tensor, W: torch.Tensor, U: torch.Tensor, b: torch.Tensor,
                  return_sequences: bool = True, pool: int = 0) -> torch.Tensor:
    return _HipLSTMTM.apply(x_tm, W, U, b, bool(return_sequences), int(pool))


class _HipLSTMLast128(torch.autograd.Function):

    @staticmethod
    def forward(ctx, x, W, U, b):
        from ..utils.native import hip_ops
        x = x.contiguous()
        need = any(ctx.needs_input_grad[:4])
        wgrad = any(ctx.needs_input_grad[1:4])
        h, g, c = hip_ops().time4_fwd(x, W.contiguous(), U.contiguous(), b.contiguous(), need, wgrad)
        ctx.params = (W, U, b)
        if need:
            ctx.save_for_backward(x, W, U, g, c, h if wgrad else x.new_zeros(0))
        return h[-1] if wgrad else h

    @staticmethod
    def backward(ctx, dout):
        from ..utils.native import hip_ops
        ops = hip_ops()
        x, W, U, g, c, h = ctx.saved_tensors
        need = ctx.needs_input_grad
        wgrad = any(need[1:4])
        Wc = W.contiguous()
        dz, dx = ops.time4_bwd(dout.contiguous(), x, g, c, Wc, U.contiguous(), wgrad)
        grads = [None, None, None]
        if wgrad:
            sinks = [_grad_sink(p) for p in ctx.params]
            with _deferred_reduce(all(d for _, d in sinks)):
                ops.lstm_tm_grads(dz, x, h, Wc, sinks[0][0], sinks[1][0], sinks[2][0], False)
            grads = [None if (direct or not n) else buf for (buf, direct), n in zip(sinks, need[1:4])]
        return (dx if need[0] else None, *grads)


class _HipLSTMLast128Prob(torch.autograd.Function):

    @staticmethod
    def forward(ctx, x, W, U, b, head, alphas, M):
        from ..utils.native import hip_ops
        x = x.contiguous()
        need = bool(ctx.needs_input_grad[0])
        prob, dh, g, c = hip_ops().time4_prob_fwd(x, W.contiguous(), U.contiguous(), b.contiguous(),
                                                  [t.contiguous() for t in head], float(alphas[0]),
                                                  float(alphas[1]), int(M), need)
        if need:
            ctx.save_for_backward(x, W, U, g, c, dh)
        ctx.M = int(M)
        return prob[:M]

    @staticmethod
    def backward(ctx, dprob):
        from ..utils.native import hip_ops
        x, W, U, g, c, dh = ctx.saved_tensors
        scale = dprob.float().contiguous()
        _, dx = hip_ops().time4_bwd(dh, x, g, c, W.contiguous(), U.contiguous(), False, 0, scale)
        return dx, None, None, None, None, None, None


def lstm_last128_prob_tm(x_tm: torch.Tensor, mod, head, alphas, M: int) -> torch.Tensor:
    if any(t.requires_grad for t in [mod.kernel, mod.recurrent_kernel, mod.bias, *head]):
        raise ValueError("lstm_last128_prob_tm: weights must be frozen (integrated gradients)")
    return _HipLSTMLast128Prob.apply(x_tm, mod.kernel, mod.recurrent_kernel, mod.bias, tuple(head), tuple(alphas), int(M))


def last128_eligible(x: torch.Tensor, mod) -> bool:
    import os
    from . import use_hip
    if os.environ.get("GNNQC_T4_TM", "1") != "1" or not use_hip(x) or x.dim() != 3:
        return False
    T, Mp, Din = x.shape
    return (mod.units == 128 and not mod.return_sequences and mod.activation == "tanh" and mod.compute_bf16
            and 1 <= T <= 16 and Mp % 16 == 0 and Din % 4 == 0 and 4 <= Din <= 64
            and mod.kernel.shape[0] <= Din and x.dtype == torch.float32)


def lstm_last128_tm(x_tm: torch.Tensor, mod) -> torch.Tensor:
    return _HipLSTMLast128.apply(x_tm, mod.kernel, mod.recurrent_kernel, mod.bias)


def lstm_layer(x: torch.Tensor, W: torch.Tensor, U: torch.Tensor, b: torch.Tensor,
               return_sequences: bool = True, activation: str = "tanh", bf16: bool = True) -> torch.Tensor:
    from . import use_hip
    H = U.shape[0]
    if use_hip(x) and activation == "tanh" and H % 16 == 0 and H in (16, 32, 64, 128) and x.shape[-1] <= 128:
        return _HipLSTM.apply(x, W, U, b, bool(bf16), bool(return_sequences))
    return lstm_eager(x, W, U, b, return_sequences, activation)


__all__ = ["unflagged_grad_writes", "lstm_layer", "lstm_eager", "lstm_layer_tm", "lstm_pair_tm", "lstm_chain_tm", "chain_fits", "tm_eligible",
           "chain_capacity", "chain_ctl", "check_chain", "ChainTimeoutError", "lstm_chain_head_tm",
           "lstm_last128_tm", "lstm_last128_prob_tm", "last128_eligible",
           "direct_grad_accumulation"]
```

Baseline: 562,100 train windows/s (whole job).

## Fuse LSTM weight-gradient partial products into the chain backward kernel epilogue

Each chain-backward stage block, after finishing its recurrent backward pass, now computes per-tile weight-gradient partial records (dz·[x,1] and dz·h_{t-1} via MFMA) in the LDS it already holds, and writes them to a workspace. The later multi-job grads kernel then only reduces those records, instead of running separate grads jobs that re-read dz, x and h. This removes a separate pass over the activations and a kernel's worth of work. In exchange the chain kernel gets longer per-block tails, adds kernel-argument size, and may delay the chain's completion signalling. It is gated by an env flag that defaults to on.

Result: faster. 575,700 train windows/s (whole job), median of 6 (+2.4%).

```diff
diff --git a/csrc/kernels/chain_wgrad.h b/csrc/kernels/chain_wgrad.h
--- /dev/null
+++ b/csrc/kernels/chain_wgrad.h
@@ -0,0 +1,141 @@
+#pragma once
+#include "lstm_grads_body.h"
+
+namespace gq {
+
+struct ChainWJob {
+  const float* x;
+  const float* h;
+  const __bf16* dz;
+  float* ws;
+  long x_elems;
+  int ldx, T, Din, on;
+};
+
+constexpr int CW_DTM = 5;
+
+template <int H>
+struct ChainWLds {
+  static constexpr int NCB = 4 * H / GR_CB;
+  static constexpr int NG = NCB < 4 ? NCB : 4;
+  static constexpr int DZT = NG * GR_CB * GR_LDR * 2;
+  static constexpr int XT = CW_DTM * 16 * GR_LDR * 2;
+  static constexpr int HT = H * GR_LDR * 2;
+  static constexpr int BYTES = DZT + XT + HT;
+};
+
+template <int H>
+__device__ __forceinline__ void chain_wgrad_body(const float* __restrict__ x, const float* __restrict__ hseq,
+                                                 const __bf16* __restrict__ dz, float* __restrict__ ws, long x_elems,
+                                                 int ldx, int T, int Dw, int Mp, int tile, char* __restrict__ smem) {
+  typedef __bf16 bf16x2_t __attribute__((ext_vector_type(2)));
+  using L = ChainWLds<H>;
+  constexpr int G4 = 4 * H, HT = H / 16, NCB = L::NCB, NG = L::NG, NPASS = NCB / NG, NTH = 256 * NG;
+  constexpr int NHI = 16 * H / 4;
+  static_assert(NCB % NG == 0 && 16 * 16 + NHI <= NTH && L::DZT % 16 == 0 && L::XT % 16 == 0, "chain wgrad tiling");
+  auto dzT = reinterpret_cast<__bf16 (*)[GR_LDR]>(smem);
+  auto xT = reinterpret_cast<__bf16 (*)[GR_LDR]>(smem + L::DZT);
+  auto hT = reinterpret_cast<__bf16 (*)[GR_LDR]>(smem + L::DZT + L::XT);
+
+  const int tid = threadIdx.x, lane = tid & 63;
+  const int wv = __builtin_amdgcn_readfirstlane(tid >> 6);
+  const bool act = wv < 4 * NG;
+  const int g = wv >> 2, wl = wv & 3;
+  const int col = lane & 15, quad = lane >> 4;
+  const int DT = (Dw + 1 + 15) / 16;
+  const int npairs = (T + 1) / 2;
+  const int seq0 = 16 * tile;
+
+  const int zq = tid % (NG * 16), zr = min(tid / (NG * 16), 15);
+  const size_t zstep = (size_t)Mp * G4;
+  const __bf16* zb = dz + (size_t)(seq0 + zr) * G4 + 4 * zq;
+  const int nq = (Dw + 3) / 4;
+  const bool isx = tid < 16 * nq, ish = act && tid >= NTH - NHI;
+  const int hi = max(tid - (NTH - NHI), 0);
+  const int ir = isx ? tid / nq : hi / (H / 4), iq = isx ? tid % nq : hi % (H / 4);
+  const long st = isx ? (long)Mp * ldx : (long)Mp * H;
+  const float* ib = isx ? x : hseq;
+  const long i0 = isx ? (long)(seq0 + ir) * ldx + 4 * iq : (long)(seq0 + ir) * H + 4 * iq;
+  const long ilast = isx ? (x_elems - 4) / 4 * 4 : (long)T * Mp * H - 4;
+  const int ioff = isx ? 0 : -1;
+  const int nch = isx ? min(4, Dw - 4 * iq) : 4;
+  __bf16* idst = &xT[(isx ? 0 : CW_DTM * 16) + 4 * iq][2 * ir];
+
+  if (act)
+    for (int e = tid; e < CW_DTM * 16 * GR_LDR; e += NTH) (&xT[0][0])[e] = (__bf16)0.f;
+
+  for (int ps = 0; ps < NPASS; ++ps) {
+    f32x4_t accW[CW_DTM], accU[HT];
+#pragma unroll
+    for (int d = 0; d < CW_DTM; ++d) accW[d] = f32x4_t{0.f, 0.f, 0.f, 0.f};
+#pragma unroll
+    for (int k = 0; k < HT; ++k) accU[k] = f32x4_t{0.f, 0.f, 0.f, 0.f};
+    const __bf16* zp = zb + ps * NG * GR_CB;
+    uint2 rz[2];
+    float4 ri[2];
+    auto load_pair = [&](int p) {
+      rz[0] = *reinterpret_cast<const uint2*>(zp + (size_t)(2 * p) * zstep);
+      rz[1] = *reinterpret_cast<const uint2*>(zp + (size_t)min(2 * p + 1, T - 1) * zstep);
+      if (isx || ish) {
+        const long o0 = (long)max(2 * p + ioff, 0) * st, o1 = (long)min(2 * p + 1 + ioff, T - 1) * st;
+        ri[0] = *reinterpret_cast<const float4*>(ib + min(i0 + o0, ilast));
+        ri[1] = *reinterpret_cast<const float4*>(ib + min(i0 + o1, ilast));
+      }
+    };
+    auto stage_pair = [&](int p) {
+      const bool v1 = 2 * p + 1 < T;
+      {
+        const unsigned a[4] = {rz[0].x << 16, rz[0].x & 0xffff0000u, rz[0].y << 16, rz[0].y & 0xffff0000u};
+        const unsigned b[4] = {rz[1].x << 16, rz[1].x & 0xffff0000u, rz[1].y << 16, rz[1].y & 0xffff0000u};
+#pragma unroll
+        for (int j = 0; j < 4; ++j)
+          *reinterpret_cast<unsigned*>(&dzT[4 * zq + j][2 * zr]) = (a[j] >> 16) | (v1 ? b[j] : 0u);
+      }
+      if (isx || ish) {
+        const bool v0 = 2 * p + ioff >= 0;
+        const float a[4] = {ri[0].x, ri[0].y, ri[0].z, ri[0].w};
+        const float b[4] = {ri[1].x, ri[1].y, ri[1].z, ri[1].w};
+#pragma unroll
+        for (int j = 0; j < 4; ++j)
+          if (j < nch)
+            *reinterpret_cast<bf16x2_t*>(idst + j * GR_LDR) = bf16x2_t{(__bf16)(v0 ? a[j] : 0.f), (__bf16)(v1 ? b[j] : 0.f)};
+      }
+      if (tid < 16) *reinterpret_cast<bf16x2_t*>(&xT[Dw][2 * tid]) = bf16x2_t{(__bf16)1.f, (__bf16)(v1 ? 1.f : 0.f)};
+    };
+
+    if (act) load_pair(0);
+    for (int p = 0; p < npairs; ++p) {
+      lds_barrier();
+      if (act) {
+        stage_pair(p);
+        load_pair(min(p + 1, npairs - 1));
+      }
+      lds_barrier();
+      if (act) {
+        const bf16x8_t az = *reinterpret_cast<const bf16x8_t*>(&dzT[GR_CB * g + 16 * wl + col][8 * quad]);
+#pragma unroll
+        for (int d = 0; d < CW_DTM; ++d) {
+          if (d < DT) {
+            const bf16x8_t bx = *reinterpret_cast<const bf16x8_t*>(&xT[16 * d + col][8 * quad]);
+            accW[d] = __builtin_amdgcn_mfma_f32_16x16x32_bf16(az, bx, accW[d], 0, 0, 0);
+          }
+        }
+#pragma unroll
+        for (int k = 0; k < HT; ++k) {
+          const bf16x8_t bh = *reinterpret_cast<const bf16x8_t*>(&hT[16 * k + col][8 * quad]);
+          accU[k] = __builtin_amdgcn_mfma_f32_16x16x32_bf16(az, bh, accU[k], 0, 0, 0);
+        }
+      }
+    }
+    if (act) {
+      float* rec = ws + ((size_t)tile * NCB + ps * NG + g) * (size_t)(DT + HT) * 1024;
+#pragma unroll
+      for (int d = 0; d < CW_DTM; ++d)
+        if (d < DT) *reinterpret_cast<f32x4_t*>(rec + ((size_t)(d * 4 + wl) * 64 + lane) * 4) = accW[d];
+#pragma unroll
+      for (int k = 0; k < HT; ++k) *reinterpret_cast<f32x4_t*>(rec + ((size_t)((DT + k) * 4 + wl) * 64 + lane) * 4) = accU[k];
+    }
+  }
+}
+
+}
diff --git a/csrc/kernels/lstm_chain.hip b/csrc/kernels/lstm_chain.hip
--- a/csrc/kernels/lstm_chain.hip
+++ b/csrc/kernels/lstm_chain.hip
@@ -1,4 +1,5 @@
 #include "chain_head.h"
+#include "chain_wgrad.h"
 #include "common.h"
 #include "gcn_fused.h"
 #include "lstm_grads_body.h"
@@ -870,6 +871,7 @@
   int* ctl;
   long long* trace;
   ChainT4B t4;
+  ChainWJob wj[CHAIN_MAX + 1];
 };
 static_assert(sizeof(ChainBArgs) <= 4096, "chain backward kernel arguments");
 
@@ -912,6 +914,8 @@
   static constexpr int BYTES = DHT + (STEP > HEAD ? STEP : HEAD);
 };
 static constexpr int CHAINB_LDS = ChainT4BLds::BYTES > CHAINB_LDS_STAGE ? ChainT4BLds::BYTES : CHAINB_LDS_STAGE;
+static_assert(ChainWLds<32>::BYTES <= CHAINB_LDS && ChainWLds<64>::BYTES <= CHAINB_LDS &&
+                  ChainWLds<128>::BYTES <= CHAINB_LDS, "the weight-gradient epilogue runs in the stages' LDS");
 
 #ifndef CHAINB_LEAD
 #define CHAINB_LEAD 1
@@ -1550,6 +1554,28 @@
   chain_head_bwd<128>(Q.hd, Q.h + (size_t)(Q.T - 1) * Mp * 128, tile, ntiles, reinterpret_cast<float*>(s), s + L::DHT);
 }
 
+static __device__ __noinline__ void chain_wgrad_epilogue(const ChainBKernArgs* ka_v, ChainLdsChar* smem, int job_v,
+                                                         int H_v, int tile_v) {
+  const unsigned long long kp = (unsigned long long)ka_v;
+  const ChainBKernArgs* ka = (const ChainBKernArgs*)(
+      ((unsigned long long)(unsigned)__builtin_amdgcn_readfirstlane((int)(kp >> 32)) << 32) |
+      (unsigned)__builtin_amdgcn_readfirstlane((int)kp));
+  const int job = __builtin_amdgcn_readfirstlane(job_v), H = __builtin_amdgcn_readfirstlane(H_v);
+  const int tile = __builtin_amdgcn_readfirstlane(tile_v);
+  const __attribute__((address_space(4))) ChainWJob* J = &ka->wj[job];
+  if (!J->on) return;
+  __syncthreads();
+  const float* x = J->x;
+  const float* h = J->h;
+  const __bf16* dz = J->dz;
+  float* ws = J->ws;
+  const long x_elems = J->x_elems;
+  const int ldx = J->ldx, T = J->T, Dw = J->Din, Mp = ka->Mp;
+  if (H == 32) chain_wgrad_body<32>(x, h, dz, ws, x_elems, ldx, T, Dw, Mp, tile, (char*)smem);
+  else if (H == 64) chain_wgrad_body<64>(x, h, dz, ws, x_elems, ldx, T, Dw, Mp, tile, (char*)smem);
+  else if (H == 128) chain_wgrad_body<128>(x, h, dz, ws, x_elems, ldx, T, Dw, Mp, tile, (char*)smem);
+}
+
 __device__ __forceinline__ void chain_t4_bwd_stage(const ChainT4B Q, const ChainBKernArgs* kargs, int tile, int ntiles,
                                                    int Mp, unsigned tagb, char* smem, long long* mk = nullptr) {
   constexpr int H = 128, G4 = 4 * H, NW = 16, CPL = 2, HP = H + 4, ZP = G4 + 8, XP = 68;
@@ -1670,6 +1696,7 @@
     __syncthreads();
     chain_t4_bwd_records(kargs, (ChainLdsChar*)smem, tile, ntiles, Mp);
   }
+  chain_wgrad_epilogue(kargs, (ChainLdsChar*)smem, CHAIN_MAX, H, tile);
   chain_head_bwd_reduce<H>(Q.hd, tile, ntiles);
 }
 
@@ -1724,6 +1751,8 @@
 #undef GQ_CHAINB_STAGE_16
 #undef GQ_CHAINB_STAGE_32
 #undef GQ_CHAINB_STAGE_64
+  if (H != 16)
+    chain_wgrad_epilogue((const ChainBKernArgs*)__builtin_amdgcn_kernarg_segment_ptr(), (ChainLdsChar*)smem, s, H, tile);
   __syncthreads();
   if (threadIdx.x == 0) A.trace[2 * blockIdx.x + 1] = (long long)__builtin_amdgcn_s_memrealtime();
   chain_finish(A.ctl, nblk);
@@ -2045,12 +2074,56 @@
                                                at::TensorList pidx, at::IntArrayRef pool, at::IntArrayRef x_width,
                                                at::IntArrayRef T_in, int extra_blocks);
 
+static ChainWJob chain_wgrad_job(const at::Tensor& x, const at::Tensor& h, const __bf16* dz, const at::Tensor& ws,
+                                 const at::Tensor& W, int H, int T, int Mp) {
+  check_f32_cuda(h, "lstm_chain_bwd weight-gradient h");
+  check_f32_cuda(ws, "lstm_chain_bwd weight-gradient workspace");
+  const int Dw = (int)W.size(0), ntiles = Mp / 16;
+  TORCH_CHECK(H == 32 || H == 64 || H == 128, "lstm_chain_bwd: a weight-gradient epilogue needs H = 32, 64 or 128");
+  TORCH_CHECK(Dw >= 1 && Dw <= 64 && W.size(1) == 4 * H, "lstm_chain_bwd: weight-gradient W shape");
+  TORCH_CHECK(x.is_cuda() && x.scalar_type() == at::kFloat && x.dim() == 3 && x.size(0) == T && x.size(1) == Mp &&
+                  x.size(2) >= Dw, "lstm_chain_bwd: weight-gradient x shape");
+  const long ldx = x.stride(1);
+  TORCH_CHECK(x.stride(2) == 1 && ldx % 4 == 0 && ldx >= x.size(2) && x.stride(0) == (long)Mp * ldx &&
+                  reinterpret_cast<uintptr_t>(x.data_ptr()) % 16 == 0, "lstm_chain_bwd: weight-gradient x layout");
+  const long x_elems = (long)(x.storage().nbytes() / sizeof(float)) - x.storage_offset();
+  TORCH_CHECK(((long)T * Mp - 1) * ldx + (Dw + 3) / 4 * 4 <= x_elems, "lstm_chain_bwd: weight-gradient x storage");
+  TORCH_CHECK(h.numel() == (long)T * Mp * H, "lstm_chain_bwd: weight-gradient h shape");
+  TORCH_CHECK(ws.numel() == (long)ntiles * GradsGeom(H, Dw).RC,
+              "lstm_chain_bwd: the weight-gradient workspace holds one record per tile");
+  ChainWJob J{};
+  J.x = x.data_ptr<float>();
+  J.h = h.data_ptr<float>();
+  J.dz = dz;
+  J.ws = ws.data_ptr<float>();
+  J.x_elems = x_elems;
+  J.ldx = (int)ldx;
+  J.T = T;
+  J.Din = Dw;
+  J.on = 1;
+  return J;
+}
+
+static void chain_wgrad_jobs(ChainBArgs& A, const std::vector<at::Tensor>& wgrad, at::TensorList W, at::IntArrayRef T_in) {
+  TORCH_CHECK((int)wgrad.size() >= 3 * A.ns, "lstm_chain_bwd: wgrad lists [x, h, ws] per stage");
+  for (int s = 0; s < A.ns; ++s) {
+    if (wgrad[3 * s + 2].numel() == 0) continue;
+    A.wj[s] = chain_wgrad_job(wgrad[3 * s], wgrad[3 * s + 1], A.st[s].dz, wgrad[3 * s + 2], W[s], A.st[s].H, (int)T_in[s],
+                              A.Mp);
+  }
+}
+
 std::vector<at::Tensor> lstm_chain_bwd(const at::Tensor& dh, at::TensorList g, at::TensorList c, at::TensorList W,
                                        at::TensorList U, at::TensorList pidx, at::IntArrayRef pool,
-                                       at::IntArrayRef x_width, at::IntArrayRef T_in) {
+                                       at::IntArrayRef x_width, at::IntArrayRef T_in,
+                                       c10::optional<std::vector<at::Tensor>> wgrad) {
   ChainBArgs A{};
   std::vector<at::Tensor> keep;
   auto res = chain_bwd_setup(A, keep, dh, g, c, W, U, pidx, pool, x_width, T_in, 0);
+  if (wgrad.has_value()) {
+    TORCH_CHECK((int)wgrad->size() == 3 * A.ns, "lstm_chain_bwd: wgrad lists [x, h, ws] per stage");
+    chain_wgrad_jobs(A, *wgrad, W, T_in);
+  }
   hipLaunchKernelGGL(lstm_chain_bwd_kernel, dim3(A.ns * A.nt8), dim3(1024), 0, stream(), A);
   GQ_LAUNCH_CHECK();
   return res;
@@ -2067,7 +2140,8 @@
                                             const at::Tensor& mask, int64_t M, double alpha1, double alpha2, double w0,
                                             double w1, at::TensorList hgrads, at::TensorList g, at::TensorList c,
                                             at::TensorList W, at::TensorList U, at::TensorList pidx,
-                                            at::IntArrayRef pool, at::IntArrayRef x_width, at::IntArrayRef T_in) {
+                                            at::IntArrayRef pool, at::IntArrayRef x_width, at::IntArrayRef T_in,
+                                            c10::optional<std::vector<at::Tensor>> wgrad) {
   check_f32_cuda(x4, "x4");
   for (const at::Tensor* t : {&dloss, &h4, &g4, &c4, &Wt4, &Ut4}) check_f32_cuda(*t, "lstm_chain_head_bwd operand");
   TORCH_CHECK(x4.dim() == 3 && x4.is_contiguous(), "lstm_chain_head_bwd: x4 must be a contiguous [T4, Mp, Din]");
@@ -2109,6 +2183,12 @@
   Q.Dw = Dw;
   at::Tensor gpart;
   t4_head_bwd_args(Q.hd, head, y, mask, M, Mp, alpha1, alpha2, w0, w1, dloss, hgrads, gpart);
+  if (wgrad.has_value()) {
+    TORCH_CHECK((int)wgrad->size() == 3 * A.ns + 1, "lstm_chain_head_bwd: wgrad lists [x, h, ws] per stage + time4's ws");
+    chain_wgrad_jobs(A, *wgrad, W, T_in);
+    const at::Tensor& ws4 = (*wgrad)[3 * A.ns];
+    if (ws4.numel() > 0) A.wj[CHAIN_MAX] = chain_wgrad_job(x4, h4, Q.dz, ws4, Wt4, 128, T4, Mp);
+  }
   hipLaunchKernelGGL(lstm_chain_bwd_kernel, dim3((A.ns + 1) * A.nt8), dim3(1024), 0, stream(), A);
   GQ_LAUNCH_CHECK();
   res.insert(res.begin(), dz4);
diff --git a/csrc/kernels/lstm_grads_jobs.hip b/csrc/kernels/lstm_grads_jobs.hip
--- a/csrc/kernels/lstm_grads_jobs.hip
+++ b/csrc/kernels/lstm_grads_jobs.hip
@@ -59,9 +59,11 @@
   int* nf;
 };
 
+template <int HMAX>
 __global__ __launch_bounds__(256) void lstm_grads_multi_kernel(MultiGrad M) {
-  __shared__ __attribute__((aligned(16))) char smem[GradsLds<128, 5>::BYTES];
-  static_assert(GcnBwdLds<2, 16>::BYTES <= GradsLds<128, 5>::BYTES, "GCN job LDS");
+  constexpr int LDSB = GradsLds<HMAX, 5>::BYTES > GcnBwdLds<2, 16>::BYTES ? GradsLds<HMAX, 5>::BYTES
+                                                                          : GcnBwdLds<2, 16>::BYTES;
+  __shared__ __attribute__((aligned(16))) char smem[LDSB];
   if ((int)blockIdx.x < M.gcn_nb) {
     const int gb = blockIdx.x;
     if (M.gcn_coef) gcn_coef_bwd_body<2, 16>(M.gcnc, gb);
@@ -76,9 +78,10 @@
   const int gb = b - M.start[k];
 #define GQ_MG(HG, DT)                                                                                    \
   case HG * 8 + DT:                                                                                      \
-    lstm_grads_body<HG, DT, 4>(gj.dz, gj.x, gj.h, gj.W, nullptr, gj.ws, gj.rows, gj.period, gj.hshift, gj.Din, \
-                               gj.ldx, 0, gj.Din, gj.xg, gj.x_elems, gb % gj.ncb, gb / gj.ncb, gj.ncb, gj.splits, \
-                               smem);                                                                    \
+    if constexpr (HG <= HMAX)                                                                            \
+      lstm_grads_body<HG, DT, 4>(gj.dz, gj.x, gj.h, gj.W, nullptr, gj.ws, gj.rows, gj.period, gj.hshift, gj.Din, \
+                                 gj.ldx, 0, gj.Din, gj.xg, gj.x_elems, gb % gj.ncb, gb / gj.ncb, gj.ncb, gj.splits, \
+                                 smem);                                                                  \
     break;
 #define GQ_MG_H(HG) GQ_MG(HG, 1) GQ_MG(HG, 2) GQ_MG(HG, 3) GQ_MG(HG, 4) GQ_MG(HG, 5)
   switch (M.key[k]) {
@@ -115,6 +118,15 @@
                                                             (long)PIPE_MAX_SPLITS}));
   c10::DeviceGuard guard(x.device());
   return at::empty({(long)splits * geo.RC}, x.options());
+}
+
+at::Tensor lstm_grads_record_ws(const at::Tensor& W, int64_t splits) {
+  check_f32_cuda(W, "W");
+  TORCH_CHECK(W.dim() == 2 && W.size(1) % 64 == 0 && splits >= 1 && splits <= PIPE_MAX_SPLITS,
+              "lstm_grads_record_ws: W [Din, 4H] and 1 .. ", PIPE_MAX_SPLITS, " records");
+  const GradsGeom geo((int)W.size(1) / 4, (int)W.size(0));
+  c10::DeviceGuard guard(W.device());
+  return at::empty({splits * (long)geo.RC}, W.options());
 }
 
 static bool grads_job_ok(const at::Tensor& x, int Dw) {
@@ -227,7 +239,7 @@
                           gcn_t[14], gcn_t[15], gcn_t[16], gcn_t[17], gcn_t[18], gcn_t[19], gcn_t[20], M.gcn_nb);
       TORCH_CHECK(M.gcn.key == 2 * 64 + 16, "lstm_grads_multi: the GCN job takes 2 input / 16 output channels");
     }
-    int nb = 0;
+    int nb = 0, hmax = 16;
     std::vector<at::Tensor> zb(ng);
     for (int k = 0; k < ng; ++k) {
       check_dz_cuda(gz[k]);
@@ -241,9 +253,11 @@
       M.key[k] = HG * 8 + GradsGeom::din_tiles(Dw);
       M.start[k] = nb;
       nb += M.j[k].nblocks;
+      hmax = std::max(hmax, HG);
     }
     M.start[ng] = nb;
-    hipLaunchKernelGGL(lstm_grads_multi_kernel, dim3(M.gcn_nb + nb), dim3(256), 0, st, M);
+    if (hmax == 16) hipLaunchKernelGGL(lstm_grads_multi_kernel<16>, dim3(M.gcn_nb + nb), dim3(256), 0, st, M);
+    else hipLaunchKernelGGL(lstm_grads_multi_kernel<128>, dim3(M.gcn_nb + nb), dim3(256), 0, st, M);
     GQ_LAUNCH_CHECK();
   }
   if (nr) {
@@ -326,5 +340,6 @@
   m.impl("lstm_tm_grads", &gq::lstm_tm_grads);
   m.impl("lstm_tm_bwd_pipe", &gq::lstm_tm_bwd_pipe);
   m.impl("lstm_grads_job_ws", &gq::lstm_grads_job_ws);
+  m.impl("lstm_grads_record_ws", &gq::lstm_grads_record_ws);
   m.impl("lstm_grads_multi", &gq::lstm_grads_multi);
 }
diff --git a/csrc/kernels/registry.hip b/csrc/kernels/registry.hip
--- a/csrc/kernels/registry.hip
+++ b/csrc/kernels/registry.hip
@@ -42,11 +42,11 @@
   m.def("lstm_chain_trace(Tensor like) -> Tensor");
   m.def("lstm_chain_prof(Tensor like) -> Tensor");
   m.def("lstm_chain_bwd(Tensor dh, Tensor[] g, Tensor[] c, Tensor[] W, Tensor[] U, Tensor[] pidx, int[] pool, "
-        "int[] x_width, int[] T_in) -> Tensor[]");
+        "int[] x_width, int[] T_in, Tensor[]? wgrad=None) -> Tensor[]");
   m.def("lstm_chain_head_bwd(Tensor dloss, Tensor x4, Tensor h4, Tensor g4, Tensor c4, Tensor Wt4, Tensor Ut4, "
         "Tensor pk, Tensor hb, Tensor[] head, Tensor y, Tensor mask, int M, float alpha1, float alpha2, float w0, float w1, "
         "Tensor(a!)[] hgrads, Tensor[] g, Tensor[] c, Tensor[] W, Tensor[] U, Tensor[] pidx, int[] pool, "
-        "int[] x_width, int[] T_in) -> Tensor[]");
+        "int[] x_width, int[] T_in, Tensor[]? wgrad=None) -> Tensor[]");
   m.def("time4_head_fwd(Tensor x, Tensor W, Tensor U, Tensor b, Tensor pk, bool train, Tensor[] head, Tensor y, Tensor mask, "
         "int M, float alpha1, float alpha2, float w0, float w1, Tensor(a!) sums, Tensor(b!) hist) -> Tensor[]");
   m.def("time4_head_bwd(Tensor dloss, Tensor x, Tensor h, Tensor g, Tensor c, Tensor W, Tensor U, Tensor pk, Tensor[] head, "
@@ -61,6 +61,7 @@
         "Tensor gh, Tensor gW, int g_period, int g_hshift, Tensor gws, Tensor rws, Tensor rW, Tensor(a!) rdW, "
         "Tensor(b!) rdU, Tensor(c!) rdb) -> Tensor");
   m.def("lstm_grads_job_ws(Tensor dz, Tensor x, Tensor W, int H) -> Tensor");
+  m.def("lstm_grads_record_ws(Tensor W, int splits) -> Tensor");
   m.def("lstm_tm_bwd(Tensor dh, Tensor g, Tensor c, Tensor x, Tensor h, Tensor W, Tensor U, Tensor b, Tensor(a!) dW, "
         "Tensor(b!) dU, Tensor(c!) db, bool need_dx, Tensor? pidx=None, int pool=0) -> Tensor");
   m.def("gcn_stats(Tensor x, Tensor mask) -> Tensor");
diff --git a/gnnqc/ops/lstm.py b/gnnqc/ops/lstm.py
--- a/gnnqc/ops/lstm.py
+++ b/gnnqc/ops/lstm.py
@@ -48,7 +48,29 @@
     job = None
     red = None
     batch = []
+    reds = []
     gcn = None
+
+
+class _ChainWgrad:
+    on = None
+
+
+def _chain_wgrad_on() -> bool:
+    if _ChainWgrad.on is None:
+        import os
+        _ChainWgrad.on = os.environ.get("GNNQC_CHAIN_WGRAD", "1") == "1"
+    return _ChainWgrad.on
+
+
+def _chain_wgrad_ws(x, h, W, sinks, need_w):
+    H = W.shape[1] // 4
+    if not (_chain_wgrad_on() and H in (32, 64, 128) and any(need_w) and _pipe_on(sinks, h.shape[1])
+            and _pipe_x_ok(x, W.shape[0]) and W.shape[0] <= 64 and x.dim() == 3
+            and x.stride(0) == x.shape[1] * x.stride(1)):
+        return None
+    from ..utils.native import hip_ops
+    return hip_ops().lstm_grads_record_ws(W, h.shape[1] // 16)
 
 
 PIPE_MAX_SEQ = 2048
@@ -96,17 +118,17 @@
 
 
 def pipe_flush():
-    if _Pipe.batch:
+    if _Pipe.batch or _Pipe.reds:
         from ..utils.native import hip_ops
         grads = ([_Pipe.job] if _Pipe.job is not None else []) + _Pipe.batch
-        reds = ([_Pipe.red] if _Pipe.red is not None else []) + grads
+        reds = ([_Pipe.red] if _Pipe.red is not None else []) + _Pipe.reds + grads
         gt, gi = _Pipe.gcn if _Pipe.gcn is not None else ([], [])
         hip_ops().lstm_grads_multi([j["dz"] for j in grads], [j["x"] for j in grads], [j["h"] for j in grads],
                                    [j["W"] for j in grads], [j["period"] for j in grads],
                                    [j["hshift"] for j in grads], [j["ws"] for j in grads],
                                    [r["ws"] for r in reds], [r["W"] for r in reds], [r["g"][0] for r in reds],
                                    [r["g"][1] for r in reds], [r["g"][2] for r in reds], gt, gi)
-        _Pipe.job, _Pipe.red, _Pipe.batch, _Pipe.gcn = None, None, [], None
+        _Pipe.job, _Pipe.red, _Pipe.batch, _Pipe.reds, _Pipe.gcn = None, None, [], [], None
     while _Pipe.job is not None or _Pipe.red is not None:
         _pipe_drain_one()
 
@@ -167,7 +189,7 @@
         yield
     finally:
         _DirectGrad.enabled = prev
-        if _Pipe.job is not None or _Pipe.red is not None or _Pipe.batch:
+        if _Pipe.job is not None or _Pipe.red is not None or _Pipe.batch or _Pipe.reds:
             pipe_flush()
         _Pipe.gcn = None
         if _Deferred.pending:
@@ -316,19 +338,28 @@
         if _chain_bwd_on() and chain_fits(dh.shape[1], ns, dh.device) and all(layer_x(i).shape[-1] % 4 == 0 for i in range(ns)):
             order = list(reversed(range(ns)))
             e8 = x.new_zeros(0, dtype=torch.uint8)
+            allsinks = {i: [_grad_sink(p) for p in ctx.params[3 * i:3 * i + 3]] for i in order
+                        if any(need[2 + 3 * i:5 + 3 * i])}
+            wws = {i: _chain_wgrad_ws(layer_x(i), outs[5 * i], Ws[i], allsinks[i], need[2 + 3 * i:5 + 3 * i])
+                   if i in allsinks else None for i in order}
+            e = x.new_zeros(0)
+            wgrad = None if all(w is None for w in wws.values()) else \
+                [t for i in order for t in (layer_x(i), outs[5 * i], wws[i] if wws[i] is not None else e)]
             res = ops.lstm_chain_bwd(dh, [outs[5 * i + 1] for i in order], [outs[5 * i + 2] for i in order],
                                      [Ws[i] for i in order], [Us[i] for i in order],
                                      [outs[5 * i + 4] if pools[i] else e8 for i in order],
                                      [pools[i] for i in order], [layer_x(i).shape[-1] for i in order],
-                                     [outs[5 * i].shape[0] for i in order])
+                                     [outs[5 * i].shape[0] for i in order], *(() if wgrad is None else (wgrad,)))
             for k, i in enumerate(order):
                 nw = need[2 + 3 * i:5 + 3 * i]
                 if not any(nw):
                     continue
                 h = outs[5 * i]
                 xi = layer_x(i)
-                sinks = [_grad_sink(p) for p in ctx.params[3 * i:3 * i + 3]]
-                if (_pipe_on(sinks, h.shape[1]) and _pipe_x_ok(xi, Ws[i].shape[0])
+                sinks = allsinks[i]
+                if wws[i] is not None:
+                    _Pipe.reds.append(dict(ws=wws[i], W=Ws[i], g=[s for s, _ in sinks]))
+                elif (_pipe_on(sinks, h.shape[1]) and _pipe_x_ok(xi, Ws[i].shape[0])
                         and len(_Pipe.batch) < _MULTI_MAX - 2):
                     _Pipe.batch.append(_pipe_job(res[k], xi, h, Ws[i], sinks, h.shape[0] * h.shape[1], h.shape[1]))
                 else:
@@ -426,19 +457,27 @@
                       [outs[5 * i].shape[0] for i in order])
         grads = [None] * npar
         sinks = {i: [_grad_sink(p) for p in ctx.params[3 * i:3 * i + 3]] for i in range(ns + 1)}
-        if _t4_chain_on() and pools[-1] == 3 and xt.is_contiguous():
+        hs = {i: outs[5 * i] for i in order}
+        hs[ns] = h4
+        t4_chain = _t4_chain_on() and pools[-1] == 3 and xt.is_contiguous()
+        wws = {i: _chain_wgrad_ws(layer_x(i), hs[i], Ws[i], sinks[i], need[8 + 3 * i:11 + 3 * i])
+               for i in (order + [ns] if t4_chain else order)}
+        e = x.new_zeros(0)
+        wgrad = [t for i in order for t in (layer_x(i), hs[i], wws[i] if wws[i] is not None else e)]
+        if t4_chain:
+            wgrad.append(wws[ns] if wws[ns] is not None else e)
+        wopt = () if all(w is None for w in wws.values()) else (wgrad,)
+        if t4_chain:
             res = ops.lstm_chain_head_bwd(g, xt, h4, g4, c4, Ws[ns], Us[ns], pk, hb, list(head), y, mask, ctx.M, *ctx.consts,
-                                          [s for s, _ in hsinks], *chain_args)
+                                          [s for s, _ in hsinks], *chain_args, *wopt)
             dz4 = res.pop(0)
         else:
             dz4, dxt = ops.time4_head_bwd(g, xt, h4, g4, c4, Ws[ns], Us[ns], pk, list(head), y, mask, ctx.M,
                                           *ctx.consts, [s for s, _ in hsinks])
-            res = ops.lstm_chain_bwd(dxt, *chain_args)
+            res = ops.lstm_chain_bwd(dxt, *chain_args, *wopt)
         dzs = {ns: dz4}
-        hs = {ns: h4}
         for k, i in enumerate(order):
             dzs[i] = res[k]
-            hs[i] = outs[5 * i]
         for i in [ns] + order:
             nw = need[8 + 3 * i:11 + 3 * i]
             if not any(nw):
@@ -446,7 +485,9 @@
             h = hs[i]
             xi = layer_x(i)
             sk = sinks[i]
-            if (_pipe_on(sk, h.shape[1]) and _pipe_x_ok(xi, Ws[i].shape[0])
+            if wws.get(i) is not None:
+                _Pipe.reds.append(dict(ws=wws[i], W=Ws[i], g=[s for s, _ in sk]))
+            elif (_pipe_on(sk, h.shape[1]) and _pipe_x_ok(xi, Ws[i].shape[0])
                     and len(_Pipe.batch) < _MULTI_MAX - 2):
                 _Pipe.batch.append(_pipe_job(dzs[i], xi, h, Ws[i], sk, h.shape[0] * h.shape[1], h.shape[1]))
             else:
```
